# SYNCC-IN/hyperscanning-signal-analysis

Hardware: AMD Instinct MI355X
Metric: MVAR+ffDTF windows/sec, 2x32-ch dyad p=8, 256 freqs (higher is better)
Workload: dtype f64; 1 GPU; C2: 1 dyad(s)/GPU, 2x32 ch @500 Hz, 10 min, 2 s windows 50% overlap (599 windows per dyad), MVAR p=8, 256 freqs 0.5-128 Hz; dyads_per_gpu=1, k1=hop blocks summed once, shared by the overlapping windows (hop 500), k2=block Levinson-Whittle recursion, one workgroup per window, one launch, normalisation=inside K3 (rows of window w by workgroups of window w+lag), parallelism=dyad-sharded x1, gather=none

## Files before the change

### hyperscanning_signal_analysis_amd/_lib.py

```python
from __future__ import annotations

import ctypes
import os
from ctypes import POINTER, c_char_p, c_double, c_int, c_int32, c_int64, c_void_p

_HERE = os.path.dirname(os.path.abspath(__file__))
LIB_PATH = os.path.join(_HERE, "libhypermvar.so")

SIGNATURES = {
    "hmv_version": (c_int, []),
    "hmv_last_error": (c_char_p, []),
    "hmv_pad": (c_int, [c_int]),
    "hmv_set_tuning": (c_int, [c_int, c_int64]),
    "hmv_get_tuning": (c_int64, [c_int]),
    "hmv_yw_workspace_doubles": (c_int64, [c_int, c_int]),
    "hmv_lagcov_f64": (c_int, [c_void_p, c_int64, c_int64, c_void_p, c_void_p, c_int64, c_int, c_int, c_int,
                               c_void_p, c_void_p]),
    "hmv_lagcov_regular_workspace_doubles": (c_int64, [c_int64, c_int, c_int, c_int64, c_int]),
    "hmv_lagcov_regular_f64": (c_int, [c_void_p, c_int64, c_int64, c_int64, c_int64, c_int64, c_int, c_int, c_int,
                                       c_void_p, c_void_p, c_void_p]),
    "hmv_yw_solve_f64": (c_int, [c_void_p, c_int64, c_int, c_int, c_void_p, c_void_p, c_void_p, c_void_p,
                                 c_void_p, c_int64, c_void_p]),
    "hmv_twiddles_f64": (c_int, [c_void_p, c_int, c_double, c_int, c_void_p, c_void_p]),
    "hmv_tf_workspace_doubles": (c_int64, [c_int64, c_int, c_int]),
    "hmv_tf_f64": (c_int, [c_void_p, c_int64, c_int, c_int, c_void_p, c_int, c_void_p, c_void_p, c_void_p,
                           c_void_p, c_void_p, c_double, c_void_p, c_void_p]),
    "hmv_ffdtf_norm_f64": (c_int, [c_void_p, c_void_p, c_void_p, c_void_p, c_int64, c_int, c_int, c_int,
                                   c_void_p]),
    "hmv_transpose_c128": (c_int, [c_void_p, c_void_p, c_int64, c_int, c_int, c_void_p]),
    "hmv_spectra_f64": (c_int, [c_void_p, c_void_p, c_void_p, c_int64, c_int, c_int, c_void_p]),
    "hmv_spectra_mmf_f64": (c_int, [c_void_p, c_void_p, c_void_p, c_int64, c_int, c_int, c_void_p]),
    "hmv_pack_c128": (c_int, [c_void_p, c_void_p, c_int64, c_int, c_int, c_void_p]),
    "hmv_cinv_c128": (c_int, [c_void_p, c_int64, c_int, c_int, c_void_p, c_void_p, c_void_p, c_double, c_void_p]),
    "hmv_partial_coherence_c128": (c_int, [c_void_p, c_void_p, c_void_p, c_int64, c_int, c_int, c_void_p]),
    "hmv_gpdc_f64": (c_int, [c_void_p, c_void_p, c_void_p, c_int64, c_int, c_int, c_void_p]),
    "hmv_trial_mean_f64": (c_int, [c_void_p, c_int64, c_int, c_int, c_void_p, c_void_p]),
    "hmv_ddtf_f64": (c_int, [c_void_p, c_void_p, c_void_p, c_int64, c_int, c_int, c_void_p]),
    "hmv_band_sums_f64": (c_int, [c_void_p, c_int64, c_int, c_void_p, c_void_p, c_int, c_void_p, c_void_p]),
    "hmv_dpss_workspace_bytes": (c_int64, [c_int64, c_int, c_int]),
    "hmv_dpss_f64": (c_int, [c_int64, c_double, c_int, c_int, c_void_p, c_void_p, c_void_p, c_int64, c_void_p]),
    "hmv_psd_workspace_bytes": (c_int64, [c_int64, c_int64, c_int]),
    "hmv_psd_multitaper_f64": (c_int, [c_void_p, c_int64, c_int64, c_int64, c_void_p, c_void_p, c_int, c_int64, c_int64,
                                       c_void_p, c_void_p, c_int64, c_int64, c_void_p]),
    "hmv_sliding_workspace_bytes": (c_int64, [c_int64, c_int, c_int, c_int]),
    "hmv_tf_ffdtf_workspace_bytes": (c_int64, [c_int64, c_int, c_int, c_int]),
    "hmv_tf_ffdtf_f64": (c_int, [c_void_p, c_int64, c_int, c_int, c_void_p, c_int, c_void_p, c_void_p, c_void_p, c_void_p,
                                 c_double, c_void_p, c_int64, c_int64, c_void_p, c_void_p, c_void_p]),
    "hmv_tf_ffdtf_bands_workspace_bytes": (c_int64, [c_int64, c_int, c_int, c_int]),
    "hmv_tf_ffdtf_bands_f64": (c_int, [c_void_p, c_int64, c_int, c_int, c_void_p, c_int, c_void_p, c_void_p, c_void_p, c_int,
                                       c_void_p, c_void_p, c_double, c_void_p, c_int64, c_int64, c_void_p, c_void_p,
                                       c_void_p]),
    "hmv_sliding_bands_workspace_bytes": (c_int64, [c_int64, c_int, c_int, c_int]),
    "hmv_sliding_ffdtf_bands_f64": (c_int, [c_void_p, c_int64, c_int64, c_void_p, c_void_p, c_int64, c_int, c_int,
                                            c_int, c_void_p, c_int, c_double, c_void_p, c_void_p, c_void_p, c_int,
                                            c_void_p, c_void_p, c_void_p, c_void_p, c_void_p, c_int64, c_int64, c_double,
                                            c_int64, c_int64, c_int64, c_int64, c_int64, c_void_p, c_void_p, c_void_p,
                                            c_void_p]),
    "hmv_sliding_spectra_workspace_bytes": (c_int64, [c_int64, c_int, c_int, c_int]),
    "hmv_sliding_ffdtf_spectra_f64": (c_int, [c_void_p, c_int64, c_int64, c_void_p, c_void_p, c_int64, c_int, c_int,
                                              c_int, c_void_p, c_int, c_double, c_void_p, c_void_p, c_void_p, c_void_p,
                                              c_void_p, c_void_p, c_void_p, c_int64, c_int64, c_double, c_int64, c_int64,
                                              c_int64, c_int64, c_int64, c_void_p, c_void_p]),
    "hmv_sliding_ffdtf_f64": (c_int, [c_void_p, c_int64, c_int64, c_void_p, c_void_p, c_int64, c_int, c_int,
                                      c_int, c_void_p, c_int, c_double, c_void_p, c_void_p, c_void_p, c_void_p,
                                      c_void_p, c_void_p, c_int64, c_int64, c_double, c_int64, c_int64, c_int64, c_int64,
                                      c_int64, c_void_p, c_void_p, c_void_p, c_void_p]),
    "hmv_sliding_ddtf_workspace_bytes": (c_int64, [c_int64, c_int, c_int, c_int, c_int]),
    "hmv_sliding_ddtf_f64": (c_int, [c_void_p, c_int64, c_int64, c_void_p, c_void_p, c_int64, c_int, c_int, c_int, c_void_p,
                                     c_int, c_double, c_void_p, c_void_p, c_void_p, c_int, c_void_p, c_void_p, c_void_p,
                                     c_void_p, c_void_p, c_int64, c_int64, c_double, c_int64, c_int64, c_int64, c_int64,
                                     c_int64, c_void_p, c_void_p]),
    "hmv_sliding_gpdc_workspace_bytes": (c_int64, [c_int64, c_int, c_int, c_int, c_int]),
    "hmv_sliding_gpdc_f64": (c_int, [c_void_p, c_int64, c_int64, c_void_p, c_void_p, c_int64, c_int, c_int, c_int, c_void_p,
                                     c_int, c_double, c_void_p, c_void_p, c_void_p, c_int, c_void_p, c_void_p, c_void_p,
                                     c_void_p, c_int64, c_int64, c_int64, c_int64, c_int64, c_int64, c_int64, c_void_p,
                                     c_void_p]),
    "hmv_yw_solve_auto_f64": (c_int, [c_void_p, c_int64, c_int, c_int, c_int, c_int] + [c_void_p] * 7 + [c_int64, c_void_p]),
    "hmv_sliding_auto_workspace_bytes": (c_int64, [c_int, c_int64, c_int, c_int, c_int, c_int]),
    "hmv_sliding_auto_f64": (c_int, [c_int, c_void_p, c_int64, c_int64, c_void_p, c_void_p, c_int64, c_int, c_int, c_int,
                                     c_int, c_void_p, c_int, c_double, c_void_p, c_void_p, c_void_p, c_int] +
                             [c_void_p] * 8 + [c_int64, c_int64, c_double, c_int64, c_int64, c_int64, c_int64, c_int64,
                                               c_void_p, c_void_p]),
    "hmv_lagcov_ensemble_workspace_doubles": (c_int64, [c_int64, c_int, c_int, c_int, c_int64, c_int64]),
    "hmv_lagcov_ensemble_f64": (c_int, [c_void_p, c_int64, c_int64, c_int64, c_void_p, c_void_p, c_void_p, c_int64,
                                        c_void_p, c_void_p, c_int64, c_int, c_int, c_int, c_void_p, c_void_p, c_int64,
                                        c_int64, c_int64, c_int64, c_void_p]),
    "hmv_sliding_ensemble_workspace_bytes": (c_int64, [c_int, c_int64, c_int, c_int, c_int, c_int, c_int, c_int64, c_int64]),
    "hmv_sliding_ensemble_f64": (c_int, [c_int, c_void_p, c_int64, c_int64, c_int64, c_void_p, c_void_p, c_void_p, c_int64,
                                         c_void_p, c_void_p, c_int64, c_int, c_int, c_int, c_void_p, c_int, c_double,
                                         c_void_p, c_void_p, c_void_p, c_int] + [c_void_p] * 6 +
                                 [c_int64, c_int64, c_double, c_int64, c_int64, c_int64, c_void_p, c_void_p]),
    "hmv_fad_workspace_bytes": (c_int64, [c_int64, c_int]),
    "hmv_fad_f64": (c_int, [c_void_p, c_int64, c_int64, c_void_p, c_void_p, c_int64, c_int, c_int, c_int, c_int, c_int,
                            c_double, c_double, c_int] + [c_void_p] * 17),
    "hmv_fad_decompose_f64": (c_int, [c_void_p, c_int64, c_int, c_double, c_double, c_int] + [c_void_p] * 13),
    "hmv_surrogate_shift_f64": (c_int, [c_void_p, c_int64, c_int64, c_int64, c_void_p, c_void_p, c_int64, c_void_p, c_int64,
                                        c_int, c_int, c_int, c_int, c_void_p, c_void_p]),
    "hmv_surrogate_phase_c128": (c_int, [c_void_p, c_int64, c_void_p, c_int, c_int, c_int, c_void_p, c_void_p]),
    "hmv_null_accumulate_f64": (c_int, [c_void_p, c_void_p, c_void_p, c_void_p, c_int64, c_int, c_int, c_int] + [c_void_p] * 12),
}

FLAG_UNFUSED_NORM = 1
FLAG_YW_TILED = 2
FLAG_YW_ONE_LAUNCH = 4
FLAG_DIRECT_LAGCOV = 8
MEASURE_FFDTF = 0
MEASURE_DDTF = 1
MEASURE_GPDC = 2
CRITERIA = {"AIC": 0, "HQ": 1, "SC": 2}
TUNE_NORM_LAG = 1
TUNE_LAG_GROUP = 2
TUNE_K3_FORM = 3
TUNE_YW_FORM = 4
TUNE_K3_LDS_PAD = 5


_lib = None


class HypermvarLibraryError(ImportError):
    pass


def load():
    global _lib
    if _lib is not None:
        return _lib
    global LIB_PATH
    LIB_PATH = os.environ.get("HYPERMVAR_LIB", LIB_PATH)
    if not os.path.exists(LIB_PATH):
        raise HypermvarLibraryError(
            f"{LIB_PATH} not found: build the HIP library first "
            f"(python -c 'import __graft_entry__ as g; g.build()' or make -C {_HERE}/csrc). "
            "There is no CPU fallback for the MVAR/ffDTF path.")
    lib = ctypes.CDLL(LIB_PATH)
    for name, (res, args) in SIGNATURES.items():
        try:
            fn = getattr(lib, name)
        except AttributeError as e:
            raise HypermvarLibraryError(f"{LIB_PATH} does not export {name}") from e
        fn.restype = res
        fn.argtypes = args
    _lib = lib
    return lib


def check(rc: int, what: str):
    if rc == 0:
        return
    lib = load()
    if rc < 0:
        raise ValueError(f"{what}: {lib.hmv_last_error().decode()} (code {rc})")
    raise RuntimeError(f"{what}: HIP error {rc}")
```

### hyperscanning_signal_analysis_amd/csrc/capi.hip

```cpp
#include "../../include/hypermvar.h"
#include "hmv_kernels.h"

#include <atomic>
#include <cmath>
#include <cstdio>
#include <cstdlib>
#include <cstring>

namespace {
thread_local char g_err[256] = "";

int fail(int code, const char* msg) {
  snprintf(g_err, sizeof(g_err), "%s", msg);
  return code;
}
int pad_of(int m) { return (m < 1 || m > HMV_MAX_CHANNELS) ? -1 : ((m + 15) / 16) * 16; }
inline hipStream_t S(void* s) { return reinterpret_cast<hipStream_t>(s); }
inline size_t align256(size_t b) { return (b + 255) & ~size_t(255); }

constexpr int N_TUNE = 6;
struct TuneRange { long long lo, hi; };
constexpr TuneRange kTuneRange[N_TUNE] = {{0, 0}, {0, 1 << 20}, {0, 3}, {0, 2}, {0, 3}, {0, 140000}};
long long env_knob(const char* name, int key) {
  const char* e = getenv(name);
  if (!e || !*e) return 0;
  char* end = nullptr;
  const long long v = strtoll(e, &end, 10);
  if (end == e || *end != 0 || v < kTuneRange[key].lo || v > kTuneRange[key].hi) {
    fprintf(stderr, "hypermvar: ignoring %s=%s (not an integer in %lld..%lld)\n", name, e, kTuneRange[key].lo,
            kTuneRange[key].hi);
    return 0;
  }
  return v;
}
std::atomic<long long> g_tune[N_TUNE] = {{0}, {env_knob("HYPERMVAR_NORM_LAG", 1)}, {env_knob("HYPERMVAR_LAG_GROUP", 2)},
                                         {env_knob("HYPERMVAR_K3_FORM", 3)}, {env_knob("HYPERMVAR_YW_FORM", 4)},
                                         {env_knob("HYPERMVAR_K3_LDS_PAD", 5)}};
}

namespace hmv {
long long tuning(int key) { return (key >= 1 && key < N_TUNE) ? g_tune[key].load(std::memory_order_relaxed) : -1; }
}

#ifdef HMV_STAMP
static unsigned long long* g_tf_stamps = nullptr;
extern "C" void hmv_debug_set_tf_stamps(void* p) { g_tf_stamps = static_cast<unsigned long long*>(p); }
#endif

extern "C" {

int hmv_version(void) { return HMV_VERSION; }
const char* hmv_last_error(void) { return g_err; }
int hmv_pad(int m) { return pad_of(m); }

int hmv_set_tuning(int key, int64_t value) {
  if (key < 1 || key >= N_TUNE) return fail(-1, "hmv_set_tuning: unknown key");
  if (value < kTuneRange[key].lo || value > kTuneRange[key].hi) return fail(-1, "hmv_set_tuning: value out of range");
  g_tune[key].store(value, std::memory_order_relaxed);
  return 0;
}
int64_t hmv_get_tuning(int key) { return hmv::tuning(key); }

int64_t hmv_yw_workspace_doubles(int m, int p) {
  const int mp = pad_of(m);
  if (mp < 0 || p < 1 || p > HMV_MAX_ORDER) return -1;
  return hmv::yw_ws_tiles(p) * (int64_t)mp * mp;
}

int hmv_lagcov_f64(const double* x, int64_t rec_stride, int64_t ld, const int64_t* item_rec,
                   const int64_t* item_start, int64_t n_items, int m, int n, int p, double* R, void* stream) {
  const int mp = pad_of(m);
  if (mp < 0) return fail(-1, "hmv_lagcov_f64: channel count must be in 1..64");
  if (p < 1 || p > HMV_MAX_ORDER) return fail(-2, "hmv_lagcov_f64: model order must be in 1..32");
  if (n <= p) return fail(-3, "hmv_lagcov_f64: window shorter than the model order");
  if (!x || !item_rec || !item_start || !R || n_items < 0) return fail(-4, "hmv_lagcov_f64: null pointer");
  hmv::LagcovArgs a{};
  a.x = x; a.rec_stride = rec_stride; a.ld = ld;
  a.item_rec = reinterpret_cast<const long long*>(item_rec);
  a.item_start = reinterpret_cast<const long long*>(item_start);
  a.n_items = n_items; a.m = m; a.n = n; a.p = p; a.R = R;
  return hmv::launch_lagcov(a, mp, S(stream));
}

int64_t hmv_lagcov_regular_workspace_doubles(int64_t n_win, int m, int n, int64_t hop, int p) {
  const int mp = pad_of(m);
  if (mp < 0 || n_win < 0 || hop < 1 || n < 1 || n % hop != 0 || p < 0) return -1;
  return (n_win + n / hop - 1) * (int64_t)(p + 1) * mp * mp;
}

int hmv_lagcov_regular_f64(const double* x, int64_t ld, int64_t T, int64_t first, int64_t hop, int64_t n_win, int m,
                           int n, int p, double* R, double* workspace, void* stream) {
  const int mp = pad_of(m);
  if (mp < 0) return fail(-1, "hmv_lagcov_regular_f64: channel count must be in 1..64");
  if (p < 1 || p > HMV_MAX_ORDER) return fail(-2, "hmv_lagcov_regular_f64: model order must be in 1..32");
  if (n <= p) return fail(-3, "hmv_lagcov_regular_f64: window shorter than the model order");
  if (!x || !R || !workspace || n_win < 0) return fail(-4, "hmv_lagcov_regular_f64: null pointer");
  if (hop < 1 || n % hop != 0 || hop <= p)
    return fail(-5, "hmv_lagcov_regular_f64: the window must be a whole number of hops and a hop longer than the order");
  if (first < 0 || ld < T || (n_win > 0 && first + (n_win - 1) * hop + n > T))
    return fail(-6, "hmv_lagcov_regular_f64: windows do not lie inside the recording");
  if (n_win == 0) return 0;
  const int k = (int)(n / hop);
  hmv::LagcovArgs a{};
  a.x = x; a.rec_stride = 0; a.ld = ld; a.item_rec = nullptr; a.item_start = nullptr;
  a.n_items = n_win + k - 1; a.m = m; a.n = (int)hop; a.p = p; a.R = workspace;
  a.blocks = 1; a.blk_first = first; a.blk_T = T;
  int rc = hmv::launch_lagcov(a, mp, S(stream));
  if (rc) return rc;
  hmv::LagcombArgs c{};
  c.Q = workspace; c.x = x; c.ld = ld; c.first = first; c.hop = hop; c.T = T; c.n_win = n_win; c.k = k; c.m = m; c.p = p;
  c.R = R;
  return hmv::launch_lagcomb(c, mp, S(stream));
}

namespace {
bool ens_shared_form(int n, int p, int64_t grid_hop, int64_t flags) {
  return grid_hop > 0 && !(flags & HMV_FLAG_DIRECT_LAGCOV) &&
         hmv::lagcov_ensemble_shared_ok(n, grid_hop, p, HMV_MAX_HOPS_ENSEMBLE);
}
bool ens_grid_ok(int64_t n_items, int64_t n_groups, int n, int64_t ld, int64_t T, int64_t grid_hop, int64_t grid_nwin) {
  return grid_hop > 0 && grid_nwin >= 1 && n_items == n_groups * grid_nwin && (grid_nwin - 1) * grid_hop + n <= T && ld >= T;
}
int64_t ens_q_tiles(int64_t n_items, int n, int p, int64_t grid_hop, int64_t grid_nwin) {
  if (grid_hop <= 0 || grid_nwin < 1 || !ens_shared_form(n, p, grid_hop, 0)) return 0;
  return hmv::lagcov_ensemble_q_tiles(n_items, grid_nwin, (int)(n / grid_hop));
}
}

int64_t hmv_lagcov_ensemble_workspace_doubles(int64_t n_items, int m, int n, int p, int64_t grid_hop, int64_t grid_nwin) {
  const int mp = pad_of(m);
  if (mp < 0 || n_items < 0 || p < 1 || p > HMV_MAX_ORDER || n <= p || grid_hop < 0 || grid_nwin < 0) return -1;
  return ens_q_tiles(n_items, n, p, grid_hop, grid_nwin) * (int64_t)(p + 1) * mp * mp;
}

int hmv_lagcov_ensemble_f64(const double* x, int64_t rec_stride, int64_t ld, int64_t T, const int64_t* trial_rec,
                            const int64_t* trial_start, const int64_t* group_ptr, int64_t n_groups,
                            const int64_t* item_group, const int64_t* item_offset, int64_t n_items, int m, int n, int p,
                            double* R, double* workspace, int64_t workspace_doubles, int64_t grid_hop, int64_t grid_nwin,
                            int64_t flags, void* stream) {
  const int mp = pad_of(m);
  if (mp < 0) return fail(-1, "hmv_lagcov_ensemble_f64: channel count must be in 1..64");
  if (p < 1 || p > HMV_MAX_ORDER) return fail(-2, "hmv_lagcov_ensemble_f64: model order must be in 1..32");
  if (n <= p) return fail(-3, "hmv_lagcov_ensemble_f64: window shorter than the model order");
  if (!x || !trial_rec || !trial_start || !group_ptr || !item_group || !item_offset || !R || n_items < 0)
    return fail(-4, "hmv_lagcov_ensemble_f64: null pointer");
  if (n_groups < 1) return fail(-10, "hmv_lagcov_ensemble_f64: n_groups must be >= 1");
  if (grid_hop != 0 && !ens_grid_ok(n_items, n_groups, n, ld, T, grid_hop, grid_nwin))
    return fail(-9, "hmv_lagcov_ensemble_f64: inconsistent regular window grid");
  const bool shared = ens_shared_form(n, p, grid_hop, flags);
  if (shared) {
    const int64_t need = ens_q_tiles(n_items, n, p, grid_hop, grid_nwin) * (int64_t)(p + 1) * mp * mp;
    if (!workspace || workspace_doubles < need) return fail(-7, "hmv_lagcov_ensemble_f64: workspace too small");
  }
  hmv::LagcovEnsArgs a{};
  a.x = x; a.rec_stride = rec_stride; a.ld = ld; a.T = T;
  a.trial_rec = reinterpret_cast<const long long*>(trial_rec);
  a.trial_start = reinterpret_cast<const long long*>(trial_start);
  a.group_ptr = reinterpret_cast<const long long*>(group_ptr);
  a.item_group = reinterpret_cast<const long long*>(item_group);
  a.item_offset = reinterpret_cast<const long long*>(item_offset);
  a.n_items = n_items; a.m = m; a.n = n; a.p = p; a.R = R;
  if (shared) { a.it0 = 0; a.nwin = grid_nwin; a.hop = grid_hop; a.k = (int)(n / grid_hop); a.Q = workspace; }
  return hmv::launch_lagcov_ensemble(a, mp, shared, S(stream));
}

int hmv_yw_solve_f64(const double* R, int64_t n_items, int m, int p, double* ws, double* ar, double* V,
                     double* vq_logdet, int32_t* info, int64_t flags, void* stream) {
  const int mp = pad_of(m);
  if (mp < 0) return fail(-1, "hmv_yw_solve_f64: channel count must be in 1..64");
  if (p < 1 || p > HMV_MAX_ORDER) return fail(-2, "hmv_yw_solve_f64: model order must be in 1..32");
  if (!R || !ws || !ar || !V || !info || n_items < 0) return fail(-4, "hmv_yw_solve_f64: null pointer");
  hmv::YwArgs a{};
  a.R = R; a.n_items = n_items; a.m = m; a.p = p; a.ws = ws; a.ar = ar; a.V = V;
  a.Vq_logdet = vq_logdet; a.info = info; a.tiled = (flags & HMV_FLAG_YW_TILED) ? 1 : ((flags & HMV_FLAG_YW_ONE_LAUNCH) ? 0 : -1);
  return hmv::launch_yw(a, mp, S(stream));
}

namespace {
double crit_factor(int crit, int n) {
  return crit == 0 ? 2.0 : (crit == 1 ? 2.0 * log(log((double)n)) : log((double)n));
}
}

int hmv_yw_solve_auto_f64(const double* R, int64_t n_items, int m, int pmax, int n, int crit, double* ws, double* ar,
                          double* V, int32_t* order_out, double* crit_out, double* vq_logdet, int32_t* info, int64_t flags,
                          void* stream) {
  const int mp = pad_of(m);
  if (mp < 0) return fail(-1, "hmv_yw_solve_auto_f64: channel count must be in 1..64");
  if (pmax < 1 || pmax > HMV_MAX_ORDER) return fail(-2, "hmv_yw_solve_auto_f64: largest model order must be in 1..32");
  if (n <= pmax) return fail(-3, "hmv_yw_solve_auto_f64: window shorter than the largest model order");
  if (crit < 0 || crit > 2) return fail(-5, "hmv_yw_solve_auto_f64: criterion must be 0 (AIC), 1 (HQ) or 2 (SC)");
  if (flags & (HMV_FLAG_YW_TILED | HMV_FLAG_YW_ONE_LAUNCH))
    return fail(-6, "hmv_yw_solve_auto_f64: the LDL^T forms of K2 have no automatic order");
  if (!R || !ws || !ar || !V || !order_out || !info || n_items < 0) return fail(-4, "hmv_yw_solve_auto_f64: null pointer");
  hmv::YwArgs a{};
  a.R = R; a.n_items = n_items; a.m = m; a.p = pmax; a.ws = ws; a.ar = ar; a.V = V; a.Vq_logdet = vq_logdet; a.info = info;
  a.tiled = -1;
  hmv::YwAutoArgs sel{};
  sel.n = n; sel.crit_c = crit_factor(crit, n); sel.order_out = order_out; sel.crit_out = crit_out;
  return hmv::launch_yw_auto(a, sel, mp, S(stream));
}

int hmv_twiddles_f64(const double* freqs, int F, double fs, int p, double* tw, void* stream) {
  if (!freqs || !tw || F < 0 || p < 1) return fail(-4, "hmv_twiddles_f64: bad argument");
  if (F == 0) return 0;
  return hmv::launch_twiddles(freqs, F, fs, p, tw, S(stream));
}

int64_t hmv_tf_workspace_doubles(int64_t n_items, int m, int p) {
  const int mp = pad_of(m);
  if (mp < 0 || p < 1 || n_items < 0) return -1;
  return (int64_t)hmv::tf_workspace_doubles(n_items, mp, p);
}

int hmv_tf_f64(const double* ar, int64_t n_items, int m, int p, const double* tw, int F, double* P,
               double* rowsum, double* H, double* A, int32_t* info, double pivot_tau, double* ws,
               void* stream) {
  const int mp = pad_of(m);
  if (mp < 0) return fail(-1, "hmv_tf_f64: channel count must be in 1..64");
  if (p < 1) return fail(-2, "hmv_tf_f64: model order must be >= 1");
  if (!ar || !tw || !info || !ws || n_items < 0 || F < 0) return fail(-4, "hmv_tf_f64: null pointer");
  if ((P == nullptr) != (rowsum == nullptr)) return fail(-5, "hmv_tf_f64: P and rowsum go together");
  if (!(pivot_tau > 0.0) || pivot_tau > 1.0) return fail(-6, "hmv_tf_f64: pivot_tau must be in (0, 1]");
  hmv::TfArgs a{};
  a.ar = ar; a.arx = ws; a.tw = tw; a.Zin = nullptr; a.detph = nullptr; a.P = P; a.rowsum = rowsum; a.H = H; a.A = A; a.info = info;
  a.n_items = n_items; a.F = F; a.p = p; a.m = m; a.tau = pivot_tau;
  a.stamps = nullptr;
#ifdef HMV_STAMP
  a.stamps = g_tf_stamps;
#endif
  return hmv::launch_tf_inv(a, mp, S(stream));
}

int hmv_ffdtf_norm_f64(const double* P, const double* rowsum, double* den, double* out, int64_t n_items,
                       int F, int m, int normalise, void* stream) {
  const int mp = pad_of(m);
  if (mp < 0) return fail(-1, "hmv_ffdtf_norm_f64: channel count must be in 1..64");
  if (!P || !out || (normalise && (!rowsum || !den))) return fail(-4, "hmv_ffdtf_norm_f64: null pointer");
  hmv::NormArgs a;
  a.P = P; a.rowsum = rowsum; a.den = den; a.out = out; a.n_items = n_items; a.F = F; a.m = m; a.m_pad = mp;
  a.normalise = normalise;
  return hmv::launch_ffdtf_norm(a, S(stream));
}

int hmv_transpose_c128(const double* in, double* out, int64_t n_items, int F, int m, void* stream) {
  const int mp = pad_of(m);
  if (mp < 0) return fail(-1, "hmv_transpose_c128: channel count must be in 1..64");
  if (!in || !out) return fail(-4, "hmv_transpose_c128: null pointer");
  return hmv::launch_transpose_c128(in, out, n_items, F, m, mp, S(stream));
}

int hmv_spectra_f64(const double* H, const double* V, double* Sout, int64_t n_items, int m, int F, void* stream) {
  const int mp = pad_of(m);
  if (mp < 0) return fail(-1, "hmv_spectra_f64: channel count must be in 1..64");
  if (!H || !V || !Sout) return fail(-4, "hmv_spectra_f64: null pointer");
  hmv::SpecArgs a;
  a.H = H; a.V = V; a.S = Sout; a.S_mmf = nullptr; a.n_items = n_items; a.F = F; a.m = m; a.sym = 0;
  return hmv::launch_spectra(a, mp, S(stream));
}

int hmv_spectra_mmf_f64(const double* H, const double* V, double* Sout, int64_t n_items, int m, int F, void* stream) {
  const int mp = pad_of(m);
  if (mp < 0) return fail(-1, "hmv_spectra_mmf_f64: channel count must be in 1..64");
  if (!H || !V || !Sout) return fail(-4, "hmv_spectra_mmf_f64: null pointer");
  hmv::SpecArgs a;
  a.H = H; a.V = V; a.S = nullptr; a.S_mmf = Sout; a.n_items = n_items; a.F = F; a.m = m; a.sym = 0;
  return hmv::launch_spectra(a, mp, S(stream));
}

int hmv_pack_c128(const double* in, double* out, int64_t n_items, int F, int m, void* stream) {
  const int mp = pad_of(m);
  if (mp < 0) return fail(-1, "hmv_pack_c128: channel count must be in 1..64");
  if (!in || !out || n_items < 0 || F < 0) return fail(-4, "hmv_pack_c128: null pointer");
  return hmv::launch_pack_c128(in, out, n_items, F, m, mp, S(stream));
}

int hmv_cinv_c128(const double* Z, int64_t n_items, int m, int F, double* Zinv, double* detph, int32_t* info,
                  double pivot_tau, void* stream) {
  const int mp = pad_of(m);
  if (mp < 0) return fail(-1, "hmv_cinv_c128: channel count must be in 1..64");
  if (!Z || !Zinv || !info || n_items < 0 || F < 0) return fail(-4, "hmv_cinv_c128: null pointer");
  if (!(pivot_tau > 0.0) || pivot_tau > 1.0) return fail(-6, "hmv_cinv_c128: pivot_tau must be in (0, 1]");
  hmv::TfArgs a{};
  a.ar = nullptr; a.arx = nullptr; a.tw = nullptr; a.Zin = Z; a.detph = detph; a.P = nullptr; a.rowsum = nullptr;
  a.H = Zinv; a.A = nullptr; a.info = info; a.n_items = n_items; a.F = F; a.p = 0; a.m = m; a.tau = pivot_tau;
  a.stamps = nullptr;
  return hmv::launch_cinv(a, mp, S(stream));
}

int hmv_partial_coherence_c128(const double* Sinv, const double* detph, double* kappa, int64_t n_items, int m, int F,
                               void* stream) {
  const int mp = pad_of(m);
  if (mp < 0) return fail(-1, "hmv_partial_coherence_c128: channel count must be in 1..64");
  if (!Sinv || !detph || !kappa || n_items < 0 || F < 0) return fail(-4, "hmv_partial_coherence_c128: null pointer");
  return hmv::launch_pcoh(Sinv, detph, kappa, n_items, F, m, mp, S(stream));
}

int hmv_gpdc_f64(const double* A, const double* V, double* G, int64_t n_items, int m, int F, void* stream) {
  const int mp = pad_of(m);
  if (mp < 0) return fail(-1, "hmv_gpdc_f64: channel count must be in 1..64");
  if (!A || !V || !G || n_items < 0 || F < 0) return fail(-4, "hmv_gpdc_f64: null pointer");
  return hmv::launch_gpdc(A, V, G, n_items, F, m, mp, S(stream));
}

int hmv_trial_mean_f64(const double* R_trials, int64_t n_trials, int m, int p, double* R_mean, void* stream) {
  const int mp = pad_of(m);
  if (mp < 0) return fail(-1, "hmv_trial_mean_f64: channel count must be in 1..64");
  if (!R_trials || !R_mean || n_trials < 1 || n_trials > 0x7fffffff || p < 0)
    return fail(-4, "hmv_trial_mean_f64: bad argument");
  return hmv::launch_trial_mean(R_trials, R_mean, (long long)(p + 1) * mp * mp, (int)n_trials, S(stream));
}

int hmv_ddtf_f64(const double* ffdtf, const double* kappa, double* ddtf, int64_t n_items, int m, int F, void* stream) {
  if (!ffdtf || !kappa || !ddtf || n_items < 0 || m < 1 || F < 0) return fail(-4, "hmv_ddtf_f64: bad argument");
  return hmv::launch_ddtf(ffdtf, kappa, ddtf, (long long)n_items * m * m * F, S(stream));
}

int hmv_band_sums_f64(const double* ffdtf, int64_t n_rows, int F, const int32_t* bin_lo, const int32_t* bin_hi,
                      int n_bands, double* out, void* stream) {
  if (!ffdtf || !bin_lo || !bin_hi || !out || n_rows < 0 || F < 1 || n_bands < 0)
    return fail(-4, "hmv_band_sums_f64: bad argument");
  return hmv::launch_band_sums(ffdtf, bin_lo, bin_hi, out, n_rows, F, n_bands, S(stream));
}

int64_t hmv_psd_workspace_bytes(int64_t ch_chunk, int64_t n_times, int n_tapers) {
  if (ch_chunk < 1 || n_times < 2 || n_tapers < 1) return -1;
  return (int64_t)hmv::psd_workspace_bytes(ch_chunk, n_times, n_tapers);
}

int hmv_psd_multitaper_f64(const double* x, int64_t n_ch, int64_t n_times, int64_t ld, const double* tapers,
                           const double* weights, int n_tapers, int64_t bin_lo, int64_t bin_hi, double* psd,
                           void* workspace, int64_t workspace_bytes, int64_t ch_chunk, void* stream) {
  if (!x || !tapers || !weights || !psd || !workspace) return fail(-4, "hmv_psd_multitaper_f64: null pointer");
  if (n_ch < 0 || n_times < 2 || n_times > 0x7fffffff || n_tapers < 1 || ch_chunk < 1 || ld < n_times)
    return fail(-2, "hmv_psd_multitaper_f64: bad size");
  if (bin_lo < 0 || bin_hi < bin_lo || bin_hi > n_times / 2) return fail(-3, "hmv_psd_multitaper_f64: bad frequency bins");
  if (workspace_bytes < hmv::psd_workspace_bytes(ch_chunk, n_times, n_tapers))
    return fail(-7, "hmv_psd_multitaper_f64: workspace too small");
  const int rc = hmv::launch_psd(x, n_ch, n_times, ld, tapers, weights, n_tapers, bin_lo, bin_hi, psd, workspace, ch_chunk,
                                 S(stream));
  if (rc <= -20) return fail(rc, "hmv_psd_multitaper_f64: hipFFT plan / execution failed");
  return rc;
}

int64_t hmv_dpss_workspace_bytes(int64_t n_times, int k_max, int sym) {
  if (n_times < 2 || k_max < 1 || k_max > n_times) return -1;
  return (int64_t)hmv::dpss_workspace_bytes(n_times, k_max, sym != 0);
}

int hmv_dpss_f64(int64_t n_times, double half_nbw, int k_max, int sym, double* tapers, double* ratios, void* workspace,
                 int64_t workspace_bytes, void* stream) {
  if (!tapers || !workspace) return fail(-4, "hmv_dpss_f64: null pointer");
  if (n_times < 2 || n_times > 0x3fffffff || k_max < 1 || k_max > n_times)
    return fail(-2, "hmv_dpss_f64: bad size");
  if (!(half_nbw > 0.0) || half_nbw >= 0.5 * (double)n_times)
    return fail(-3, "hmv_dpss_f64: the time-half-bandwidth product must lie in (0, n_times / 2)");
  if (workspace_bytes < hmv::dpss_workspace_bytes(n_times, k_max, sym != 0)) return fail(-7, "hmv_dpss_f64: workspace too small");
  const int rc = hmv::launch_dpss(n_times, half_nbw, k_max, sym != 0, tapers, ratios, workspace, S(stream));
  if (rc <= -20) return fail(rc, "hmv_dpss_f64: hipFFT plan / execution failed");
  if (rc < 0) return fail(rc, "hmv_dpss_f64: bad argument");
  return rc;
}

namespace {
struct TfFfWs {
  size_t off_arx, off_P, off_rowsum, off_cnt, off_tail, total;
};
int64_t norm_lag_items(int mp, int F);
TfFfWs tf_ff_layout(int64_t n, int mp, int p, int F, bool bands = false) {
  TfFfWs w;
  size_t o = 0;
  const size_t t = (size_t)mp * mp;
  w.off_arx = o;    o += align256(sizeof(double) * hmv::tf_workspace_doubles(n, mp, p));
  w.off_P = o;      o += align256(sizeof(double) * n * F * t);
  w.off_rowsum = o; o += align256(sizeof(double) * n * F * mp);
  w.off_cnt = o;    o += align256(sizeof(int) * (2 * n + 1 + n * mp));
  w.off_tail = o;
  if (bands) {
    const int64_t lag = norm_lag_items(mp, F);
    o += align256(sizeof(double) * (size_t)(n < lag ? n : lag) * F * t);
  }
  w.total = o;
  return w;
}
int64_t norm_lag_items(int mp, int F) {
  const int64_t slots = (mp == 64 || mp == 48) ? 1024 : (mp == 32 ? 2048 : 5120);
  int64_t lag = (6 * slots + F - 1) / (F < 1 ? 1 : F);
  if (const int64_t t = hmv::tuning(HMV_TUNE_NORM_LAG)) lag = t;
  return lag < 8 ? 8 : lag;
}
}

int64_t hmv_tf_ffdtf_workspace_bytes(int64_t n_items, int m, int p, int F) {
  const int mp = pad_of(m);
  if (mp < 0 || n_items < 0 || p < 1 || F < 1) return -1;
  return (int64_t)tf_ff_layout(n_items, mp, p, F).total;
}

namespace {
int tf_ffdtf_impl(const char* who, const double* ar, int64_t n_items, int m, int p, const double* tw, int F, double* ffdtf,
                  double* band_out, const int32_t* bin_lo, const int32_t* bin_hi, int n_bands, double* den, double* H,
                  int32_t* info, double pivot_tau, void* workspace, int64_t workspace_bytes, int64_t flags,
                  void* ev_k3_start, void* ev_k3_stop, void* stream) {
  auto failw = [&](int code, const char* msg) {
    char buf[200];
    snprintf(buf, sizeof(buf), "%s: %s", who, msg);
    return fail(code, buf);
  };
  const int mp = pad_of(m);
  const bool bands = (band_out != nullptr);
  if (mp < 0) return failw(-1, "channel count must be in 1..64");
  if (p < 1) return failw(-2, "model order must be >= 1");
  if (n_items == 0) return 0;
  if (!ar || !tw || (!ffdtf && !bands) || !den || !info || !workspace || n_items < 0 || F < 1)
    return failw(-4, "null pointer / empty grid");
  if (!(pivot_tau > 0.0) || pivot_tau > 1.0) return failw(-6, "pivot_tau must be in (0, 1]");
  if (bands) {
    if (!bin_lo || !bin_hi || n_bands < 1) return failw(-4, "band bins missing");
    if (F % 32 != 0 || F > hmv::tf_band_max_F(mp) || (flags & HMV_FLAG_UNFUSED_NORM))
      return failw(-10, "in-kernel band sums need F % 32 == 0, F within the row worker's LDS block and the fused normalisation");
  }
  const TfFfWs w = tf_ff_layout(n_items, mp, p, F, bands);
  if ((int64_t)w.total > workspace_bytes) return failw(-7, "workspace too small");
  char* base = static_cast<char*>(workspace);
  const size_t t = (size_t)mp * mp;
  hmv::TfArgs a{};
  a.ar = ar; a.arx = reinterpret_cast<double*>(base + w.off_arx); a.tw = tw;
  a.P = reinterpret_cast<double*>(base + w.off_P); a.rowsum = reinterpret_cast<double*>(base + w.off_rowsum);
  a.H = H;
  a.info = info; a.n_items = n_items; a.F = F; a.p = p; a.m = m; a.tau = pivot_tau;
  const bool fused = bands || (!(flags & HMV_FLAG_UNFUSED_NORM) && (F % 16 == 0) && (reinterpret_cast<uintptr_t>(ffdtf) % 16 == 0));
  const int64_t lag = norm_lag_items(mp, F);
  const int64_t n_fused = fused ? n_items : 0;
  if (n_fused > 0) {
    a.ff = bands ? nullptr : ffdtf; a.den = den; a.fuse_items = n_fused; a.lag = (int)lag;
    if (bands) {
      a.bands = band_out; a.band_lo = reinterpret_cast<const int*>(bin_lo); a.band_hi = reinterpret_cast<const int*>(bin_hi);
      a.nb = n_bands;
    }
    a.wcount = reinterpret_cast<int*>(base + w.off_cnt);
    a.ready = a.wcount + n_items;
    a.missed = a.ready + n_items;
  }
#ifdef HMV_STAMP
  a.stamps = g_tf_stamps;
#endif
  hipStream_t st = S(stream);
  int rc = hmv::launch_tf_inv(a, mp, st, reinterpret_cast<hipEvent_t>(ev_k3_start), reinterpret_cast<hipEvent_t>(ev_k3_stop));
  if (rc) return rc;
  if (n_fused < n_items) {
    const int64_t n_tail = n_items - n_fused;
    double* tail = bands ? reinterpret_cast<double*>(base + w.off_tail) : ffdtf + (size_t)n_fused * m * m * F;
    rc = hmv_ffdtf_norm_f64(a.P + (size_t)n_fused * F * t, a.rowsum + (size_t)n_fused * F * mp, den + (size_t)n_fused * mp,
                            tail, n_tail, F, m, 1, stream);
    if (!rc && bands)
      rc = hmv::launch_band_sums(tail, reinterpret_cast<const int*>(bin_lo), reinterpret_cast<const int*>(bin_hi),
                                 band_out + (size_t)n_fused * m * m * n_bands, n_tail * (long long)m * m, F, n_bands, st);
  }
  return rc;
}
}

int64_t hmv_tf_ffdtf_bands_workspace_bytes(int64_t n_items, int m, int p, int F) {
  const int mp = pad_of(m);
  if (mp < 0 || n_items < 0 || p < 1 || F < 1) return -1;
  return (int64_t)tf_ff_layout(n_items, mp, p, F, true).total;
}

int hmv_tf_ffdtf_f64(const double* ar, int64_t n_items, int m, int p, const double* tw, int F, double* ffdtf,
                     double* den, double* H, int32_t* info, double pivot_tau, void* workspace, int64_t workspace_bytes,
                     int64_t flags, void* ev_k3_start, void* ev_k3_stop, void* stream) {
  return tf_ffdtf_impl("hmv_tf_ffdtf_f64", ar, n_items, m, p, tw, F, ffdtf, nullptr, nullptr, nullptr, 0, den, H, info,
                       pivot_tau, workspace, workspace_bytes, flags, ev_k3_start, ev_k3_stop, stream);
}

int hmv_tf_ffdtf_bands_f64(const double* ar, int64_t n_items, int m, int p, const double* tw, int F, double* band_out,
                           const int32_t* bin_lo, const int32_t* bin_hi, int n_bands, double* den, int32_t* info,
                           double pivot_tau, void* workspace, int64_t workspace_bytes, int64_t flags, void* ev_k3_start,
                           void* ev_k3_stop, void* stream) {
  if (!band_out) return fail(-4, "hmv_tf_ffdtf_bands_f64: null pointer / empty grid");
  return tf_ffdtf_impl("hmv_tf_ffdtf_bands_f64", ar, n_items, m, p, tw, F, nullptr, band_out, bin_lo, bin_hi, n_bands, den,
                       nullptr, info, pivot_tau, workspace, workspace_bytes, flags, ev_k3_start, ev_k3_stop, stream);
}

namespace {
enum Measure { MEAS_FFDTF = 0, MEAS_DDTF = 1, MEAS_GPDC = 2 };
struct SlidingWs {
  size_t off_R, off_Q, off_ws, off_ar, off_V, off_tf, off_den, off_tw, off_H, off_B, off_G, off_full, total;
};
SlidingWs sliding_layout(int64_t chunk, int mp, int p, int F, bool bands = false, bool spectra = false, int measure = MEAS_FFDTF,
                         int64_t q_tiles = -1) {
  SlidingWs w;
  size_t o = 0;
  const size_t t = (size_t)mp * mp;
  w.off_R = o;      o += align256(sizeof(double) * chunk * (p + 1) * t);
  w.off_Q = o;      o += align256(sizeof(double) * (q_tiles >= 0 ? q_tiles : chunk + HMV_MAX_HOPS_PER_WINDOW - 1) * (p + 1) * t);
  w.off_ws = o;     o += align256(sizeof(double) * chunk * hmv::yw_ws_tiles(p) * t);
  w.off_ar = o;     o += align256(sizeof(double) * chunk * t * p);
  w.off_V = o;      o += align256(sizeof(double) * chunk * t);
  w.off_tf = o;
  if (measure != MEAS_GPDC) o += tf_ff_layout(chunk, mp, p, F, bands && measure == MEAS_FFDTF).total;
  w.off_den = o;    o += align256(sizeof(double) * chunk * mp);
  w.off_tw = o;     o += align256(sizeof(double) * F * p * 2);
  w.off_H = o;
  if (spectra) o += align256(sizeof(double) * 2 * chunk * F * t);
  w.off_B = o;
  if (measure == MEAS_DDTF) o += align256(sizeof(double) * chunk * (p + 1) * t);
  w.off_G = o;
  if (measure == MEAS_DDTF) o += align256(sizeof(double) * chunk * (2 * p + 1) * t);
  w.off_full = o;
  if (measure != MEAS_FFDTF && bands) o += align256(sizeof(double) * chunk * (mp * mp) * F);
  w.total = o;
  return w;
}
int64_t sliding_bytes(int64_t chunk, int m, int p, int F, int n_bands = 0, bool spectra = false, int measure = MEAS_FFDTF,
                      int64_t q_tiles = -1) {
  const int mp = pad_of(m);
  if (mp < 0 || chunk < 1 || p < 1 || p > HMV_MAX_ORDER || F < 1 || n_bands < 0 || measure < MEAS_FFDTF ||
      measure > MEAS_GPDC)
    return -1;
  return (int64_t)sliding_layout(chunk, mp, p, F, n_bands > 0, spectra, measure, q_tiles).total;
}
struct ForkJoin {
  hipEvent_t fork = nullptr, join = nullptr;
};
ForkJoin* fork_join_events() {
  constexpr int MAXDEV = 64;
  thread_local ForkJoin tl[MAXDEV];
  int dev = 0;
  if (hipGetDevice(&dev) != hipSuccess || dev < 0 || dev >= MAXDEV) return nullptr;
  ForkJoin& e = tl[dev];
  if (!e.fork) {
    if (hipEventCreateWithFlags(&e.fork, hipEventDisableTiming) != hipSuccess) return nullptr;
    if (hipEventCreateWithFlags(&e.join, hipEventDisableTiming) != hipSuccess) return nullptr;
  }
  return &e;
}
}

int64_t hmv_sliding_workspace_bytes(int64_t chunk, int m, int p, int F) { return sliding_bytes(chunk, m, p, F); }

namespace {
struct EnsDesc {
  const int64_t* trial_rec;
  const int64_t* trial_start;
  const int64_t* group_ptr;
  int64_t n_groups, T;
};
struct SlidingArgs {
  const char* who;
  const double* x = nullptr;
  int64_t rec_stride = 0, ld = 0;
  const int64_t* item_rec = nullptr;
  const int64_t* item_start = nullptr;
  int64_t n_items = 0;
  int m = 0, n = 0, p = 0;
  const double* freqs = nullptr;
  int F = 0;
  double fs = 0.0;
  double* ffdtf = nullptr;
  double* band_out = nullptr;
  const int32_t* bin_lo = nullptr;
  const int32_t* bin_hi = nullptr;
  int n_bands = 0;
  double* S_out = nullptr;
  double* ar_out = nullptr;
  double* V_out = nullptr;
  int32_t* info_yw = nullptr;
  int32_t* info_tf = nullptr;
  void* workspace = nullptr;
  int64_t workspace_bytes = 0, chunk = 0;
  double pivot_tau = 1.0;
  int64_t flags = 0, grid_hop = 0, grid_first = 0, grid_nwin = 0, grid_T = 0;
  void* ev_k3_start = nullptr;
  void* ev_k3_stop = nullptr;
  void* stream = nullptr;
  void* aux_stream = nullptr;
  int measure = MEAS_FFDTF;
  int crit = -1;
  int32_t* order_out = nullptr;
  double* crit_out = nullptr;
  const EnsDesc* ens = nullptr;
};
int sliding_impl(const SlidingArgs& a) {
  const bool automatic = a.crit >= 0;
  const bool bands = (a.band_out != nullptr);
  auto fail = [&](int code, const char* msg) {
    const char* own = strchr(msg, ':');
    char buf[220];
    snprintf(buf, sizeof(buf), "%s%s", a.who, own ? own : msg);
    return ::fail(code, buf);
  };
  const int mp = pad_of(a.m);
  if (mp < 0) return fail(-1, "hmv_sliding_ffdtf_f64: channel count must be in 1..64");
  if (a.p < 1 || a.p > HMV_MAX_ORDER) return fail(-2, "hmv_sliding_ffdtf_f64: model order must be in 1..32");
  if (a.n <= a.p) return fail(-3, "hmv_sliding_ffdtf_f64: window shorter than the model order");
  if (automatic && a.crit > 2) return fail(-5, "hmv_sliding_ffdtf_f64: criterion must be 0 (AIC), 1 (HQ) or 2 (SC)");
  if (automatic && (a.flags & (HMV_FLAG_YW_TILED | HMV_FLAG_YW_ONE_LAUNCH)))
    return fail(-6, "hmv_sliding_ffdtf_f64: the LDL^T forms of K2 have no automatic order");
  if (a.n_items == 0) return 0;
  if (automatic && !a.order_out) return fail(-4, "hmv_sliding_ffdtf_f64: null pointer / empty grid");
  if (!a.x || !a.item_rec || !a.item_start || !a.freqs || (!a.ffdtf && !bands) || !a.info_yw ||
      (!a.info_tf && a.measure != MEAS_GPDC) || !a.workspace || a.F < 1 || a.chunk < 1)
    return fail(-4, "hmv_sliding_ffdtf_f64: null pointer / empty grid");
  if (bands && (!a.bin_lo || !a.bin_hi || a.n_bands < 1)) return fail(-4, "hmv_sliding_ffdtf_f64: band bins missing");
  bool ens_shared = false;
  if (a.ens) {
    if (!a.ens->trial_rec || !a.ens->trial_start || !a.ens->group_ptr)
      return fail(-4, "hmv_sliding_ffdtf_f64: null pointer / empty grid");
    if (a.ens->n_groups < 1) return fail(-10, "hmv_sliding_ffdtf_f64: n_groups must be >= 1");
    if (a.grid_hop != 0 && !ens_grid_ok(a.n_items, a.ens->n_groups, a.n, a.ld, a.ens->T, a.grid_hop, a.grid_nwin))
      return fail(-9, "hmv_sliding_ffdtf_f64: inconsistent regular window grid");
    ens_shared = ens_shared_form(a.n, a.p, a.grid_hop, a.flags);
  }
  const SlidingWs w = sliding_layout(a.chunk, mp, a.p, a.F, bands, a.S_out != nullptr, a.measure,
                                     a.ens ? (ens_shared ? ens_q_tiles(a.chunk, a.n, a.p, a.grid_hop, a.grid_nwin) : 0) : -1);
  if ((int64_t)w.total > a.workspace_bytes) return fail(-7, "hmv_sliding_ffdtf_f64: workspace too small");
  bool regular = !a.ens && a.grid_hop > 0 && !(a.flags & HMV_FLAG_DIRECT_LAGCOV);
  if (regular) {
    if (a.grid_nwin < 1 || a.grid_first < 0 || a.n_items % a.grid_nwin != 0 ||
        a.grid_first + (a.grid_nwin - 1) * a.grid_hop + a.n > a.grid_T || a.ld < a.grid_T)
      return fail(-9, "hmv_sliding_ffdtf_f64: inconsistent regular window grid");
    regular = (a.n % a.grid_hop == 0) && (a.n / a.grid_hop >= 2) && (a.n / a.grid_hop <= HMV_MAX_HOPS_PER_WINDOW) &&
              a.grid_hop > a.p;
  }
  hipStream_t st0 = S(a.stream), st1 = S(a.aux_stream);
  const bool split = (a.aux_stream && a.aux_stream != a.stream) && !(a.flags & HMV_FLAG_YW_ONE_LAUNCH);
  ForkJoin* fj = nullptr;
  if (split) {
    fj = fork_join_events();
    if (!fj) return fail(-8, "hmv_sliding_ffdtf_f64: cannot create fork/join events");
  }
  int rc = 0;
  const size_t t = (size_t)mp * mp;
  const int64_t n_chunks = (a.n_items + a.chunk - 1) / a.chunk;
  char* base = static_cast<char*>(a.workspace);
  double* R = reinterpret_cast<double*>(base + w.off_R);
  double* Qb = reinterpret_cast<double*>(base + w.off_Q);
  double* ws = reinterpret_cast<double*>(base + w.off_ws);
  double* ar = reinterpret_cast<double*>(base + w.off_ar);
  double* V = reinterpret_cast<double*>(base + w.off_V);
  void* tfws = base + w.off_tf;
  double* den = reinterpret_cast<double*>(base + w.off_den);
  double* tw = reinterpret_cast<double*>(base + w.off_tw);
  const bool k3_bands = bands && a.measure == MEAS_FFDTF;
  const int64_t tfws_bytes = (int64_t)tf_ff_layout(a.chunk, mp, a.p, a.F, k3_bands).total;
  rc = hmv_twiddles_f64(a.freqs, a.F, a.fs, a.p, tw, st0);
  const size_t ws_item = (size_t)hmv_yw_workspace_doubles(a.m, a.p);
  for (int64_t ci = 0; ci < n_chunks && rc == 0; ++ci) {
    const int64_t i0 = ci * a.chunk;
    const int64_t c = (a.n_items - i0 < a.chunk) ? (a.n_items - i0) : a.chunk;
    double* ar_c = a.ar_out ? a.ar_out + (size_t)i0 * t * a.p : ar;
    double* V_c = a.V_out ? a.V_out + (size_t)i0 * t : V;
    if (a.ens) {
      hmv::LagcovEnsArgs ea{};
      ea.x = a.x; ea.rec_stride = a.rec_stride; ea.ld = a.ld; ea.T = a.ens->T;
      ea.trial_rec = reinterpret_cast<const long long*>(a.ens->trial_rec);
      ea.trial_start = reinterpret_cast<const long long*>(a.ens->trial_start);
      ea.group_ptr = reinterpret_cast<const long long*>(a.ens->group_ptr);
      ea.item_group = reinterpret_cast<const long long*>(a.item_rec + i0);
      ea.item_offset = reinterpret_cast<const long long*>(a.item_start + i0);
      ea.n_items = c; ea.m = a.m; ea.n = a.n; ea.p = a.p; ea.R = R;
      if (ens_shared) {
        ea.it0 = i0; ea.nwin = a.grid_nwin; ea.hop = a.grid_hop; ea.k = (int)(a.n / a.grid_hop); ea.Q = Qb;
      }
      rc = hmv::launch_lagcov_ensemble(ea, mp, ens_shared, st0);
    } else if (regular) {
      for (int64_t it = i0; it < i0 + c && rc == 0;) {
        const int64_t rec = it / a.grid_nwin, w0 = it - rec * a.grid_nwin;
        const int64_t run = ((a.grid_nwin - w0) < (i0 + c - it)) ? (a.grid_nwin - w0) : (i0 + c - it);
        rc = hmv_lagcov_regular_f64(a.x + rec * a.rec_stride, a.ld, a.grid_T, a.grid_first + w0 * a.grid_hop, a.grid_hop,
                                    run, a.m, a.n, a.p, R + (size_t)(it - i0) * (a.p + 1) * t, Qb, st0);
        it += run;
      }
    } else {
      rc = hmv_lagcov_f64(a.x, a.rec_stride, a.ld, a.item_rec + i0, a.item_start + i0, c, a.m, a.n, a.p, R, st0);
    }
    if (rc) break;
    if (automatic) {
      hmv::YwArgs ya{};
      ya.R = R; ya.n_items = c; ya.m = a.m; ya.p = a.p; ya.ws = ws; ya.ar = ar_c; ya.V = V_c; ya.info = a.info_yw + i0;
      ya.tiled = -1;
      hmv::YwAutoArgs sel{};
      sel.n = a.n; sel.crit_c = crit_factor(a.crit, a.n); sel.order_out = a.order_out + i0;
      sel.crit_out = a.crit_out ? a.crit_out + (size_t)i0 * a.p : nullptr;
      rc = hmv::launch_yw_auto(ya, sel, mp, st0);
      if (rc) break;
    }
    const bool ldl = (a.flags & (HMV_FLAG_YW_TILED | HMV_FLAG_YW_ONE_LAUNCH)) || hmv::tuning(HMV_TUNE_YW_FORM) == 1;
    const bool tiled = (a.flags & HMV_FLAG_YW_TILED) || (ldl && !(a.flags & HMV_FLAG_YW_ONE_LAUNCH) && mp == 64 && c >= 128);
    const int64_t yw_flags = (a.flags & ~(int64_t)(HMV_FLAG_YW_TILED | HMV_FLAG_YW_ONE_LAUNCH)) |
                             (ldl ? (tiled ? HMV_FLAG_YW_TILED : HMV_FLAG_YW_ONE_LAUNCH) : 0);
    const int64_t c0 = (split && tiled && c >= 16) ? (c + 1) / 2 : c, c1 = c - c0;
    if (c1 > 0 && !automatic) {
      int hrc = (int)hipEventRecord(fj->fork, st0);
      if (!hrc) hrc = (int)hipStreamWaitEvent(st1, fj->fork, 0);
      if (hrc) { rc = hrc; break; }
      rc = hmv_yw_solve_f64(R + (size_t)c0 * (a.p + 1) * t, c1, a.m, a.p, ws + (size_t)c0 * ws_item,
                            ar_c + (size_t)c0 * t * a.p, V_c + (size_t)c0 * t, nullptr, a.info_yw + i0 + c0, yw_flags, st1);
      hrc = (int)hipEventRecord(fj->join, st1);
      if (!hrc) hrc = (int)hipStreamWaitEvent(st0, fj->join, 0);
      if (hrc) {
        (void)hipStreamSynchronize(st1);
        if (!rc) rc = hrc;
      }
      if (rc) break;
    }
    if (!automatic) rc = hmv_yw_solve_f64(R, c0, a.m, a.p, ws, ar_c, V_c, nullptr, a.info_yw + i0, yw_flags, st0);
    if (rc) break;
    const bool last = (ci == n_chunks - 1);
    double* Hc = a.S_out ? reinterpret_cast<double*>(base + w.off_H) : nullptr;
    double* full_c = (a.measure == MEAS_FFDTF) ? nullptr
                     : bands ? reinterpret_cast<double*>(base + w.off_full) : a.ffdtf + (size_t)i0 * a.m * a.m * a.F;
    if (a.measure == MEAS_GPDC) {
      rc = hmv::launch_gpdc_sliding(ar_c, V_c, tw, full_c, c, a.F, a.m, mp, a.p, st0);
    } else {
      rc = tf_ffdtf_impl(a.who, ar_c, c, a.m, a.p, tw, a.F,
                         k3_bands ? nullptr : (full_c ? full_c : a.ffdtf + (size_t)i0 * a.m * a.m * a.F),
                         k3_bands ? a.band_out + (size_t)i0 * a.m * a.m * a.n_bands : nullptr, a.bin_lo, a.bin_hi,
                         a.n_bands, den, Hc, a.info_tf + (size_t)i0 * a.F, a.pivot_tau, tfws, tfws_bytes, a.flags,
                         last ? a.ev_k3_start : nullptr, last ? a.ev_k3_stop : nullptr, st0);
    }
    if (!rc && a.measure == MEAS_DDTF) {
      hmv::DdtfArgs da{};
      da.ar = ar_c; da.V = V_c; da.info_yw = a.info_yw + i0;
      da.B = reinterpret_cast<double*>(base + w.off_B); da.G = reinterpret_cast<double*>(base + w.off_G);
      da.freqs = a.freqs; da.fs = a.fs; da.ff = full_c; da.out = full_c;
      da.n_items = c; da.F = a.F; da.m = a.m; da.p = a.p;
      rc = hmv::launch_ddtf_sliding(da, mp, st0);
    }
    if (!rc && a.measure != MEAS_FFDTF && bands)
      rc = hmv::launch_band_sums(full_c, reinterpret_cast<const int*>(a.bin_lo), reinterpret_cast<const int*>(a.bin_hi),
                                 a.band_out + (size_t)i0 * a.m * a.m * a.n_bands, c * (long long)a.m * a.m, a.F,
                                 a.n_bands, st0);
    if (!rc && a.S_out) {
      hmv::SpecArgs sa;
      sa.H = Hc; sa.V = V_c; sa.S = nullptr; sa.S_mmf = a.S_out + (size_t)i0 * a.m * a.m * a.F * 2;
      sa.n_items = c; sa.F = a.F; sa.m = a.m; sa.sym = 1;
      rc = hmv::launch_spectra(sa, mp, st0);
    }
  }
  return rc;
}
}

int64_t hmv_sliding_bands_workspace_bytes(int64_t chunk, int m, int p, int F) { return sliding_bytes(chunk, m, p, F, 1); }

int hmv_sliding_ffdtf_f64(const double* x, int64_t rec_stride, int64_t ld, const int64_t* item_rec,
                          const int64_t* item_start, int64_t n_items, int m, int n, int p,
                          const double* freqs, int F, double fs, double* ffdtf, double* ar_out, double* V_out,
                          int32_t* info_yw, int32_t* info_tf, void* workspace, int64_t workspace_bytes,
                          int64_t chunk, double pivot_tau, int64_t flags, int64_t grid_hop, int64_t grid_first,
                          int64_t grid_nwin, int64_t grid_T, void* ev_k3_start, void* ev_k3_stop, void* stream,
                          void* aux_stream) {
  SlidingArgs a{"hmv_sliding_ffdtf_f64"};
  a.x = x; a.rec_stride = rec_stride; a.ld = ld; a.item_rec = item_rec; a.item_start = item_start; a.n_items = n_items;
  a.m = m; a.n = n; a.p = p; a.freqs = freqs; a.F = F; a.fs = fs;
  a.ffdtf = ffdtf;
  a.ar_out = ar_out; a.V_out = V_out; a.info_yw = info_yw; a.info_tf = info_tf;
  a.workspace = workspace; a.workspace_bytes = workspace_bytes; a.chunk = chunk; a.pivot_tau = pivot_tau; a.flags = flags;
  a.grid_hop = grid_hop; a.grid_first = grid_first; a.grid_nwin = grid_nwin; a.grid_T = grid_T;
  a.ev_k3_start = ev_k3_start; a.ev_k3_stop = ev_k3_stop;
  a.stream = stream; a.aux_stream = aux_stream;
  return sliding_impl(a);
}

int hmv_sliding_ffdtf_bands_f64(const double* x, int64_t rec_stride, int64_t ld, const int64_t* item_rec,
                                const int64_t* item_start, int64_t n_items, int m, int n, int p,
                                const double* freqs, int F, double fs, double* band_out, const int32_t* bin_lo,
                                const int32_t* bin_hi, int n_bands, double* ar_out, double* V_out,
                                int32_t* info_yw, int32_t* info_tf, void* workspace, int64_t workspace_bytes,
                                int64_t chunk, double pivot_tau, int64_t flags, int64_t grid_hop, int64_t grid_first,
                                int64_t grid_nwin, int64_t grid_T, void* ev_k3_start, void* ev_k3_stop, void* stream,
                                void* aux_stream) {
  if (!band_out && n_items != 0) return fail(-4, "hmv_sliding_ffdtf_bands_f64: null pointer / empty grid");
  SlidingArgs a{"hmv_sliding_ffdtf_bands_f64"};
  a.x = x; a.rec_stride = rec_stride; a.ld = ld; a.item_rec = item_rec; a.item_start = item_start; a.n_items = n_items;
  a.m = m; a.n = n; a.p = p; a.freqs = freqs; a.F = F; a.fs = fs;
  a.band_out = band_out; a.bin_lo = bin_lo; a.bin_hi = bin_hi; a.n_bands = n_bands;
  a.ar_out = ar_out; a.V_out = V_out; a.info_yw = info_yw; a.info_tf = info_tf;
  a.workspace = workspace; a.workspace_bytes = workspace_bytes; a.chunk = chunk; a.pivot_tau = pivot_tau; a.flags = flags;
  a.grid_hop = grid_hop; a.grid_first = grid_first; a.grid_nwin = grid_nwin; a.grid_T = grid_T;
  a.ev_k3_start = ev_k3_start; a.ev_k3_stop = ev_k3_stop;
  a.stream = stream; a.aux_stream = aux_stream;
  return sliding_impl(a);
}

int64_t hmv_sliding_spectra_workspace_bytes(int64_t chunk, int m, int p, int F) {
  return sliding_bytes(chunk, m, p, F, 0, true);
}

int hmv_sliding_ffdtf_spectra_f64(const double* x, int64_t rec_stride, int64_t ld, const int64_t* item_rec,
                                  const int64_t* item_start, int64_t n_items, int m, int n, int p,
                                  const double* freqs, int F, double fs, double* ffdtf, double* S_out, double* ar_out,
                                  double* V_out, int32_t* info_yw, int32_t* info_tf, void* workspace,
                                  int64_t workspace_bytes, int64_t chunk, double pivot_tau, int64_t flags,
                                  int64_t grid_hop, int64_t grid_first, int64_t grid_nwin, int64_t grid_T, void* stream,
                                  void* aux_stream) {
  if (!S_out && n_items != 0) return fail(-4, "hmv_sliding_ffdtf_spectra_f64: null pointer / empty grid");
  SlidingArgs a{"hmv_sliding_ffdtf_spectra_f64"};
  a.x = x; a.rec_stride = rec_stride; a.ld = ld; a.item_rec = item_rec; a.item_start = item_start; a.n_items = n_items;
  a.m = m; a.n = n; a.p = p; a.freqs = freqs; a.F = F; a.fs = fs;
  a.ffdtf = ffdtf; a.S_out = S_out;
  a.ar_out = ar_out; a.V_out = V_out; a.info_yw = info_yw; a.info_tf = info_tf;
  a.workspace = workspace; a.workspace_bytes = workspace_bytes; a.chunk = chunk; a.pivot_tau = pivot_tau; a.flags = flags;
  a.grid_hop = grid_hop; a.grid_first = grid_first; a.grid_nwin = grid_nwin; a.grid_T = grid_T;
  a.stream = stream; a.aux_stream = aux_stream;
  return sliding_impl(a);
}

int64_t hmv_sliding_ddtf_workspace_bytes(int64_t chunk, int m, int p, int F, int n_bands) {
  return sliding_bytes(chunk, m, p, F, n_bands, false, MEAS_DDTF);
}

int hmv_sliding_ddtf_f64(const double* x, int64_t rec_stride, int64_t ld, const int64_t* item_rec,
                         const int64_t* item_start, int64_t n_items, int m, int n, int p, const double* freqs, int F,
                         double fs, double* out, const int32_t* bin_lo, const int32_t* bin_hi, int n_bands,
                         double* ar_out, double* V_out, int32_t* info_yw, int32_t* info_tf, void* workspace,
                         int64_t workspace_bytes, int64_t chunk, double pivot_tau, int64_t flags, int64_t grid_hop,
                         int64_t grid_first, int64_t grid_nwin, int64_t grid_T, void* stream, void* aux_stream) {
  if (n_bands < 0) return fail(-4, "hmv_sliding_ddtf_f64: n_bands must be >= 0");
  if (!out && n_items != 0) return fail(-4, "hmv_sliding_ddtf_f64: null pointer / empty grid");
  SlidingArgs a{"hmv_sliding_ddtf_f64"};
  a.measure = MEAS_DDTF;
  a.x = x; a.rec_stride = rec_stride; a.ld = ld; a.item_rec = item_rec; a.item_start = item_start; a.n_items = n_items;
  a.m = m; a.n = n; a.p = p; a.freqs = freqs; a.F = F; a.fs = fs;
  if (n_bands > 0) a.band_out = out; else a.ffdtf = out;
  a.bin_lo = bin_lo; a.bin_hi = bin_hi; a.n_bands = n_bands;
  a.ar_out = ar_out; a.V_out = V_out; a.info_yw = info_yw; a.info_tf = info_tf;
  a.workspace = workspace; a.workspace_bytes = workspace_bytes; a.chunk = chunk; a.pivot_tau = pivot_tau; a.flags = flags;
  a.grid_hop = grid_hop; a.grid_first = grid_first; a.grid_nwin = grid_nwin; a.grid_T = grid_T;
  a.stream = stream; a.aux_stream = aux_stream;
  return sliding_impl(a);
}

int64_t hmv_sliding_gpdc_workspace_bytes(int64_t chunk, int m, int p, int F, int n_bands) {
  return sliding_bytes(chunk, m, p, F, n_bands, false, MEAS_GPDC);
}

int hmv_sliding_gpdc_f64(const double* x, int64_t rec_stride, int64_t ld, const int64_t* item_rec,
                         const int64_t* item_start, int64_t n_items, int m, int n, int p, const double* freqs, int F,
                         double fs, double* out, const int32_t* bin_lo, const int32_t* bin_hi, int n_bands,
                         double* ar_out, double* V_out, int32_t* info_yw, void* workspace, int64_t workspace_bytes,
                         int64_t chunk, int64_t flags, int64_t grid_hop, int64_t grid_first, int64_t grid_nwin,
                         int64_t grid_T, void* stream, void* aux_stream) {
  if (n_bands < 0) return fail(-4, "hmv_sliding_gpdc_f64: n_bands must be >= 0");
  if (!out && n_items != 0) return fail(-4, "hmv_sliding_gpdc_f64: null pointer / empty grid");
  SlidingArgs a{"hmv_sliding_gpdc_f64"};
  a.measure = MEAS_GPDC;
  a.x = x; a.rec_stride = rec_stride; a.ld = ld; a.item_rec = item_rec; a.item_start = item_start; a.n_items = n_items;
  a.m = m; a.n = n; a.p = p; a.freqs = freqs; a.F = F; a.fs = fs;
  if (n_bands > 0) a.band_out = out; else a.ffdtf = out;
  a.bin_lo = bin_lo; a.bin_hi = bin_hi; a.n_bands = n_bands;
  a.ar_out = ar_out; a.V_out = V_out; a.info_yw = info_yw;
  a.workspace = workspace; a.workspace_bytes = workspace_bytes; a.chunk = chunk; a.flags = flags;
  a.grid_hop = grid_hop; a.grid_first = grid_first; a.grid_nwin = grid_nwin; a.grid_T = grid_T;
  a.stream = stream; a.aux_stream = aux_stream;
  return sliding_impl(a);
}

int64_t hmv_sliding_auto_workspace_bytes(int measure, int64_t chunk, int m, int pmax, int F, int n_bands) {
  const bool spectra = (n_bands == -1 && measure == HMV_MEASURE_FFDTF);
  return sliding_bytes(chunk, m, pmax, F, spectra ? 0 : n_bands, spectra, measure);
}

int hmv_sliding_auto_f64(int measure, const double* x, int64_t rec_stride, int64_t ld, const int64_t* item_rec,
                         const int64_t* item_start, int64_t n_items, int m, int n, int pmax, int crit, const double* freqs,
                         int F, double fs, double* out, const int32_t* bin_lo, const int32_t* bin_hi, int n_bands,
                         double* S_out, double* ar_out, double* V_out, int32_t* order_out, double* crit_out,
                         int32_t* info_yw, int32_t* info_tf, void* workspace, int64_t workspace_bytes, int64_t chunk,
                         double pivot_tau, int64_t flags, int64_t grid_hop, int64_t grid_first, int64_t grid_nwin,
                         int64_t grid_T, void* stream, void* aux_stream) {
  if (measure < HMV_MEASURE_FFDTF || measure > HMV_MEASURE_GPDC)
    return fail(-4, "hmv_sliding_auto_f64: measure must be HMV_MEASURE_FFDTF, _DDTF or _GPDC");
  if (crit < 0 || crit > 2) return fail(-5, "hmv_sliding_auto_f64: criterion must be 0 (AIC), 1 (HQ) or 2 (SC)");
  if (n_bands < 0) return fail(-4, "hmv_sliding_auto_f64: n_bands must be >= 0");
  if (S_out && (measure != HMV_MEASURE_FFDTF || n_bands != 0))
    return fail(-4, "hmv_sliding_auto_f64: spectra come with the full ffDTF only");
  if (!out && n_items != 0) return fail(-4, "hmv_sliding_auto_f64: null pointer / empty grid");
  SlidingArgs a{"hmv_sliding_auto_f64"};
  a.measure = measure; a.crit = crit; a.order_out = order_out; a.crit_out = crit_out;
  a.x = x; a.rec_stride = rec_stride; a.ld = ld; a.item_rec = item_rec; a.item_start = item_start; a.n_items = n_items;
  a.m = m; a.n = n; a.p = pmax; a.freqs = freqs; a.F = F; a.fs = fs;
  if (n_bands > 0) a.band_out = out; else a.ffdtf = out;
  a.bin_lo = bin_lo; a.bin_hi = bin_hi; a.n_bands = n_bands; a.S_out = S_out;
  a.ar_out = ar_out; a.V_out = V_out; a.info_yw = info_yw; a.info_tf = info_tf;
  a.workspace = workspace; a.workspace_bytes = workspace_bytes; a.chunk = chunk; a.pivot_tau = pivot_tau; a.flags = flags;
  if (measure == HMV_MEASURE_GPDC) { a.info_tf = nullptr; a.pivot_tau = 1.0; }
  a.grid_hop = grid_hop; a.grid_first = grid_first; a.grid_nwin = grid_nwin; a.grid_T = grid_T;
  a.stream = stream; a.aux_stream = aux_stream;
  return sliding_impl(a);
}

int64_t hmv_sliding_ensemble_workspace_bytes(int measure, int64_t chunk, int m, int n, int p, int F, int n_bands,
                                             int64_t grid_hop, int64_t grid_nwin) {
  const bool spectra = (n_bands == -1 && measure == HMV_MEASURE_FFDTF);
  if (n <= p || grid_hop < 0 || grid_nwin < 0) return -1;
  const int64_t q_tiles = ens_q_tiles(chunk, n, p, grid_hop, grid_nwin);
  return sliding_bytes(chunk, m, p, F, spectra ? 0 : n_bands, spectra, measure, q_tiles);
}

int hmv_sliding_ensemble_f64(int measure, const double* x, int64_t rec_stride, int64_t ld, int64_t T,
                             const int64_t* trial_rec, const int64_t* trial_start, const int64_t* group_ptr,
                             int64_t n_groups, const int64_t* item_group, const int64_t* item_offset, int64_t n_items,
                             int m, int n, int p, const double* freqs, int F, double fs, double* out,
                             const int32_t* bin_lo, const int32_t* bin_hi, int n_bands, double* S_out, double* ar_out,
                             double* V_out, int32_t* info_yw, int32_t* info_tf, void* workspace, int64_t workspace_bytes,
                             int64_t chunk, double pivot_tau, int64_t flags, int64_t grid_hop, int64_t grid_nwin,
                             void* stream, void* aux_stream) {
  if (measure < HMV_MEASURE_FFDTF || measure > HMV_MEASURE_GPDC)
    return fail(-4, "hmv_sliding_ensemble_f64: measure must be HMV_MEASURE_FFDTF, _DDTF or _GPDC");
  if (n_bands < 0) return fail(-4, "hmv_sliding_ensemble_f64: n_bands must be >= 0");
  if (S_out && (measure != HMV_MEASURE_FFDTF || n_bands != 0))
    return fail(-4, "hmv_sliding_ensemble_f64: spectra come with the full ffDTF only");
  const int mp = pad_of(m);
  if (mp >= 0 && p >= 1 && p <= HMV_MAX_ORDER && n > p && !out && n_items != 0)
    return fail(-4, "hmv_sliding_ensemble_f64: null pointer / empty grid");
  const EnsDesc ens{trial_rec, trial_start, group_ptr, n_groups, T};
  SlidingArgs a{"hmv_sliding_ensemble_f64"};
  a.measure = measure; a.ens = &ens;
  a.x = x; a.rec_stride = rec_stride; a.ld = ld; a.item_rec = item_group; a.item_start = item_offset; a.n_items = n_items;
  a.m = m; a.n = n; a.p = p; a.freqs = freqs; a.F = F; a.fs = fs;
  if (n_bands > 0) a.band_out = out; else a.ffdtf = out;
  a.bin_lo = bin_lo; a.bin_hi = bin_hi; a.n_bands = n_bands; a.S_out = S_out;
  a.ar_out = ar_out; a.V_out = V_out; a.info_yw = info_yw; a.info_tf = info_tf;
  a.workspace = workspace; a.workspace_bytes = workspace_bytes; a.chunk = chunk; a.pivot_tau = pivot_tau; a.flags = flags;
  if (measure == HMV_MEASURE_GPDC) { a.info_tf = nullptr; a.pivot_tau = 1.0; }
  a.grid_hop = grid_hop; a.grid_nwin = grid_nwin; a.grid_T = T;
  a.stream = stream; a.aux_stream = aux_stream;
  return sliding_impl(a);
}

int64_t hmv_fad_workspace_bytes(int64_t n_series, int pmax) {
  return (n_series < 0 || pmax < 1 || pmax > HMV_MAX_ORDER) ? -1 : 0;
}

int hmv_fad_f64(const double* x, int64_t rec_stride, int64_t ld, const int64_t* item_rec, const int64_t* item_start,
                int64_t n_items, int m, int n, int pmax, int order, int crit, double fs, double imag_tol,
                int pair_conjugates, int32_t* order_out, double* crit_out, double* ar, double* noise_variance,
                double* poles, double* C, double* alpha, double* freq, double* beta, double* bandwidth, double* phi,
                double* B, uint8_t* osc_mask, int32_t* paired, int32_t* n_paired, int32_t* info, void* stream) {
  if (m < 1 || m > HMV_MAX_CHANNELS) return fail(-1, "hmv_fad_f64: channel count must be in 1..64");
  if (pmax < 1 || pmax > HMV_MAX_ORDER) return fail(-2, "hmv_fad_f64: maximum model order must be in 1..32");
  if (n <= pmax) return fail(-3, "hmv_fad_f64: series shorter than the model order");
  if (!x || !item_rec || !item_start || !order_out || !ar || !noise_variance || !poles || !C || !alpha || !freq ||
      !beta || !bandwidth || !phi || !B || !osc_mask || !paired || !n_paired || !info || n_items < 0)
    return fail(-4, "hmv_fad_f64: null pointer");
  if (crit < 0 || crit > 2) return fail(-5, "hmv_fad_f64: criterion must be 0 (AIC), 1 (HQ) or 2 (SC)");
  if (order < 0 || order > pmax) return fail(-6, "hmv_fad_f64: model order must be 0 (automatic) or in 1..pmax");
  hmv::FadArgs a{};
  a.from_fit = 1;
  a.x = x; a.rec_stride = rec_stride; a.ld = ld;
  a.item_rec = reinterpret_cast<const long long*>(item_rec);
  a.item_start = reinterpret_cast<const long long*>(item_start);
  a.n_series = n_items * m; a.m = m; a.n = n; a.pmax = pmax; a.order = order; a.crit = crit;
  a.fs = fs; a.imag_tol = imag_tol; a.pair_conjugates = pair_conjugates != 0;
  a.order_out = order_out; a.crit_out = crit_out; a.ar = ar; a.noise = noise_variance;
  a.poles = poles; a.C = C; a.alpha = alpha; a.freq = freq; a.beta = beta; a.bw = bandwidth; a.phi = phi; a.B = B;
  a.osc = osc_mask; a.paired = paired; a.n_paired = n_paired; a.info = info;
  return hmv::launch_fad(a, S(stream));
}

int hmv_fad_decompose_f64(const double* ar, int64_t n_series, int p, double fs, double imag_tol, int pair_conjugates,
                          double* poles, double* C, double* alpha, double* freq, double* beta, double* bandwidth,
                          double* phi, double* B, uint8_t* osc_mask, int32_t* paired, int32_t* n_paired, int32_t* info,
                          void* stream) {
  if (p < 1 || p > HMV_MAX_ORDER) return fail(-2, "hmv_fad_decompose_f64: model order must be in 1..32");
  if (!ar || !poles || !C || !alpha || !freq || !beta || !bandwidth || !phi || !B || !osc_mask || !paired ||
      !n_paired || !info || n_series < 0)
    return fail(-4, "hmv_fad_decompose_f64: null pointer");
  hmv::FadArgs a{};
  a.from_fit = 0;
  a.n_series = n_series; a.pmax = p;
  a.fs = fs; a.imag_tol = imag_tol; a.pair_conjugates = pair_conjugates != 0;
  a.ar = const_cast<double*>(ar);
  a.poles = poles; a.C = C; a.alpha = alpha; a.freq = freq; a.beta = beta; a.bw = bandwidth; a.phi = phi; a.B = B;
  a.osc = osc_mask; a.paired = paired; a.n_paired = n_paired; a.info = info;
  return hmv::launch_fad(a, S(stream));
}

int hmv_surrogate_shift_f64(const double* x, int64_t rec_stride, int64_t ld, int64_t T, const int64_t* item_rec,
                            const int64_t* item_start, int64_t n_win, const int64_t* shift, int64_t n_rec, int n_surr, int m,
                            int n, int split, double* out, void* stream) {
  if (m < 1 || m > HMV_MAX_CHANNELS) return fail(-1, "hmv_surrogate_shift_f64: channel count must be in 1..64");
  if (n < 2 || n > T) return fail(-3, "hmv_surrogate_shift_f64: window length must be in 2..T");
  if (split < 1 || split >= m) return fail(-5, "hmv_surrogate_shift_f64: split must be in 1..m-1");
  if (n_surr < 1) return fail(-6, "hmv_surrogate_shift_f64: surrogate count must be >= 1");
  if (n_win < 0 || n_rec < 1) return fail(-4, "hmv_surrogate_shift_f64: bad window / recording count");
  if (n_win == 0) return 0;
  if (!x || !item_rec || !item_start || !shift || !out) return fail(-4, "hmv_surrogate_shift_f64: null pointer");
  return hmv::launch_surrogate_shift(x, rec_stride, ld, T, reinterpret_cast<const long long*>(item_rec),
                                     reinterpret_cast<const long long*>(item_start), n_win,
                                     reinterpret_cast<const long long*>(shift), n_rec, n_surr, m, n, split, out, S(stream));
}

int hmv_surrogate_phase_c128(const double* spec, int64_t n_win, const double* phi, int n_surr, int m, int n, double* out,
                             void* stream) {
  if (m < 1 || m > HMV_MAX_CHANNELS) return fail(-1, "hmv_surrogate_phase_c128: channel count must be in 1..64");
  if (n < 2) return fail(-3, "hmv_surrogate_phase_c128: window length must be >= 2");
  if (n_surr < 1) return fail(-6, "hmv_surrogate_phase_c128: surrogate count must be >= 1");
  if (n_win < 0) return fail(-4, "hmv_surrogate_phase_c128: bad window count");
  if (n_win == 0) return 0;
  if (!spec || !phi || !out) return fail(-4, "hmv_surrogate_phase_c128: null pointer");
  return hmv::launch_surrogate_phase(spec, n_win, phi, n_surr, m, n, out, S(stream));
}

int hmv_null_accumulate_f64(const double* observed, const double* surr, const uint8_t* surr_bad, const uint8_t* tested,
                            int64_t n_win, int n_surr, int m, int n_bands, double* M, int32_t* n_valid, int32_t* count,
                            int32_t* count_fwe, int32_t* n_cell, double* mean, double* m2, double* p, double* p_fwe,
                            double* null_mean, double* null_std, void* stream) {
  if (m < 1 || m > HMV_MAX_CHANNELS) return fail(-1, "hmv_null_accumulate_f64: channel count must be in 1..64");
  if (n_bands < 1) return fail(-2, "hmv_null_accumulate_f64: band count must be >= 1");
  if (n_surr < 1) return fail(-6, "hmv_null_accumulate_f64: surrogate count must be >= 1");
  if (n_win < 0) return fail(-4, "hmv_null_accumulate_f64: bad window count");
  const int fin = (p != nullptr) + (p_fwe != nullptr) + (null_mean != nullptr) + (null_std != nullptr);
  if (fin != 0 && fin != 4) return fail(-7, "hmv_null_accumulate_f64: p, p_fwe, null_mean and null_std go together");
  if (n_win == 0) return 0;
  if (!observed || !surr || !surr_bad || !tested || !M || !n_valid || !count || !count_fwe || !n_cell || !mean || !m2)
    return fail(-4, "hmv_null_accumulate_f64: null pointer");
  hmv::NullAccArgs a{};
  a.obs = observed; a.surr = surr; a.bad = surr_bad; a.tested = tested;
  a.n_win = n_win; a.n_surr = n_surr; a.m = m; a.nb = n_bands;
  a.M = M; a.n_valid = n_valid; a.cnt = count; a.cnt_fwe = count_fwe; a.n_cell = n_cell; a.mean = mean; a.m2 = m2;
  a.p = p; a.p_fwe = p_fwe; a.null_mean = null_mean; a.null_std = null_std;
// ... 5 lines not shown
```

### hyperscanning_signal_analysis_amd/csrc/hmv_common.h

```cpp
#pragma once
#include <hip/hip_runtime.h>
#include <stdint.h>
#include <utility>

#define HMV_WAVE 64

namespace hmv {

__device__ __forceinline__ double mfma4(double a, double b, double c) {
  return __builtin_amdgcn_mfma_f64_4x4x4f64(a, b, c, 0, 0, 0);
}
__device__ __forceinline__ double mfma4_nega(double a, double b, double c) {
  return __builtin_amdgcn_mfma_f64_4x4x4f64(a, b, c, 0, 0, 1);
}

template <typename F, int... S>
__device__ __forceinline__ void static_for_impl(F&& f, std::integer_sequence<int, S...>) {
  (f(std::integral_constant<int, S>{}), ...);
}
template <int N, typename F>
__device__ __forceinline__ void static_for(F&& f) {
  static_for_impl(static_cast<F&&>(f), std::make_integer_sequence<int, N>{});
}

__device__ __forceinline__ int lane_id() { return threadIdx.x & 63; }

__device__ __forceinline__ int uni(int v) { return __builtin_amdgcn_readfirstlane(v); }

__device__ __forceinline__ double readlane_f64(double v, int lane) {
  union { double d; int i[2]; } u;
  u.d = v;
  u.i[0] = __builtin_amdgcn_readlane(u.i[0], lane);
  u.i[1] = __builtin_amdgcn_readlane(u.i[1], lane);
  return u.d;
}

__device__ __forceinline__ double shfl_f64(double v, int src_lane) {
  union { double d; int i[2]; } u;
  u.d = v;
  u.i[0] = __builtin_amdgcn_ds_bpermute(src_lane << 2, u.i[0]);
  u.i[1] = __builtin_amdgcn_ds_bpermute(src_lane << 2, u.i[1]);
  return u.d;
}

template <int PATTERN>
__device__ __forceinline__ double swizzle_f64(double v) {
  union { double d; int i[2]; } u;
  u.d = v;
  u.i[0] = __builtin_amdgcn_ds_swizzle(u.i[0], PATTERN);
  u.i[1] = __builtin_amdgcn_ds_swizzle(u.i[1], PATTERN);
  return u.d;
}

__device__ __forceinline__ unsigned long long shfl_u64(unsigned long long v, int src_lane) {
  union { unsigned long long q; int i[2]; } u;
  u.q = v;
  u.i[0] = __builtin_amdgcn_ds_bpermute(src_lane << 2, u.i[0]);
  u.i[1] = __builtin_amdgcn_ds_bpermute(src_lane << 2, u.i[1]);
  return u.q;
}

__device__ __forceinline__ unsigned long long wave_max_u64(unsigned long long k) {
  const int l = lane_id();
#pragma unroll
  for (int m = 1; m < 64; m <<= 1) {
    unsigned long long o = shfl_u64(k, l ^ m);
    k = o > k ? o : k;
  }
  return k;
}

template <int CTRL>
__device__ __forceinline__ unsigned dpp_u32(unsigned v) {
  return (unsigned)__builtin_amdgcn_update_dpp((int)v, (int)v, CTRL, 0xf, 0xf, false);
}
__device__ __forceinline__ unsigned row16_max_u32(unsigned v) {
  asm("s_nop 1\n\t"
      "v_max_u32_dpp %0, %0, %0 quad_perm:[1,0,3,2] row_mask:0xf bank_mask:0xf\n\t"
      "s_nop 1\n\t"
      "v_max_u32_dpp %0, %0, %0 quad_perm:[2,3,0,1] row_mask:0xf bank_mask:0xf\n\t"
      "s_nop 1\n\t"
      "v_max_u32_dpp %0, %0, %0 row_half_mirror row_mask:0xf bank_mask:0xf\n\t"
      "s_nop 1\n\t"
      "v_max_u32_dpp %0, %0, %0 row_mirror row_mask:0xf bank_mask:0xf\n\t"
      "s_nop 1"
      : "+v"(v));
  return v;
}
__device__ __forceinline__ unsigned wave_max_u32(unsigned v) {
  v = row16_max_u32(v);
  asm("v_max_u32_dpp %0, %0, %0 row_bcast:15 row_mask:0xa bank_mask:0xf\n\t"
      "s_nop 1\n\t"
      "v_max_u32_dpp %0, %0, %0 row_bcast:31 row_mask:0xc bank_mask:0xf\n\t"
      "s_nop 1"
      : "+v"(v));
  return (unsigned)__builtin_amdgcn_readlane((int)v, 63);
}
template <int CTRL>
__device__ __forceinline__ double dpp_f64(double v) {
  union { double d; int i[2]; } u;
  u.d = v;
  u.i[0] = __builtin_amdgcn_update_dpp(u.i[0], u.i[0], CTRL, 0xf, 0xf, false);
  u.i[1] = __builtin_amdgcn_update_dpp(u.i[1], u.i[1], CTRL, 0xf, 0xf, false);
  return u.d;
}
__device__ __forceinline__ double row16_sum_dpp(double v) {
  v += dpp_f64<0xB1>(v);
  v += dpp_f64<0x4E>(v);
  v += dpp_f64<0x141>(v);
  v += dpp_f64<0x140>(v);
  return v;
}

__device__ __forceinline__ double row16_sum(double v) {
  const int l = lane_id();
#pragma unroll
  for (int m = 1; m < 16; m <<= 1) v += shfl_f64(v, l ^ m);
  return v;
}

}
```

### hyperscanning_signal_analysis_amd/csrc/hmv_kernels.h

```cpp
#pragma once
#include <hip/hip_runtime.h>
#include <stdint.h>

namespace hmv {

long long tuning(int key);

struct LagcovArgs {
  const double* x;
  long long rec_stride;
  long long ld;
  const long long* item_rec;
  const long long* item_start;
  long long n_items;
  int m, n, p;
  double* R;
  int blocks;
  long long blk_first, blk_T;
};
int launch_lagcov(const LagcovArgs& a, int m_pad, hipStream_t st);
struct LagcombArgs {
  const double* Q;
  const double* x;
  long long ld, first, hop, T;
  long long n_win;
  int k, m, p;
  double* R;
};
int launch_lagcomb(const LagcombArgs& a, int m_pad, hipStream_t st);
struct LagcovEnsArgs {
  const double* x;
  long long rec_stride, ld;
  long long T;
  const long long* trial_rec;
  const long long* trial_start;
  const long long* group_ptr;
  const long long* item_group;
  const long long* item_offset;
  long long n_items;
  int m, n, p;
  double* R;
  long long it0, nwin, hop;
  int k;
  double* Q;
};
bool lagcov_ensemble_shared_ok(int n, long long hop, int p, int max_k);
long long lagcov_ensemble_q_tiles(long long n_items, long long nwin, int k);
int launch_lagcov_ensemble(const LagcovEnsArgs& a, int m_pad, bool shared, hipStream_t st);

struct YwArgs {
  const double* R;
  long long n_items;
  int m, p;
  double* ws;
  double* ar;
  double* V;
  double* Vq_logdet;
  int* info;
  int tiled;
  int only_guarded;
  const int* order;
};
struct YwAutoArgs {
  int n;
  double crit_c;
  int* order_out;
  double* crit_out;
};
long long yw_ws_tiles(int p);
int launch_yw(const YwArgs& a, int m_pad, hipStream_t st);
int launch_yw_lwr(const YwArgs& a, int m_pad, hipStream_t st);
int launch_yw_lwr2(const YwArgs& a, int m_pad, hipStream_t st);
int launch_yw_auto(const YwArgs& a, const YwAutoArgs& s, int m_pad, hipStream_t st);
int launch_yw_guarded(const YwArgs& a, int m_pad, hipStream_t st);

struct TfArgs {
  const double* ar;
  const double* arx;
  const double* tw;
  const double* Zin;
  double* detph;
  double* P;
  double* rowsum;
  double* H;
  double* A;
  int* info;
  long long n_items;
  int F, p, m;
  double tau;
  double* ff;
  double* den;
  int* wcount;
  int* ready;
  int* missed;
  long long fuse_items;
  int lag;
  double* bands;
  const int* band_lo;
  const int* band_hi;
  int nb;
  unsigned long long* stamps;
};
int launch_twiddles(const double* freqs, int F, double fs, int p, double* tw, hipStream_t st);
int launch_tf_inv(const TfArgs& a, int m_pad, hipStream_t st, hipEvent_t ev_start = nullptr, hipEvent_t ev_stop = nullptr);
int launch_cinv(const TfArgs& a, int m_pad, hipStream_t st);
long long tf_workspace_doubles(long long n_items, int m_pad, int p);
int tf_band_max_F(int m_pad);

struct NormArgs {
  const double* P;
  const double* rowsum;
  double* den;
  double* out;
  long long n_items;
  int F, m, m_pad;
  int normalise;
};
int launch_ffdtf_norm(const NormArgs& a, hipStream_t st);

int launch_trial_mean(const double* in, double* out, long long n, int trials, hipStream_t st);
int launch_ddtf(const double* ff, const double* kappa, double* out, long long n, hipStream_t st);
int launch_band_sums(const double* in, const int* lo, const int* hi, double* out, long long rows, int F, int nb,
                     hipStream_t st);

int launch_transpose_c128(const double* in, double* out, long long n_items, int F, int m, int m_pad, hipStream_t st);

struct SpecArgs {
  const double* H;
  const double* V;
  double* S;
  double* S_mmf;
  long long n_items;
  int F, m;
  int sym;
};
int launch_spectra(const SpecArgs& a, int m_pad, hipStream_t st);

int launch_pack_c128(const double* in, double* out, long long n_items, int F, int m, int m_pad, hipStream_t st);
int launch_pcoh(const double* Sinv, const double* detph, double* out, long long n_items, int F, int m, int m_pad, hipStream_t st);
int launch_gpdc(const double* A, const double* V, double* out, long long n_items, int F, int m, int m_pad, hipStream_t st);

struct DdtfArgs {
  const double* ar;
  const double* V;
  int* info_yw;
  double* B;
  double* G;
  const double* freqs;
  double fs;
  const double* ff;
  double* out;
  long long n_items;
  int F, m, p;
};
int launch_ddtf_sliding(const DdtfArgs& a, int m_pad, hipStream_t st);
int launch_gpdc_sliding(const double* ar, const double* V, const double* tw, double* out, long long n_items, int F, int m,
                        int m_pad, int p, hipStream_t st);

long long psd_workspace_bytes(long long ch_chunk, long long n, int K);
int launch_psd(const double* x, long long n_ch, long long n, long long ld, const double* tapers, const double* w, int K,
               long long lo, long long hi, double* psd, void* workspace, long long ch_chunk, hipStream_t st);

long long dpss_workspace_bytes(long long M, int K, int sym);
int launch_dpss(long long M, double NW, int K, int sym, double* tapers, double* ratios, void* workspace, hipStream_t st);

struct FadArgs {
  int from_fit;
  const double* x;
  long long rec_stride, ld;
  const long long* item_rec;
  const long long* item_start;
  long long n_series;
  int m, n;
  int pmax;
  int order;
  int crit;
  double fs, imag_tol;
  int pair_conjugates;
  int* order_out;
  double* crit_out;
  double* ar;
  double* noise;
  double* poles;
  double* C;
  double* alpha;
  double* freq, *beta, *bw, *phi, *B;
  unsigned char* osc;
  int* paired;
  int* n_paired;
  int* info;
};
int launch_fad(const FadArgs& a, hipStream_t st);

int launch_surrogate_shift(const double* x, long long rec_stride, long long ld, long long T, const long long* item_rec,
                           const long long* item_start, long long n_win, const long long* shift, long long n_rec, int n_surr,
                           int m, int n, int split, double* out, hipStream_t st);
int launch_surrogate_phase(const double* spec, long long n_win, const double* phi, int n_surr, int m, int n, double* out,
                           hipStream_t st);
struct NullAccArgs {
  const double* obs;
  const double* surr;
  const unsigned char* bad;
  const unsigned char* tested;
  long long n_win;
  int n_surr, m, nb;
  double* M;
  int* n_valid;
  int* cnt, *cnt_fwe, *n_cell;
  double* mean, *m2;
  double* p, *p_fwe, *null_mean, *null_std;
};
int launch_null_accumulate(const NullAccArgs& a, hipStream_t st);

}
```

### hyperscanning_signal_analysis_amd/csrc/lagcov.hip

```cpp
#include "hmv_common.h"
#include "hmv_kernels.h"
#include <cstdlib>

namespace hmv {

constexpr int LC_TC = 64;
constexpr int LC_HALO = 32;
constexpr int LC_S = LC_TC + LC_HALO + 6;

template <int NT, int LG>
__global__ void __launch_bounds__(256, 2) lagcov_kernel(LagcovArgs a) {
  constexpr int MP = 16 * NT, NIW = NT, NJ = NT;
  __shared__ double xs[MP * LC_S];
  const int l = lane_id();
  const int wv = uni(threadIdx.x >> 6);
  const long long item = blockIdx.x;
  const int lag0 = blockIdx.y * LG;
  const int nl = min(LG, a.p + 1 - lag0);
  const int i = l >> 4, cc = l & 15;
  const int n = a.n, m = a.m;
  const bool blk = a.blocks != 0;
  const long long start = blk ? a.blk_first + item * (long long)n : a.item_start[item];
  const double* x = a.x + (blk ? 0 : a.item_rec[item] * a.rec_stride) + start;
  const long long vlen = blk ? a.blk_T - start : (long long)n;
  const bool mask_a = blk && (n & 3) != 0;

  double acc[LG][NIW][NJ];
#pragma unroll
  for (int g = 0; g < LG; ++g)
#pragma unroll
    for (int I = 0; I < NIW; ++I)
#pragma unroll
      for (int J = 0; J < NJ; ++J) acc[g][I][J] = 0.0;

  constexpr int W = LC_TC + LC_HALO;
  constexpr int NLD = (MP * W + 255) / 256;
  for (int t0 = 0; t0 < n; t0 += LC_TC) {
    double stg[NLD];
#pragma unroll
    for (int r = 0; r < NLD; ++r) {
      const int idx = threadIdx.x + 256 * r;
      const int ch = idx / W, tt = idx - ch * W;
      const int t = t0 + tt;
      stg[r] = (idx < MP * W && ch < m && t < vlen) ? x[(size_t)ch * a.ld + t] : 0.0;
    }
    __syncthreads();
#pragma unroll
    for (int r = 0; r < NLD; ++r) {
      const int idx = threadIdx.x + 256 * r;
      const int ch = idx / W, tt = idx - ch * W;
      if (idx < MP * W) xs[ch * LC_S + tt] = stg[r];
    }
    __syncthreads();
    const int steps = min(LC_TC, n - t0 + 3) >> 2;
    const double* xa = xs + (4 * NT * wv + (l & 3)) * LC_S + (l >> 4);
    const double* xb = xs + cc * LC_S + lag0 + (l >> 4);
    for (int ts = 0; ts < steps; ++ts) {
      double av[NIW];
#pragma unroll
      for (int I = 0; I < NIW; ++I) av[I] = xa[4 * I * LC_S + 4 * ts];
      if (mask_a && t0 + 4 * ts + 3 >= n) {
        const bool in = t0 + 4 * ts + (l >> 4) < n;
#pragma unroll
        for (int I = 0; I < NIW; ++I) av[I] = in ? av[I] : 0.0;
      }
      static_for<LG>([&](auto gc) __attribute__((always_inline)) {
        constexpr int g = decltype(gc)::value;
        if (g < nl) {
          double bv[NJ];
#pragma unroll
          for (int J = 0; J < NJ; ++J) bv[J] = xb[16 * J * LC_S + 4 * ts + g];
#pragma unroll
          for (int I = 0; I < NIW; ++I)
#pragma unroll
            for (int J = 0; J < NJ; ++J) acc[g][I][J] = mfma4(av[I], bv[J], acc[g][I][J]);
        }
      });
    }
  }
  const double scale = blk ? 1.0 : 1.0 / (double)n;
  static_for<LG>([&](auto gc) __attribute__((always_inline)) {
    constexpr int g = decltype(gc)::value;
    if (g < nl) {
      const int lag = lag0 + g;
      double* R = a.R + ((size_t)item * (a.p + 1) + lag) * MP * MP;
#pragma unroll
      for (int I = 0; I < NIW; ++I)
#pragma unroll
        for (int J = 0; J < NJ; ++J) {
          const int row = 4 * (NT * wv + I) + i, col = 16 * J + cc;
          double v = acc[g][I][J] * scale;
          if (!blk && lag == 0 && row == col && row >= m) v = 1.0;
          R[(size_t)row * MP + col] = v;
        }
    }
  });
}

template <int NT>
__global__ void __launch_bounds__(256) lagcomb_kernel(LagcombArgs a) {
  constexpr int MP = 16 * NT, TILE = MP * MP;
  __shared__ double xa[MP * 32], xb[MP * 32];
  const long long w = blockIdx.x;
  const int lag = blockIdx.y;
  const int n = (int)(a.hop * a.k), m = a.m;
  const long long s = a.first + w * a.hop;
  for (int idx = threadIdx.x; idx < MP * lag; idx += 256) {
    const int ch = idx / lag, u = idx - ch * lag;
    const long long ta = s + n - lag + u, tb = s + n + u;
    xa[ch * 32 + u] = (ch < m && ta < a.T) ? a.x[(size_t)ch * a.ld + ta] : 0.0;
    xb[ch * 32 + u] = (ch < m && tb < a.T) ? a.x[(size_t)ch * a.ld + tb] : 0.0;
  }
  __syncthreads();
  const double inv_n = 1.0 / (double)n;
  const double* Q = a.Q + ((size_t)w * (a.p + 1) + lag) * TILE;
  double* R = a.R + ((size_t)w * (a.p + 1) + lag) * TILE;
  for (int e = threadIdx.x; e < TILE; e += 256) {
    const int row = e / MP, col = e - row * MP;
    double acc = 0.0;
    for (int j = 0; j < a.k; ++j) acc += Q[(size_t)j * (a.p + 1) * TILE + e];
    double c = 0.0;
    for (int u = 0; u < lag; ++u) c = __builtin_fma(xa[row * 32 + u], xb[col * 32 + u], c);
    double v = (acc - c) * inv_n;
    if (lag == 0 && row == col && row >= m) v = 1.0;
    R[e] = v;
  }
}

int launch_lagcomb(const LagcombArgs& a, int m_pad, hipStream_t st) {
  if (a.n_win == 0) return 0;
  if (a.p > LC_HALO) return -2;
  const dim3 grid((unsigned)a.n_win, a.p + 1), block(256);
  switch (m_pad) {
    case 16: hipLaunchKernelGGL(lagcomb_kernel<1>, grid, block, 0, st, a); break;
    case 32: hipLaunchKernelGGL(lagcomb_kernel<2>, grid, block, 0, st, a); break;
    case 48: hipLaunchKernelGGL(lagcomb_kernel<3>, grid, block, 0, st, a); break;
    case 64: hipLaunchKernelGGL(lagcomb_kernel<4>, grid, block, 0, st, a); break;
    default: return -1;
  }
  return (int)hipGetLastError();
}

template <int LG>
static int launch_lagcov_lg(const LagcovArgs& a, int m_pad, hipStream_t st) {
  const dim3 grid((unsigned)a.n_items, (a.p + LG) / LG), block(256);
  switch (m_pad) {
    case 16: hipLaunchKernelGGL((lagcov_kernel<1, LG>), grid, block, 0, st, a); break;
    case 32: hipLaunchKernelGGL((lagcov_kernel<2, LG>), grid, block, 0, st, a); break;
    case 48: hipLaunchKernelGGL((lagcov_kernel<3, LG>), grid, block, 0, st, a); break;
    case 64: hipLaunchKernelGGL((lagcov_kernel<4, LG>), grid, block, 0, st, a); break;
    default: return -1;
  }
  return (int)hipGetLastError();
}

int launch_lagcov(const LagcovArgs& a, int m_pad, hipStream_t st) {
  if (a.n_items == 0) return 0;
  if (a.p > LC_HALO) return -2;
  const long long lg = tuning(2 );
  switch (lg) {
    case 1: return launch_lagcov_lg<1>(a, m_pad, st);
    case 2: return launch_lagcov_lg<2>(a, m_pad, st);
    default: return launch_lagcov_lg<3>(a, m_pad, st);
  }
}

}
```

### hyperscanning_signal_analysis_amd/csrc/tf_inv.hip

```cpp
#include "hmv_common.h"
#include "hmv_kernels.h"

namespace hmv {

#ifndef HMV_K3_WGS
#define HMV_K3_WGS 4
#endif

#ifndef HMV_ROW_LOADS_SC1
#define HMV_ROW_LOADS_SC1 0
#endif

#define HMV_LDS_FENCE()                                     \
  do {                                                      \
    __builtin_amdgcn_fence(__ATOMIC_RELEASE, "wavefront");  \
    __builtin_amdgcn_wave_barrier();                        \
    __builtin_amdgcn_fence(__ATOMIC_ACQUIRE, "wavefront");  \
  } while (0)

#ifdef HMV_STAMP
#define HMV_T(idx)                                                                     \
  do {                                                                                 \
    __builtin_amdgcn_sched_barrier(0);                                                 \
    unsigned long long t_;                                                             \
// ... 532 lines not shown
        dd = __builtin_fma(pr, pr, pi * pi);
        double y = __builtin_amdgcn_rcp(dd);
        y = __builtin_fma(__builtin_fma(-dd, y, 1.0), y, y);
        const double e = __builtin_fma(-dd, y, 1.0), tr = pr * y, ti = -pi * y;
        ivr = __builtin_fma(tr, e, tr);
        ivi = __builtin_fma(ti, e, ti);
      };
      reciprocal();
      int rstar = col;
      if (__builtin_expect(need_search, 0)) {
        const unsigned key = valid ? __float_as_uint((float)cand) : 0u;
        const unsigned kmax = wave_max_u32(key);
        rstar = (int)__builtin_ctzll(__builtin_amdgcn_ballot_w64(valid && key == kmax));
        if (rstar != col) {
          pr = readlane_f64(x[jj].x, rstar);
          pi = readlane_f64(x[jj].y, rstar);
          reciprocal();
#pragma unroll
          for (int j2 = 0; j2 < 4; ++j2) {
            const double2 cv = Pbuf[col * 5 + j2];
            x[j2].x = (l == rstar) ? cv.x : x[j2].x;
            x[j2].y = (l == rstar) ? cv.y : x[j2].y;
          }
          if (l == 0) {
            const int oc = s_orig[col], orr = s_orig[rstar];
            s_orig[col] = orr;
            s_orig[rstar] = oc;
          }
        }
      }
      rs[jj] = rstar;
      if constexpr (GEN) {
        double rsq = __builtin_amdgcn_rsq(dd);
        rsq = rsq * __builtin_fma(-0.5 * dd * rsq, rsq, 1.5);
        rsq = rsq * __builtin_fma(-0.5 * dd * rsq, rsq, 1.5);
        const double sg = (rstar != col) ? -rsq : rsq;
        const double ur = pr * sg, ui = pi * sg;
        const double nr_ = __builtin_fma(dpr, ur, -(dpi * ui)), ni_ = __builtin_fma(dpr, ui, dpi * ur);
        dpr = nr_;
        dpi = ni_;
      }
      double2 pv[4];
      {
        const double2* prow = Pbuf + uni(rstar) * 5;
#pragma unroll
        for (int j2 = 0; j2 < 4; ++j2) pv[j2] = prow[j2];
      }
      HMV_LDS_FENCE();
      dds[jj] = dd;
      const bool isp = (l == col);
      const double fr = x[jj].x, fi = x[jj].y;
      double mr = __builtin_fma(fi, ivi, -(fr * ivr));
      double mi = __builtin_fma(-fr, ivi, -(fi * ivr));
      mr = isp ? ivr : mr;
      mi = isp ? ivi : mi;
      const double keep = isp ? 0.0 : 1.0;
#pragma unroll
      for (int j2 = 0; j2 < 4; ++j2) {
        if (j2 == jj) continue;
        const double br = x[j2].x * keep, bi = x[j2].y * keep;
        x[j2].x = __builtin_fma(-mi, pv[j2].y, __builtin_fma(mr, pv[j2].x, br));
        x[j2].y = __builtin_fma(mi, pv[j2].x, __builtin_fma(mr, pv[j2].y, bi));
      }
      x[jj].x = mr;
      x[jj].y = mi;
    }
    if (NT == 4 || l < MP) {
#pragma unroll
      for (int jj = 0; jj < 4; ++jj) Nout[l * 4 + jj] = x[jj];
    }
    const bool all_ok = (dds[0] > 0.0) && (dds[1] > 0.0) && (dds[2] > 0.0) && (dds[3] > 0.0);
    if (l == 0) {
      *reinterpret_cast<int4*>(&s_swp[t % NR][0]) =
          make_int4(rs[0] - 4 * t, rs[1] - (4 * t + 1), rs[2] - (4 * t + 2), rs[3] - (4 * t + 3));
      if (__builtin_expect(!all_ok, 0)) {
        const int bad = !(dds[0] > 0.0) ? 4 * t + 1 : (!(dds[1] > 0.0) ? 4 * t + 2 : (!(dds[2] > 0.0) ? 4 * t + 3 : 4 * t + 4));
        if (s_info == 0) s_info = bad;
      }
      if constexpr (GEN) {
        const double qr = s_det[0], qi = s_det[1];
        s_det[0] = __builtin_fma(qr, dpr, -(qi * dpi));
        s_det[1] = __builtin_fma(qr, dpi, qi * dpr);
      }
    }
    __builtin_amdgcn_s_setprio(0);
  };

  auto load_n = [&](auto tc, double (&nr)[NG], double (&ni)[NG]) __attribute__((always_inline)) {
    constexpr int t = decltype(tc)::value;
    const double2* Nt = Nbuf + (t % NR) * L::NBUF;
    const double dlt = (b == (t & 3) && j == i) ? 1.0 : 0.0;
#pragma unroll
    for (int Ig = 0; Ig < NG; ++Ig) {
      const double2 v = Nt[(16 * Ig + (l & 15)) * 4 + (l >> 4)];
      nr[Ig] = (Ig == (t >> 2)) ? v.x - dlt : v.x;
      ni[Ig] = v.y;
    }
  };
  auto update_block = [&](auto tc, auto jc, const double (&nr)[NG], const double (&ni)[NG])
                          __attribute__((always_inline)) {
    constexpr int t = decltype(tc)::value, J = decltype(jc)::value;
    constexpr int pat = 0x13 | (((t & 3) << 2) << 5);
    const double ur = swizzle_f64<pat>(re[t >> 2][J]), ui = swizzle_f64<pat>(im[t >> 2][J]);
#pragma unroll
    for (int Ig = 0; Ig < NG; ++Ig) {
      re[Ig][J] = mfma4(nr[Ig], ur, re[Ig][J]);
      im[Ig][J] = mfma4(nr[Ig], ui, im[Ig][J]);
    }
#pragma unroll
    for (int Ig = 0; Ig < NG; ++Ig) {
      re[Ig][J] = mfma4_nega(ni[Ig], ui, re[Ig][J]);
      im[Ig][J] = mfma4(ni[Ig], ur, im[Ig][J]);
    }
  };
  auto interchange = [&](auto tc) __attribute__((always_inline)) {
    constexpr int t = decltype(tc)::value, Igp = t >> 2, bp = t & 3;
    const int4 swv = *reinterpret_cast<const int4*>(&s_swp[t % NR][0]);
    if (__builtin_expect(uni(swv.x | swv.y | swv.z | swv.w) == 0, 1)) return;
    const int swr[4] = {uni(swv.x) + 4 * t, uni(swv.y) + 4 * t + 1, uni(swv.z) + 4 * t + 2, uni(swv.w) + 4 * t + 3};
#pragma unroll
    for (int jj = 0; jj < 4; ++jj) {
      const int col = 4 * t + jj;
      const int rstar = swr[jj];
      if (rstar != col) {
        const int Igs = rstar >> 4, bs = (rstar >> 2) & 3, is = rstar & 3;
        if (i == jj && b == bp) {
#pragma unroll
          for (int Jl = 0; Jl < 4; ++Jl) swapb[Jl * 4 + j] = make_double2(re[Igp][Jl], im[Igp][Jl]);
        }
        HMV_LDS_FENCE();
        static_for<NG - Igp>([&](auto ic) __attribute__((always_inline)) {
          constexpr int Ig = Igp + decltype(ic)::value;
          if (Ig == Igs) {
            if (i == is && b == bs) {
#pragma unroll
              for (int Jl = 0; Jl < 4; ++Jl) swapb[16 + Jl * 4 + j] = make_double2(re[Ig][Jl], im[Ig][Jl]);
#pragma unroll
              for (int Jl = 0; Jl < 4; ++Jl) {
                const double2 v = swapb[Jl * 4 + j];
                re[Ig][Jl] = v.x;
                im[Ig][Jl] = v.y;
              }
            }
          }
        });
        HMV_LDS_FENCE();
        if (i == jj && b == bp) {
#pragma unroll
          for (int Jl = 0; Jl < 4; ++Jl) {
            const double2 v = swapb[16 + Jl * 4 + j];
            re[Igp][Jl] = v.x;
            im[Igp][Jl] = v.y;
          }
        }
        HMV_LDS_FENCE();
      }
    }
  };
  auto take_panel = [&](auto tc, auto jc) __attribute__((always_inline)) {
    constexpr int t = decltype(tc)::value, J = decltype(jc)::value;
    const double2* Nt = Nbuf + (t % NR) * L::NBUF;
#pragma unroll
    for (int Ig = 0; Ig < NG; ++Ig) {
      const double2 v = Nt[(16 * Ig + rowl) * 4 + j];
      re[Ig][J] = v.x;
      im[Ig][J] = v.y;
    }
  };

  if (w == 0) factor_panel(std::integral_constant<int, 0>{}, std::integral_constant<int, 0>{});
  HMV_T(1);
  __syncthreads();
  HMV_T(2);
  static_for<NSTEP>([&](auto sc) __attribute__((always_inline)) {
    constexpr int s = decltype(sc)::value;
    constexpr int own = s % NT, Js = s / NT;
    constexpr bool has_next = (s + 1 < NSTEP);
    constexpr int nxt = (s + 1) % NT, Jn = has_next ? (s + 1) / NT : 0;
    if (has_next && w == nxt) __builtin_amdgcn_s_setprio(3);
    if constexpr (s >= 1) {
      constexpr int t = s - 1;
      double ar_[NG], ai_[NG];
#pragma unroll
      for (int Ig = 0; Ig < NG; ++Ig) ar_[Ig] = ai_[Ig] = 0.0;
      if (w == own) load_n(std::integral_constant<int, t>{}, ar_, ai_);
      static_for<4>([&](auto jc) __attribute__((always_inline)) {
        constexpr int Jl = decltype(jc)::value;
        if constexpr (Jl != Js && !(NT == 1 && Jl == t / NT)) {
          if (w == own) update_block(std::integral_constant<int, t>{}, jc, ar_, ai_);
        }
      });
    }
    HMV_T(3);
    __builtin_amdgcn_sched_barrier(0);
    double nr[NG], ni[NG];
    load_n(sc, nr, ni);
    interchange(sc);
    HMV_T(3);
    const bool is_nxt = has_next && (w == nxt);
    if (w == own) take_panel(sc, std::integral_constant<int, Js>{});
    if (is_nxt || !(w == own && Jn == Js)) update_block(sc, std::integral_constant<int, Jn>{}, nr, ni);
    static_for<4>([&](auto jc) __attribute__((always_inline)) {
      constexpr int Jl = decltype(jc)::value;
      if constexpr (Jl != Jn) {
        if (!is_nxt && !(w == own && Jl == Js)) update_block(sc, jc, nr, ni);
      }
    });
    HMV_T(3);
    __builtin_amdgcn_sched_barrier(0);
    if (is_nxt) factor_panel(std::integral_constant<int, s + 1>{}, std::integral_constant<int, Jn>{});
    HMV_T(1);
    __syncthreads();
    HMV_T(2);
  });

  HMV_T(3);
  tf_outputs<NT, GEN, (NT < 4)>(a, item, f, gw, w, wv, re, im, smem, rsum, s_orig, &s_info, s_det
#ifdef HMV_STAMP
                      , tsum, tlast
#endif
  );
}

#ifndef HMV_K3A_INC
#define HMV_K3A_INC "tf_inv64_body.inc"
#endif
#include HMV_K3A_INC
#ifndef HMV_K3A_WGS
#ifdef HMV_STAMP
#define HMV_K3A_WGS 4
#else
#define HMV_K3A_WGS 5
#endif
#endif
static_assert(K3A_PBUF == 0 && K3A_NBUF == 16 * TfLds<4>::PBUF && K3A_RSUM == 16 * (TfLds<4>::TOTAL - TfLds<4>::RSUM),
              "LDS map of the generated body and of the epilogue disagree");

__global__ void __launch_bounds__(256, HMV_K3A_WGS) tf_inv64_asm_kernel(TfArgs a) {
  constexpr int NT = 4;
  __shared__ __attribute__((aligned(16))) unsigned char lds[K3A_LDS_TOTAL];
  int* s_orig = reinterpret_cast<int*>(lds + K3A_SORIG);
  int* s_flag = reinterpret_cast<int*>(lds + K3A_SINFO);
  const int wv = uni(threadIdx.x >> 6);
  const int w = (wv + (int)((blockIdx.x * 2654435761u) >> 20)) % NT;
  const int item = uni((int)(blockIdx.x / (unsigned)a.F));
  const int f = uni((int)(blockIdx.x - (unsigned)item * (unsigned)a.F));
  const long long gw = (long long)item * a.F + f;
  if (w == 0) {
    const int l = lane_id();
    s_orig[l] = l;
    if (l == 0) *s_flag = 0;
  }
  const int p = a.p, P2 = (p + 1) >> 1;
  const double* arx = a.arx + ((size_t)item * NT + w) * (size_t)(16 * 64 * 2) * P2;
  const double* tw = a.tw + (size_t)f * p * 2;
  const double tau = a.tau;
  const unsigned ldsbase = (unsigned)(uintptr_t)lds;
  double acc[32];
#ifdef HMV_STAMP
  unsigned long long tsum[8] = {0, 0, 0, 0, 0, 0, 0, 0}, tlast = 0, q0, q1, q2, q3;
  unsigned tl32;
  K3A_BODY_STAMPED(acc, arx, tw, p, w, tau, ldsbase, q0, q1, q2, q3, tl32);
  {
    const unsigned long long d[8] = {q0 & 0xffffffffull, q0 >> 32, q1 & 0xffffffffull, q1 >> 32,
                                     q2 & 0xffffffffull, q2 >> 32, q3 & 0xffffffffull, q3 >> 32};
    tsum[0] = d[0]; tsum[2] = d[1]; tsum[3] = d[2] + d[3] + d[4]; tsum[1] = d[5] + d[6] + d[7];
    unsigned long long now;
    asm volatile("s_memtime %0\n\ts_waitcnt lgkmcnt(0)" : "=s"(now)::"memory");
    tlast = (now & ~0xffffffffull) | tl32;
    if (tlast > now) tlast -= 0x100000000ull;
    if (a.stamps && lane_id() == 0) {
      unsigned long long* det = a.stamps + ((size_t)a.n_items * a.F * NT + (size_t)(gw * NT + wv)) * 8;
      for (int k = 0; k < 8; ++k) det[k] = d[k];
    }
  }
#else
  K3A_BODY(acc, arx, tw, p, w, tau, ldsbase);
#endif
  double re[NT][4], im[NT][4];
#pragma unroll
  for (int Ig = 0; Ig < 4; ++Ig)
#pragma unroll
    for (int Jl = 0; Jl < 4; ++Jl) {
      re[Ig][Jl] = acc[2 * (4 * Ig + Jl)];
      im[Ig][Jl] = acc[2 * (4 * Ig + Jl) + 1];
    }
  double2* smem = reinterpret_cast<double2*>(lds);
  double* rsum = reinterpret_cast<double*>(lds + K3A_RSUM);
  tf_outputs<NT, false>(a, item, f, gw, w, wv, re, im, smem, rsum, s_orig, s_flag, nullptr
#ifdef HMV_STAMP
                        , tsum, tlast
#endif
  );
}

template <int NT>
__global__ void __launch_bounds__(256) ar_pack_kernel(const double* ar, double* arx, long long n_items, int p) {
  constexpr int MP = 16 * NT;
  const int P2 = (p + 1) >> 1;
  const long long per_item = (long long)MP * MP * P2;
  const long long idx = (long long)blockIdx.x * 256 + threadIdx.x;
  if (idx >= n_items * per_item) return;
  const long long item = idx / per_item;
  long long r = idx - item * per_item;
  const int lane = (int)(r & 63); r >>= 6;
  const int h = (int)(r % P2); r /= P2;
  const int Jl = (int)(r & 3); r >>= 2;
  const int Ig = (int)(r % NT);
  const int w = (int)(r / NT);
  const int row = 16 * Ig + 4 * ((lane >> 2) & 3) + (lane >> 4), col = 4 * (Jl * NT + w) + (lane & 3);
  const double* e = ar + ((size_t)item * MP * MP + (size_t)row * MP + col) * p;
  double2 v;
  v.x = e[2 * h];
  v.y = (2 * h + 1 < p) ? e[2 * h + 1] : 0.0;
  reinterpret_cast<double2*>(arx)[idx] = v;
}

__global__ void twiddle_kernel(const double* freqs, int F, double fs, int p, double* tw) {
  const int idx = blockIdx.x * blockDim.x + threadIdx.x;
  if (idx >= F * p) return;
  const int f = idx / p, k = idx - f * p;
  const double c = (double)(-(k + 1) * 2) * 3.141592653589793;
  const double th = c * freqs[f] / fs;
  double s, co;
  sincos(th, &s, &co);
  tw[2 * idx] = co;
  tw[2 * idx + 1] = s;
}

int launch_twiddles(const double* freqs, int F, double fs, int p, double* tw, hipStream_t st) {
  const int n = F * p;
  hipLaunchKernelGGL(twiddle_kernel, dim3((n + 255) / 256), dim3(256), 0, st, freqs, F, fs, p, tw);
  return (int)hipGetLastError();
}

int tf_band_max_F(int m_pad) {
  switch (m_pad) {
    case 16: return (2 * TfLds<1>::TOTAL) & ~31;
    case 32: return (2 * TfLds<2>::TOTAL) & ~31;
    case 48: return (2 * TfLds<3>::TOTAL) & ~31;
    case 64: return (2 * TfLds<4>::TOTAL) & ~31;
  }
  return 0;
}

long long tf_workspace_doubles(long long n_items, int m_pad, int p) {
  return n_items * (long long)m_pad * m_pad * 2 * ((p + 1) / 2);
}

int launch_tf_inv(const TfArgs& a_in, int m_pad, hipStream_t st, hipEvent_t ev_start, hipEvent_t ev_stop) {
  TfArgs a = a_in;
  if (a.n_items == 0 || a.F == 0) return 0;
  const bool fused = ((a.ff != nullptr || a.bands != nullptr) && a.fuse_items > 0);
  if (fused) {
    if (!a.P || !a.den || !a.wcount || !a.ready || !a.missed || a.lag < 1) return -3;
    if (a.bands && (!a.band_lo || !a.band_hi || a.nb < 1 || a.F % 32 != 0 || a.F > tf_band_max_F(m_pad) || a.A)) return -3;
    if (const hipError_t e = hipMemsetAsync(a.wcount, 0, sizeof(int) * (2 * (size_t)a.n_items + 1), st)) return (int)e;
  } else {
    a.ff = nullptr;
    a.bands = nullptr;
  }
  const long long n = a.n_items * (long long)a.F;
  const dim3 grid((unsigned)n);
  const long long slots = a.n_items * (long long)m_pad * m_pad * ((a.p + 1) / 2);
  const dim3 pgrid((unsigned)((slots + 255) / 256));
  double* arx = const_cast<double*>(a.arx);
  switch (m_pad) {
    case 16: hipLaunchKernelGGL(ar_pack_kernel<1>, pgrid, dim3(256), 0, st, a.ar, arx, a.n_items, a.p); break;
    case 32: hipLaunchKernelGGL(ar_pack_kernel<2>, pgrid, dim3(256), 0, st, a.ar, arx, a.n_items, a.p); break;
    case 48: hipLaunchKernelGGL(ar_pack_kernel<3>, pgrid, dim3(256), 0, st, a.ar, arx, a.n_items, a.p); break;
    case 64: hipLaunchKernelGGL(ar_pack_kernel<4>, pgrid, dim3(256), 0, st, a.ar, arx, a.n_items, a.p); break;
    default: return -1;
  }
  if (ev_start)
    if (const hipError_t e = hipEventRecord(ev_start, st)) return (int)e;
  switch (m_pad) {
    case 16: hipLaunchKernelGGL((tf_inv_kernel<1, false>), grid, dim3(64), 0, st, a); break;
    case 32: hipLaunchKernelGGL((tf_inv_kernel<2, false>), grid, dim3(128), 0, st, a); break;
    case 48: hipLaunchKernelGGL((tf_inv_kernel<3, false>), grid, dim3(192), 0, st, a); break;
    case 64:
      if (tuning(5) > 0) {
        (void)hipFuncSetAttribute(reinterpret_cast<const void*>(&tf_inv64_asm_kernel), hipFuncAttributeMaxDynamicSharedMemorySize,
                                  (int)tuning(5));
        (void)hipFuncSetAttribute(reinterpret_cast<const void*>(&tf_inv_kernel<4, false>),
                                  hipFuncAttributeMaxDynamicSharedMemorySize, (int)tuning(5));
      }
      if ((tuning(3 ) != 1 || a.bands != nullptr) && a.A == nullptr)
        hipLaunchKernelGGL(tf_inv64_asm_kernel, grid, dim3(256), (unsigned)tuning(5 ), st, a);
      else
        hipLaunchKernelGGL((tf_inv_kernel<4, false>), grid, dim3(256), (unsigned)tuning(5), st, a);
      break;
  }
  if (ev_stop)
    if (const hipError_t e = hipEventRecord(ev_stop, st)) return (int)e;
  if (fused) {
    const long long tail_rows = (a.fuse_items > a.lag ? a.lag : a.fuse_items) * a.m;
    const dim3 mgrid((unsigned)(tail_rows > 2048 ? 2048 : (tail_rows < 256 ? 256 : tail_rows)));
    switch (m_pad) {
      case 16: hipLaunchKernelGGL(norm_missed_kernel<1>, mgrid, dim3(64), 0, st, a); break;
      case 32: hipLaunchKernelGGL(norm_missed_kernel<2>, mgrid, dim3(128), 0, st, a); break;
      case 48: hipLaunchKernelGGL(norm_missed_kernel<3>, mgrid, dim3(192), 0, st, a); break;
      case 64: hipLaunchKernelGGL(norm_missed_kernel<4>, mgrid, dim3(256), 0, st, a); break;
    }
  }
  return (int)hipGetLastError();
}

int launch_cinv(const TfArgs& a_in, int m_pad, hipStream_t st) {
  TfArgs a = a_in;
  a.ff = nullptr;
  a.bands = nullptr;
  a.fuse_items = 0;
  const long long n = a.n_items * (long long)a.F;
  if (n == 0) return 0;
  const dim3 grid((unsigned)n);
  switch (m_pad) {
    case 16: hipLaunchKernelGGL((tf_inv_kernel<1, true>), grid, dim3(64), 0, st, a); break;
    case 32: hipLaunchKernelGGL((tf_inv_kernel<2, true>), grid, dim3(128), 0, st, a); break;
    case 48: hipLaunchKernelGGL((tf_inv_kernel<3, true>), grid, dim3(192), 0, st, a); break;
    case 64: hipLaunchKernelGGL((tf_inv_kernel<4, true>), grid, dim3(256), 0, st, a); break;
    default: return -1;
  }
  return (int)hipGetLastError();
}

}
```

### hyperscanning_signal_analysis_amd/csrc/yw_auto.hip

```cpp
#include "yw_lwr_core.h"

namespace hmv {

template <int NT>
__global__ void __launch_bounds__(256, 3) yw_auto_kernel(YwArgs a, YwAutoArgs sel) {
  yw_lwr_body<NT, true, true>(a, sel);
}

int launch_yw_auto(const YwArgs& a_in, const YwAutoArgs& sel, int m_pad, hipStream_t st) {
  YwArgs a = a_in;
  if (a.n_items == 0) return 0;
  a.order = nullptr;
  a.only_guarded = 0;
  const dim3 grid((unsigned)a.n_items), block(256);
  switch (m_pad) {
    case 16: hipLaunchKernelGGL((yw_auto_kernel<1>), grid, block, 0, st, a, sel); break;
    case 32: hipLaunchKernelGGL((yw_auto_kernel<2>), grid, block, 0, st, a, sel); break;
    case 48: hipLaunchKernelGGL((yw_auto_kernel<3>), grid, block, 0, st, a, sel); break;
    case 64: hipLaunchKernelGGL((yw_auto_kernel<4>), grid, block, 0, st, a, sel); break;
    default: return -1;
  }
  if (const int rc = (int)hipGetLastError()) return rc;
  a.order = sel.order_out;
  return launch_yw_guarded(a, m_pad, st);
}

}
```

### hyperscanning_signal_analysis_amd/csrc/yw_common.h

```cpp
#pragma once
#include "hmv_common.h"
#include "hmv_kernels.h"

namespace hmv {

typedef double f64x2 __attribute__((ext_vector_type(2)));

#define HMV_WAVE_SYNC()                                     \
  do {                                                      \
    __builtin_amdgcn_fence(__ATOMIC_RELEASE, "wavefront");  \
    __builtin_amdgcn_wave_barrier();                        \
    __builtin_amdgcn_fence(__ATOMIC_ACQUIRE, "wavefront");  \
  } while (0)

__host__ __device__ inline long long yw_tri(int a, int b) { return (long long)a * (a + 1) / 2 + b; }
__host__ __device__ inline long long yw_ws_tiles_d(int p) {
  const long long a = 2 * yw_tri(p + 1, 0) + 2 * (long long)p, b = 4 * (long long)p + 6;
  return (a > b ? a : b) + 1;
}
__host__ __device__ inline int* yw_guard_ptr(double* ws, long long item, int p, int tile) {
  return reinterpret_cast<int*>(ws + (size_t)(item + 1) * yw_ws_tiles_d(p) * tile) - 1;
}

template <int NT>
struct YwCfg {
  static constexpr int MP = 16 * NT;
  static constexpr int S = (MP <= 38) ? 38 : 70;
};

template <int NT, int S>
__device__ __forceinline__ void spd_inverse_coop(const double* Xs, double* Pb, double* Nb2, int* s_info,
                                                 double* s_ld, double* dinv_out, double* logdet_out, int info_base,
                                                 double* pm = nullptr) {
  constexpr int MP = 16 * NT, NI = 4 * NT, NSTEP = MP / 4;
  const int l = lane_id();
  const int w = uni(threadIdx.x >> 6);
  const int i = l >> 4, cc = l & 15;
  const bool active = (w < NT);
  double m[NI];
  if (active) {
#pragma unroll
    for (int I = 0; I < NI; ++I) m[I] = Xs[(4 * I + i) * S + 16 * w + cc];
  }
  double mypiv = 1.0;
  double pmin = 1.7976931348623157e308, pmax = 0.0;
  static_for<NSTEP>([&](auto sc) __attribute__((always_inline)) {
    constexpr int s = decltype(sc)::value;
    constexpr int ws = s >> 2, q = s & 3;
    double* Nb = Nb2 + (s & 1) * MP * 4;
    if (w == ws) {
      if ((cc >> 2) == q) {
#pragma unroll
        for (int I = 0; I < NI; ++I) Pb[(4 * I + i) * 4 + (cc & 3)] = m[I];
      }
      HMV_WAVE_SYNC();
      double x[4];
      {
        const int r = (l < MP) ? l : 0;
#pragma unroll
        for (int jj = 0; jj < 4; ++jj) x[jj] = Pb[r * 4 + jj];
      }
#pragma unroll
      for (int jj = 0; jj < 4; ++jj) {
        const int col = 4 * s + jj;
        const double piv = readlane_f64(x[jj], col);
        if (!(piv > 0.0) && l == 0 && *s_info == 0) *s_info = info_base + col + 1;
        mypiv = (l == col) ? piv : mypiv;
        pmin = fmin(pmin, piv);
        pmax = fmax(pmax, piv);
        double inv = __builtin_amdgcn_rcp(piv);
        inv = __builtin_fma(__builtin_fma(-piv, inv, 1.0), inv, inv);
        inv = __builtin_fma(__builtin_fma(-piv, inv, 1.0), inv, inv);
        double qv[4];
#pragma unroll
        for (int j2 = 0; j2 < 4; ++j2) qv[j2] = (j2 == jj) ? inv : readlane_f64(x[j2], col) * inv;
        const double f = x[jj];
        const bool isp = (l == col);
#pragma unroll
        for (int j2 = 0; j2 < 4; ++j2) {
          const double base = (j2 == jj) ? 0.0 : x[j2];
          const double nr = __builtin_fma(-f, qv[j2], base);
          x[j2] = isp ? qv[j2] : nr;
        }
      }
      if (l < MP) {
#pragma unroll
        for (int jj = 0; jj < 4; ++jj) Nb[l * 4 + jj] = x[jj];
      }
    }
    __syncthreads();
    if (active) {
      const double u = m[s];
#pragma unroll
      for (int I = 0; I < NI; ++I) {
        double nv = Nb[(4 * I + (l & 3)) * 4 + (l >> 4)];
        if (I == s) nv -= ((l & 3) == (l >> 4)) ? 1.0 : 0.0;
        m[I] = mfma4(nv, u, m[I]);
      }
      if (w == ws && (cc >> 2) == q) {
#pragma unroll
        for (int I = 0; I < NI; ++I) m[I] = Nb[(4 * I + i) * 4 + (cc & 3)];
      }
    }
  });
  if (dinv_out && active) {
#pragma unroll
    for (int I = 0; I < NI; ++I) dinv_out[(size_t)(4 * I + i) * MP + 16 * w + cc] = m[I];
  }
  if (logdet_out) {
    double v = row16_sum_dpp(log(mypiv));
    v = readlane_f64(v, 0) + readlane_f64(v, 16) + readlane_f64(v, 32) + readlane_f64(v, 48);
    if (l == 0) s_ld[w] = v;
    __syncthreads();
    if (threadIdx.x == 0) *logdet_out = ((s_ld[0] + s_ld[1]) + s_ld[2]) + s_ld[3];
  }
  if (pm) {
    __syncthreads();
    if (l == 0 && w < NT) {
      pm[2 + 2 * w] = pmin;
      pm[3 + 2 * w] = pmax;
    }
    __syncthreads();
    if (threadIdx.x == 0) {
      double a = pm[2], b = pm[3];
      for (int k = 1; k < NT; ++k) {
        a = fmin(a, pm[2 + 2 * k]);
        b = fmax(b, pm[3 + 2 * k]);
      }
      pm[0] = a;
      pm[1] = b;
    }
    __syncthreads();
  }
}

template <int NT, int S>
__device__ __forceinline__ void spd_inverse_coop2(const double (&ga)[NT][NT], const double (&gb)[NT][NT], double* img,
                                                  double* Pb2, double* Nb4, int* s_info, double* s_ld, double* out_a,
                                                  double* out_b, double* logdet_b, int info_base, double* pm) {
  constexpr int MP = 16 * NT, NI = 4 * NT, NSTEP = MP / 4, ROT = NT / 2;
  const int l = lane_id();
  const int w = uni(threadIdx.x >> 6);
  const int i = l >> 4, cc = l & 15;
  const bool active = (w < NT);
  const int wB = active ? (w + ROT) % NT : 0;
  double ma[NI], mb[NI];
  __syncthreads();
#pragma unroll
  for (int ii = 0; ii < NT; ++ii)
#pragma unroll
    for (int J = 0; J < NT; ++J) img[(4 * (w * NT + ii) + i) * S + 16 * J + cc] = ga[ii][J];
  __syncthreads();
  if (active) {
#pragma unroll
    for (int I = 0; I < NI; ++I) ma[I] = img[(4 * I + i) * S + 16 * w + cc];
  }
  __syncthreads();
#pragma unroll
  for (int ii = 0; ii < NT; ++ii)
#pragma unroll
    for (int J = 0; J < NT; ++J) img[(4 * (w * NT + ii) + i) * S + 16 * J + cc] = gb[ii][J];
  __syncthreads();
  if (active) {
#pragma unroll
    for (int I = 0; I < NI; ++I) mb[I] = img[(4 * I + i) * S + 16 * wB + cc];
  }
  double mypiv_b = 1.0;
  double pmin_a = 1.7976931348623157e308, pmax_a = 0.0, pmin_b = 1.7976931348623157e308, pmax_b = 0.0;
  auto factor = [&](double (&m)[NI], auto sc, double* Pb, double* Nb, double& pmin, double& pmax, double* mypiv)
                    __attribute__((always_inline)) {
    constexpr int s = decltype(sc)::value, q = s & 3;
    if ((cc >> 2) == q) {
#pragma unroll
      for (int I = 0; I < NI; ++I) Pb[(4 * I + i) * 4 + (cc & 3)] = m[I];
    }
    HMV_WAVE_SYNC();
    double x[4];
    {
      const int r = (l < MP) ? l : 0;
#pragma unroll
      for (int jj = 0; jj < 4; ++jj) x[jj] = Pb[r * 4 + jj];
    }
#pragma unroll
    for (int jj = 0; jj < 4; ++jj) {
      const int col = 4 * s + jj;
      const double piv = readlane_f64(x[jj], col);
      if (!(piv > 0.0) && l == 0 && *s_info == 0) *s_info = info_base + col + 1;
      if (mypiv) *mypiv = (l == col) ? piv : *mypiv;
      pmin = fmin(pmin, piv);
      pmax = fmax(pmax, piv);
      double inv = __builtin_amdgcn_rcp(piv);
      inv = __builtin_fma(__builtin_fma(-piv, inv, 1.0), inv, inv);
      inv = __builtin_fma(__builtin_fma(-piv, inv, 1.0), inv, inv);
      double qv[4];
#pragma unroll
      for (int j2 = 0; j2 < 4; ++j2) qv[j2] = (j2 == jj) ? inv : readlane_f64(x[j2], col) * inv;
      const double f = x[jj];
      const bool isp = (l == col);
#pragma unroll
      for (int j2 = 0; j2 < 4; ++j2) {
        const double base = (j2 == jj) ? 0.0 : x[j2];
        const double nr = __builtin_fma(-f, qv[j2], base);
        x[j2] = isp ? qv[j2] : nr;
      }
    }
    if (l < MP) {
#pragma unroll
      for (int jj = 0; jj < 4; ++jj) Nb[l * 4 + jj] = x[jj];
    }
  };
  auto update = [&](double (&m)[NI], auto sc, const double* Nb, bool owner) __attribute__((always_inline)) {
    constexpr int s = decltype(sc)::value, q = s & 3;
    const double u = m[s];
#pragma unroll
    for (int I = 0; I < NI; ++I) {
      double nv = Nb[(4 * I + (l & 3)) * 4 + (l >> 4)];
      if (I == s) nv -= ((l & 3) == (l >> 4)) ? 1.0 : 0.0;
      m[I] = mfma4(nv, u, m[I]);
    }
    if (owner && (cc >> 2) == q) {
#pragma unroll
      for (int I = 0; I < NI; ++I) m[I] = Nb[(4 * I + i) * 4 + (cc & 3)];
    }
  };
  static_for<NSTEP>([&](auto sc) __attribute__((always_inline)) {
    constexpr int s = decltype(sc)::value;
    constexpr int wa = s >> 2, wb = ((s >> 2) - ROT + NT) % NT;
    double* NbA = Nb4 + (s & 1) * MP * 4;
    double* NbB = Nb4 + (2 + (s & 1)) * MP * 4;
    if (w == wa) factor(ma, sc, Pb2, NbA, pmin_a, pmax_a, nullptr);
    if (w == wb) factor(mb, sc, Pb2 + MP * 4, NbB, pmin_b, pmax_b, &mypiv_b);
    __syncthreads();
    if (active) {
      update(ma, sc, NbA, w == wa);
      update(mb, sc, NbB, w == wb);
    }
  });
  if (active) {
#pragma unroll
    for (int I = 0; I < NI; ++I) {
      out_a[(size_t)(4 * I + i) * MP + 16 * w + cc] = ma[I];
      out_b[(size_t)(4 * I + i) * MP + 16 * wB + cc] = mb[I];
    }
  }
  if (logdet_b) {
    double v = row16_sum_dpp(log(mypiv_b));
    v = readlane_f64(v, 0) + readlane_f64(v, 16) + readlane_f64(v, 32) + readlane_f64(v, 48);
    if (l == 0 && active) s_ld[wB] = v;
    if (l == 0 && !active) s_ld[w] = 0.0;
    __syncthreads();
    if (threadIdx.x == 0) *logdet_b = ((s_ld[0] + s_ld[1]) + s_ld[2]) + s_ld[3];
  }
  __syncthreads();
  if (l == 0 && w < NT) {
    pm[4 + 4 * w] = pmin_a;
    pm[5 + 4 * w] = pmax_a;
    pm[6 + 4 * w] = pmin_b;
    pm[7 + 4 * w] = pmax_b;
  }
  __syncthreads();
  if (threadIdx.x == 0) {
    double a0 = pm[4], a1 = pm[5], b0 = pm[6], b1 = pm[7];
    for (int k = 1; k < NT; ++k) {
      a0 = fmin(a0, pm[4 + 4 * k]);
      a1 = fmax(a1, pm[5 + 4 * k]);
      b0 = fmin(b0, pm[6 + 4 * k]);
      b1 = fmax(b1, pm[7 + 4 * k]);
    }
    pm[0] = a0;
    pm[1] = a1;
    pm[2] = b0;
    pm[3] = b1;
  }
  __syncthreads();
}

}
```

### hyperscanning_signal_analysis_amd/csrc/yw_lwr.hip

```cpp
#include "yw_lwr_core.h"

namespace hmv {

template <int NT, bool VQ>
__global__ void __launch_bounds__(256, 3) yw_lwr_kernel(YwArgs a) {
  yw_lwr_body<NT, VQ, false>(a, YwAutoArgs{});
}

int launch_yw_lwr(const YwArgs& a, int m_pad, hipStream_t st) {
  if (a.n_items == 0) return 0;
  if (tuning(4 ) == 3) return launch_yw_lwr2(a, m_pad, st);
  const dim3 grid((unsigned)a.n_items), block(256);
  const bool vq = (a.Vq_logdet != nullptr);
  switch (m_pad) {
    case 16: if (vq) hipLaunchKernelGGL((yw_lwr_kernel<1, true>), grid, block, 0, st, a);
             else hipLaunchKernelGGL((yw_lwr_kernel<1, false>), grid, block, 0, st, a); break;
    case 32: if (vq) hipLaunchKernelGGL((yw_lwr_kernel<2, true>), grid, block, 0, st, a);
             else hipLaunchKernelGGL((yw_lwr_kernel<2, false>), grid, block, 0, st, a); break;
    case 48: if (vq) hipLaunchKernelGGL((yw_lwr_kernel<3, true>), grid, block, 0, st, a);
             else hipLaunchKernelGGL((yw_lwr_kernel<3, false>), grid, block, 0, st, a); break;
    case 64: if (vq) hipLaunchKernelGGL((yw_lwr_kernel<4, true>), grid, block, 0, st, a);
             else hipLaunchKernelGGL((yw_lwr_kernel<4, false>), grid, block, 0, st, a); break;
    default: return -1;
  }
  return (int)hipGetLastError();
}

}
```

### hyperscanning_signal_analysis_amd/csrc/yw_lwr_core.h

```cpp
#pragma once
#include "yw_common.h"

namespace hmv {

#ifndef HMV_LWR_GUARD
#define HMV_LWR_GUARD 1e-7
#endif

template <int NT, bool VQ, bool AUTO>
__device__ __forceinline__ void yw_lwr_body(const YwArgs& a, const YwAutoArgs& sel) {
  static_assert(VQ || !AUTO, "the selecting form needs every log det Vf_q");
  constexpr int MP = 16 * NT, KH = MP / 2, SH = KH + 6, NIW = NT, NJ = NT, TILE = MP * MP;
  constexpr int NV = (MP * KH / 2 + 255) / 256;
  constexpr int SI = YwCfg<NT>::S;
  constexpr int GEMM_D = 2 * MP * SH, INV_D = MP * SI, BUF_D = GEMM_D > INV_D ? GEMM_D : INV_D;
  __shared__ __attribute__((aligned(16))) double buf[BUF_D];
  __shared__ double Pb[2 * MP * 4];
  __shared__ double Nb[4 * MP * 4];
  __shared__ int s_info;
  __shared__ double s_ld[4];
  __shared__ double s_pm[4 + 4 * 4];
  __shared__ int s_guard;
  __shared__ double s_logdet, s_best;
  __shared__ int s_qstar, s_take;
  double* Xh = buf;
  double* Yh = buf + MP * SH;
  const int wv = uni(threadIdx.x >> 6);
  const int p = a.p;
  const long long item = blockIdx.x;
  double* ws = a.ws + (size_t)item * yw_ws_tiles_d(p) * TILE;
  double* Agen[2] = {ws, ws + (size_t)p * TILE};
  double* Bgen[2] = {ws + (size_t)2 * p * TILE, ws + (size_t)3 * p * TILE};
  double* Vf = ws + (size_t)4 * p * TILE;
  double* Vb = Vf + TILE;
  double* VfI = Vb + TILE;
  double* VbI = VfI + TILE;
  double* Dq = VbI + TILE;
  const double* R = a.R + (size_t)item * (p + 1) * TILE;
  if (threadIdx.x == 0) {
    s_info = 0;
    s_guard = 0;
    if (AUTO) {
      s_best = __builtin_inf();
      s_qstar = 0;
    }
  }

  auto lane = [&]() __attribute__((always_inline)) {
    int lo;
    asm volatile("v_mbcnt_lo_u32_b32 %0, -1, 0\n\tv_mbcnt_hi_u32_b32 %0, -1, %0" : "=v"(lo));
    return lo;
  };
  auto zero = [&](double (&v)[NIW][NJ]) __attribute__((always_inline)) {
#pragma unroll
    for (int ii = 0; ii < NIW; ++ii)
#pragma unroll
      for (int J = 0; J < NJ; ++J) v[ii][J] = 0.0;
  };
  auto fetch = [&](f64x2 (&v)[NV], const double* src, int kh, bool tr) __attribute__((always_inline)) {
    const int t0 = lane() + 64 * wv;
#pragma unroll
    for (int r = 0; r < NV; ++r) {
      const int idx = t0 + 256 * r;
      if (NV * 256 == MP * KH / 2 || idx < MP * KH / 2) {
        if (!tr) {
          const int row = idx / (KH / 2), c2 = idx - row * (KH / 2);
          v[r] = *reinterpret_cast<const f64x2*>(src + (size_t)row * MP + kh * KH + 2 * c2);
        } else {
          const int k = idx / (MP / 2), c2 = idx - k * (MP / 2);
          v[r] = *reinterpret_cast<const f64x2*>(src + (size_t)(kh * KH + k) * MP + 2 * c2);
        }
      }
    }
  };
  auto park = [&](double* dst, const f64x2 (&v)[NV], bool tr) __attribute__((always_inline)) {
    const int t0 = lane() + 64 * wv;
#pragma unroll
    for (int r = 0; r < NV; ++r) {
      const int idx = t0 + 256 * r;
      if (NV * 256 == MP * KH / 2 || idx < MP * KH / 2) {
        if (!tr) {
          const int row = idx / (KH / 2), c2 = idx - row * (KH / 2);
          double* d = dst + row * SH + 2 * c2;
          d[0] = v[r].x;
          d[1] = v[r].y;
        } else {
          const int k = idx / (MP / 2), c2 = idx - k * (MP / 2);
          dst[(2 * c2) * SH + k] = v[r].x;
          dst[(2 * c2 + 1) * SH + k] = v[r].y;
        }
      }
    }
  };
  auto park_strip = [&](const double (&v)[NIW][NJ], int kh) __attribute__((always_inline)) {
    const int l = lane(), i = l >> 4, cc = l & 15;
#pragma unroll
    for (int ii = 0; ii < NIW; ++ii)
#pragma unroll
      for (int J = 0; J < NJ; ++J) {
        const int col = 16 * J + cc - kh * KH;
        if (col >= 0 && col < KH) Xh[(4 * (wv * NT + ii) + i) * SH + col] = v[ii][J];
      }
  };
#ifndef HMV_LWR_GEMM_PIPE
#define HMV_LWR_GEMM_PIPE 1
#endif
  auto gemm_half = [&](double (&acc)[NIW][NJ]) __attribute__((always_inline)) {
    const int l = lane();
    const double* xa = Xh + (4 * wv * NT + (l & 3)) * SH + (l >> 4);
    const double* yb = Yh + (l & 15) * SH + (l >> 4);
#if HMV_LWR_GEMM_PIPE
    constexpr int NS = KH / 4;
    double av[2][NIW], bv[2][NJ];
    auto rd = [&](int set, int k0) __attribute__((always_inline)) {
#pragma unroll
      for (int ii = 0; ii < NIW; ++ii) av[set][ii] = xa[4 * ii * SH + k0];
#pragma unroll
      for (int J = 0; J < NJ; ++J) bv[set][J] = yb[16 * J * SH + k0];
    };
    rd(0, 0);
    static_for<NS>([&](auto sc) __attribute__((always_inline)) {
      constexpr int s = decltype(sc)::value, cur = s & 1;
      if constexpr (s + 1 < NS) rd(cur ^ 1, 4 * (s + 1));
      __builtin_amdgcn_sched_barrier(0);
#pragma unroll
      for (int ii = 0; ii < NIW; ++ii)
#pragma unroll
        for (int J = 0; J < NJ; ++J) acc[ii][J] = mfma4(av[cur][ii], bv[cur][J], acc[ii][J]);
      __builtin_amdgcn_sched_barrier(0);
    });
#else
#pragma unroll 2
    for (int k0 = 0; k0 < KH; k0 += 4) {
      double av[NIW], bv[NJ];
#pragma unroll
      for (int ii = 0; ii < NIW; ++ii) av[ii] = xa[4 * ii * SH + k0];
#pragma unroll
      for (int J = 0; J < NJ; ++J) bv[J] = yb[16 * J * SH + k0];
#pragma unroll
      for (int ii = 0; ii < NIW; ++ii)
#pragma unroll
        for (int J = 0; J < NJ; ++J) acc[ii][J] = mfma4(av[ii], bv[J], acc[ii][J]);
    }
#endif
  };
  auto product = [&](double (&acc)[NIW][NJ], const double* srcX, bool trX, const double (&xr)[NIW][NJ], const double* srcY,
                     bool trY) __attribute__((always_inline)) {
    f64x2 vx[NV], vy[NV];
    if (srcX) fetch(vx, srcX, 0, trX);
    fetch(vy, srcY, 0, trY);
    __syncthreads();
    if (srcX) park(Xh, vx, trX); else park_strip(xr, 0);
    park(Yh, vy, trY);
    if (srcX) fetch(vx, srcX, 1, trX);
    fetch(vy, srcY, 1, trY);
    __syncthreads();
    gemm_half(acc);
    __syncthreads();
    if (srcX) park(Xh, vx, trX); else park_strip(xr, 1);
    park(Yh, vy, trY);
    __syncthreads();
    gemm_half(acc);
  };
  auto store_tile = [&](double* dst, const double (&v)[NIW][NJ]) __attribute__((always_inline)) {
    const int l = lane(), i = l >> 4, cc = l & 15;
#pragma unroll
    for (int ii = 0; ii < NIW; ++ii)
#pragma unroll
      for (int J = 0; J < NJ; ++J) dst[(size_t)(4 * (wv * NT + ii) + i) * MP + 16 * J + cc] = v[ii][J];
  };
  auto load_tile = [&](double (&v)[NIW][NJ], const double* src, bool tr) __attribute__((always_inline)) {
    const int l = lane(), i = l >> 4, cc = l & 15;
#pragma unroll
    for (int ii = 0; ii < NIW; ++ii)
#pragma unroll
      for (int J = 0; J < NJ; ++J) {
        const int row = 4 * (wv * NT + ii) + i, col = 16 * J + cc;
        v[ii][J] = tr ? src[(size_t)col * MP + row] : src[(size_t)row * MP + col];
      }
  };
  auto sub = [&](double (&g)[NIW][NJ], const double (&acc)[NIW][NJ]) __attribute__((always_inline)) {
#pragma unroll
    for (int ii = 0; ii < NIW; ++ii)
#pragma unroll
      for (int J = 0; J < NJ; ++J) g[ii][J] -= acc[ii][J];
  };
  auto invert = [&](const double (&g)[NIW][NJ], double* out, double* logdet, int q) __attribute__((always_inline)) {
    const int info_base = q * MP;
    const int l = lane(), i = l >> 4, cc = l & 15;
    __syncthreads();
#pragma unroll
    for (int ii = 0; ii < NIW; ++ii)
#pragma unroll
      for (int J = 0; J < NJ; ++J) buf[(4 * (wv * NT + ii) + i) * SI + 16 * J + cc] = g[ii][J];
    __syncthreads();
    spd_inverse_coop<NT, SI>(buf, Pb, Nb, &s_info, s_ld, out, logdet, info_base, s_pm);
    if (threadIdx.x == 0 && !(s_pm[0] >= HMV_LWR_GUARD * s_pm[1])) {
      if (!AUTO) s_guard = 1;
      else if (s_guard == 0) s_guard = q + 1;
    }
    __syncthreads();
  };

  auto invert2 = [&](const double (&ga)[NIW][NJ], const double (&gb)[NIW][NJ], double* out_a, double* out_b, double* logdet_b,
                     int q) __attribute__((always_inline)) {
    const int info_base = q * MP;
    spd_inverse_coop2<NT, SI>(ga, gb, buf, Pb, Nb, &s_info, s_ld, out_a, out_b, logdet_b, info_base, s_pm);
    if (threadIdx.x == 0 && (!(s_pm[0] >= HMV_LWR_GUARD * s_pm[1]) || !(s_pm[2] >= HMV_LWR_GUARD * s_pm[3]))) {
      if (!AUTO) s_guard = 1;
      else if (s_guard == 0) s_guard = q + 1;
    }
    __syncthreads();
  };

  auto ld_dst = [&](int q) __attribute__((always_inline)) -> double* {
    if (AUTO) return &s_logdet;
    return a.Vq_logdet + (size_t)item * p + (q - 1);
  };
  auto select = [&](int q) __attribute__((always_inline)) {
    if (threadIdx.x == 0) {
      const double ld = s_logdet;
      const double crit = ld + ((sel.crit_c * (double)q) * (double)(a.m * a.m)) / (double)sel.n;
      if (sel.crit_out) sel.crit_out[(size_t)item * p + (q - 1)] = crit;
      if (a.Vq_logdet) a.Vq_logdet[(size_t)item * p + (q - 1)] = ld;
      const int take = (crit < s_best) ? 1 : 0;
      if (take) {
        s_best = crit;
        s_qstar = q;
      }
      s_take = take;
    }
    __syncthreads();
    if (s_take) {
      const double* Aq = Agen[q & 1];
      double* ar = a.ar + (size_t)item * TILE * p;
      const int total = TILE * q;
      for (int idx = threadIdx.x; idx < total; idx += 256) {
        const int e = idx / q, k = idx - e * q;
        ar[(size_t)e * p + k] = Aq[(size_t)k * TILE + e];
      }
      double* Vo = a.V + (size_t)item * TILE;
      for (int idx = threadIdx.x; idx < TILE; idx += 256) Vo[idx] = Vf[idx];
    }
  };

  double g[NIW][NJ], acc[NIW][NJ], dacc[NIW][NJ];
  const double (&none)[NIW][NJ] = g;
  load_tile(g, R, false);
  store_tile(Vf, g);
  store_tile(Vb, g);
  load_tile(g, R + TILE, true);
  store_tile(Dq, g);
  __syncthreads();
  for (int q = 0; q < p; ++q) {
    const double* Ao = Agen[q & 1];
    const double* Bo = Bgen[q & 1];
    double* An = Agen[(q + 1) & 1];
    double* Bn = Bgen[(q + 1) & 1];
    const bool last = (q == p - 1);
    load_tile(g, Vb, false);
#ifndef HMV_LWR_SINGLE_INVERSES
    if (!last || (VQ && q >= 1)) {
      load_tile(acc, Vf, false);
      invert2(g, acc, VbI, VfI, (VQ && q >= 1) ? ld_dst(q) : nullptr, q);
    } else {
      invert(g, VbI, nullptr, q);
    }
#else
    invert(g, VbI, nullptr, q);
    if (!last || (VQ && q >= 1)) {
      load_tile(g, Vf, false);
      invert(g, VfI, (VQ && q >= 1) ? ld_dst(q) : nullptr, q);
    }
#endif
    if (AUTO && q >= 1) select(q);
    zero(acc);
    product(acc, Dq, false, none, VbI, false);
    store_tile(An + (size_t)q * TILE, acc);
    zero(dacc);
    product(dacc, nullptr, false, acc, Dq, false);
    load_tile(g, Vf, false);
    sub(g, dacc);
    store_tile(Vf, g);
    if (!last) {
      zero(acc);
      product(acc, Dq, true, none, VfI, false);
      store_tile(Bn + (size_t)q * TILE, acc);
      zero(dacc);
      product(dacc, nullptr, false, acc, Dq, true);
      load_tile(g, Vb, false);
      sub(g, dacc);
      store_tile(Vb, g);
    }
    __syncthreads();
    zero(dacc);
    for (int k = 0; k < q; ++k) {
      zero(acc);
      product(acc, An + (size_t)q * TILE, false, none, Bo + (size_t)(q - 1 - k) * TILE, true);
      load_tile(g, Ao + (size_t)k * TILE, false);
      sub(g, acc);
      store_tile(An + (size_t)k * TILE, g);
      if (!last) {
        product(dacc, nullptr, false, g, R + (size_t)(q + 1 - k) * TILE, false);
        zero(acc);
        product(acc, Bn + (size_t)q * TILE, false, none, Ao + (size_t)(q - 1 - k) * TILE, true);
        load_tile(g, Bo + (size_t)k * TILE, false);
        sub(g, acc);
        store_tile(Bn + (size_t)k * TILE, g);
      }
    }
    if (!last) {
      product(dacc, An + (size_t)q * TILE, false, none, R + TILE, false);
      load_tile(g, R + (size_t)(q + 2) * TILE, true);
      sub(g, dacc);
      store_tile(Dq, g);
    }
    __syncthreads();
  }
  if (VQ) {
    load_tile(g, Vf, false);
    invert(g, VfI, ld_dst(p), p);
  }
  if (AUTO) {
    select(p);
    __syncthreads();
    const int bad = s_info, qs = bad ? 0 : s_qstar;
    if (threadIdx.x == 0) {
      a.info[item] = bad ? bad : (qs == 0 ? -1 : 0);
      sel.order_out[item] = qs;
      *yw_guard_ptr(a.ws, item, p, TILE) = (bad == 0 && qs > 0 && s_guard != 0 && s_guard - 1 <= qs) ? 1 : 0;
    }
    double* ar = a.ar + (size_t)item * TILE * p;
    const int total = TILE * p;
    for (int idx = threadIdx.x; idx < total; idx += 256) {
      const int e = idx / p, k = idx - e * p;
      if (k >= qs) ar[idx] = 0.0;
    }
    if (qs == 0) {
      double* Vo = a.V + (size_t)item * TILE;
      for (int idx = threadIdx.x; idx < TILE; idx += 256) Vo[idx] = R[idx];
    }
    return;
  }
  load_tile(g, Vf, false);
  store_tile(a.V + (size_t)item * TILE, g);
  if (threadIdx.x == 0) {
    a.info[item] = s_info;
    *yw_guard_ptr(a.ws, item, p, TILE) = (s_info == 0) ? s_guard : 0;
  }
  const double* Af = Agen[p & 1];
  double* ar = a.ar + (size_t)item * TILE * p;
  const int total = TILE * p;
  for (int idx = threadIdx.x; idx < total; idx += 256) {
    const int e = idx / p, k = idx - e * p;
    ar[idx] = Af[(size_t)k * TILE + e];
  }
}

}
```

### hyperscanning_signal_analysis_amd/csrc/yw_solve.hip

```cpp
#include "yw_common.h"
#include <cstdlib>

namespace hmv {

long long yw_ws_tiles(int p) { return yw_ws_tiles_d(p); }

struct YwPtrs {
  const double* R;
  double *Yt, *Lt, *Dinv, *Zt;
};
template <int MP>
__device__ __forceinline__ YwPtrs yw_ptrs(const YwArgs& a, long long item, int p) {
  constexpr int TILE = MP * MP;
  double* ws = a.ws + (size_t)item * yw_ws_tiles_d(a.p) * TILE;
  const long long ntri = yw_tri(p + 1, 0);
  YwPtrs q;
  q.R = a.R + (size_t)item * (a.p + 1) * TILE;
  q.Yt = ws;
  q.Lt = ws + ntri * TILE;
  q.Dinv = ws + 2 * ntri * TILE;
  q.Zt = q.Dinv + (size_t)p * TILE;
  return q;
}

template <int NT>
struct YwWin {
  static constexpr int MP = 16 * NT, KH = MP / 2, SH = KH + 6, NIW = NT, NJ = NT, TILE = MP * MP;
  static constexpr int NV = (MP * KH / 2 + 255) / 256;
  static constexpr int SI = YwCfg<NT>::S;
  static constexpr int GEMM_D = 2 * MP * SH, INV_D = MP * SI;
  static constexpr int BUF_D = GEMM_D > INV_D ? GEMM_D : INV_D;
};

template <int NT, bool VQ, int MODE = 0>
__global__ void __launch_bounds__(256, VQ ? 2 : (MODE == 2 ? 4 : 3)) yw_window_kernel(YwArgs a, int tb_arg) {
  constexpr bool BACK_ONLY = (MODE == 1);
  using W = YwWin<NT>;
  constexpr int MP = W::MP, KH = W::KH, SH = W::SH, NIW = NT, NJ = NT, TILE = W::TILE, NV = W::NV;
  constexpr bool PACKED = (MODE == 2) && !VQ && (MP * MP + 12 * MP <= W::BUF_D);
  constexpr int SI = PACKED ? MP : W::SI;
  __shared__ __attribute__((aligned(16))) double buf[W::BUF_D];
  __shared__ double Pb_[PACKED ? 1 : MP * 4];
  __shared__ double Nb_[PACKED ? 1 : 2 * MP * 4];
  double* Pb = PACKED ? buf + MP * MP : Pb_;
  double* Nb = PACKED ? buf + MP * MP + 4 * MP : Nb_;
  __shared__ int s_info;
  __shared__ double s_ld[4];
  double* Xh = buf;
  double* Yh = buf + MP * SH;
  const int wv = uni(threadIdx.x >> 6);
  int p = a.p;
  long long item = blockIdx.x;
  int ta_col = 0;
  if (MODE == 2) {
    const unsigned ntile = (unsigned)(p - tb_arg + 1);
    const unsigned grp = blockIdx.x / (8u * ntile), r = blockIdx.x - grp * (8u * ntile);
    item = (long long)grp * 8 + (r & 7u);
    if (item >= a.n_items) return;
    ta_col = tb_arg + (int)(r >> 3);
  }
  if (MODE == 0 && a.only_guarded) {
    if (*yw_guard_ptr(a.ws, item, p, TILE) == 0) return;
  }
  if (MODE == 0 && a.order) p = uni(a.order[item]);
  const YwPtrs q = yw_ptrs<MP>(a, item, p);
  if (threadIdx.x == 0) s_info = 0;

  auto lane = [&]() __attribute__((always_inline)) {
    int lo;
    asm volatile("v_mbcnt_lo_u32_b32 %0, -1, 0\n\tv_mbcnt_hi_u32_b32 %0, -1, %0" : "=v"(lo));
    return lo;
  };
  auto zero = [&](double (&v)[NIW][NJ]) __attribute__((always_inline)) {
#pragma unroll
    for (int ii = 0; ii < NIW; ++ii)
#pragma unroll
      for (int J = 0; J < NJ; ++J) v[ii][J] = 0.0;
  };
  auto fetch = [&](f64x2 (&v)[NV], const double* src, int kh, bool tr) __attribute__((always_inline)) {
    const int t0 = lane() + 64 * wv;
#pragma unroll
    for (int r = 0; r < NV; ++r) {
      const int idx = t0 + 256 * r;
      if (NV * 256 == MP * KH / 2 || idx < MP * KH / 2) {
        if (!tr) {
          const int row = idx / (KH / 2), c2 = idx - row * (KH / 2);
          v[r] = *reinterpret_cast<const f64x2*>(src + (size_t)row * MP + kh * KH + 2 * c2);
        } else {
          const int k = idx / (MP / 2), c2 = idx - k * (MP / 2);
          v[r] = *reinterpret_cast<const f64x2*>(src + (size_t)(kh * KH + k) * MP + 2 * c2);
        }
      }
    }
  };
  auto park = [&](double* dst, const f64x2 (&v)[NV], bool tr) __attribute__((always_inline)) {
    const int t0 = lane() + 64 * wv;
#pragma unroll
    for (int r = 0; r < NV; ++r) {
      const int idx = t0 + 256 * r;
      if (NV * 256 == MP * KH / 2 || idx < MP * KH / 2) {
        if (!tr) {
          const int row = idx / (KH / 2), c2 = idx - row * (KH / 2);
          double* d = dst + row * SH + 2 * c2;
          d[0] = v[r].x;
          d[1] = v[r].y;
        } else {
          const int k = idx / (MP / 2), c2 = idx - k * (MP / 2);
          dst[(2 * c2) * SH + k] = v[r].x;
          dst[(2 * c2 + 1) * SH + k] = v[r].y;
        }
      }
    }
  };
  auto park_strip = [&](const double (&v)[NIW][NJ], int kh) __attribute__((always_inline)) {
    const int l = lane(), i = l >> 4, cc = l & 15;
#pragma unroll
    for (int ii = 0; ii < NIW; ++ii)
#pragma unroll
      for (int J = 0; J < NJ; ++J) {
        const int col = 16 * J + cc - kh * KH;
        if (col >= 0 && col < KH) Xh[(4 * (wv * NT + ii) + i) * SH + col] = v[ii][J];
      }
  };
  auto gemm_half = [&](double (&acc)[NIW][NJ]) __attribute__((always_inline)) {
    const int l = lane();
    const double* xa = Xh + (4 * wv * NT + (l & 3)) * SH + (l >> 4);
    const double* yb = Yh + (l & 15) * SH + (l >> 4);
#pragma unroll 2
    for (int k0 = 0; k0 < KH; k0 += 4) {
      double av[NIW], bv[NJ];
#pragma unroll
      for (int ii = 0; ii < NIW; ++ii) av[ii] = xa[4 * ii * SH + k0];
#pragma unroll
      for (int J = 0; J < NJ; ++J) bv[J] = yb[16 * J * SH + k0];
#pragma unroll
      for (int ii = 0; ii < NIW; ++ii)
#pragma unroll
        for (int J = 0; J < NJ; ++J) acc[ii][J] = mfma4(av[ii], bv[J], acc[ii][J]);
    }
  };
  auto product = [&](double (&acc)[NIW][NJ], const double* srcX, const double (&xr)[NIW][NJ], const double* srcY,
                     bool trY) __attribute__((always_inline)) {
    f64x2 vx[NV], vy[NV];
    if (srcX) fetch(vx, srcX, 0, false);
    fetch(vy, srcY, 0, trY);
    __syncthreads();
    if (srcX) park(Xh, vx, false); else park_strip(xr, 0);
    park(Yh, vy, trY);
    if (srcX) fetch(vx, srcX, 1, false);
    fetch(vy, srcY, 1, trY);
    __syncthreads();
    gemm_half(acc);
    __syncthreads();
    if (srcX) park(Xh, vx, false); else park_strip(xr, 1);
    park(Yh, vy, trY);
    __syncthreads();
    gemm_half(acc);
  };
  auto load_G = [&](double (&g)[NIW][NJ], int ta, int tb) __attribute__((always_inline)) {
    const int l = lane(), i = l >> 4, cc = l & 15;
    const bool tr = !(ta < p) && (tb < p);
    const double* src = q.R + (size_t)((ta < p) ? (ta - tb) : (tb < p ? tb + 1 : 0)) * TILE;
#pragma unroll
    for (int ii = 0; ii < NIW; ++ii)
#pragma unroll
      for (int J = 0; J < NJ; ++J) {
        const int row = 4 * (wv * NT + ii) + i, col = 16 * J + cc;
        g[ii][J] = tr ? src[col * MP + row] : src[row * MP + col];
      }
  };
  auto store_tile = [&](double* dst, const double (&v)[NIW][NJ]) __attribute__((always_inline)) {
    const int l = lane(), i = l >> 4, cc = l & 15;
#pragma unroll
    for (int ii = 0; ii < NIW; ++ii)
#pragma unroll
      for (int J = 0; J < NJ; ++J) dst[(size_t)(4 * (wv * NT + ii) + i) * MP + 16 * J + cc] = v[ii][J];
  };
  auto load_tile = [&](double (&v)[NIW][NJ], const double* src) __attribute__((always_inline)) {
    const int l = lane(), i = l >> 4, cc = l & 15;
#pragma unroll
    for (int ii = 0; ii < NIW; ++ii)
#pragma unroll
      for (int J = 0; J < NJ; ++J) v[ii][J] = src[(size_t)(4 * (wv * NT + ii) + i) * MP + 16 * J + cc];
  };
  auto tile_to_lds = [&](const double (&v)[NIW][NJ]) __attribute__((always_inline)) {
    const int l = lane(), i = l >> 4, cc = l & 15;
    __syncthreads();
#pragma unroll
    for (int ii = 0; ii < NIW; ++ii)
#pragma unroll
      for (int J = 0; J < NJ; ++J) buf[(4 * (wv * NT + ii) + i) * SI + 16 * J + cc] = v[ii][J];
    __syncthreads();
  };

  double g[NIW][NJ], acc[NIW][NJ];
  const double (&none)[NIW][NJ] = g;
  if (MODE == 2) {
    const int tb = tb_arg, ta = ta_col;
    if (tb > 0) {
      load_tile(g, q.Yt + yw_tri(ta, tb - 1) * TILE);
      zero(acc);
      product(acc, nullptr, g, q.Dinv + (size_t)(tb - 1) * TILE, true);
      store_tile(q.Lt + yw_tri(ta, tb - 1) * TILE, acc);
      if (ta == p) store_tile(q.Zt + (size_t)(tb - 1) * TILE, acc);
      __syncthreads();
    }
    load_G(g, ta, tb);
    zero(acc);
    for (int c = 0; c < tb; ++c) {
      product(acc, q.Lt + yw_tri(ta, c) * TILE, none, q.Yt + yw_tri(tb, c) * TILE, false);
      if (VQ && ta == p && tb == p) {
        double vq[NIW][NJ];
#pragma unroll
        for (int ii = 0; ii < NIW; ++ii)
#pragma unroll
          for (int J = 0; J < NJ; ++J) vq[ii][J] = g[ii][J] - acc[ii][J];
        tile_to_lds(vq);
        spd_inverse_coop<NT, SI>(buf, Pb, Nb, &s_info, s_ld, nullptr, a.Vq_logdet + (size_t)item * p + c, tb * MP);
      }
    }
#pragma unroll
    for (int ii = 0; ii < NIW; ++ii)
#pragma unroll
      for (int J = 0; J < NJ; ++J) g[ii][J] -= acc[ii][J];
    if (ta != tb) {
      store_tile(q.Yt + yw_tri(ta, tb) * TILE, g);
    } else if (tb == p) {
      store_tile(a.V + (size_t)item * TILE, g);
    } else {
      tile_to_lds(g);
      spd_inverse_coop<NT, SI>(buf, Pb, Nb, &s_info, s_ld, q.Dinv + (size_t)tb * TILE, nullptr, tb * MP);
      __syncthreads();
      if (threadIdx.x == 0 && s_info != 0) atomicCAS(&a.info[item], 0, s_info);
    }
    return;
  }
  for (int tb = 0; tb <= (BACK_ONLY ? -1 : p); ++tb) {
    load_G(g, tb, tb);
    zero(acc);
    for (int c = 0; c < tb; ++c) {
      product(acc, q.Lt + yw_tri(tb, c) * TILE, none, q.Yt + yw_tri(tb, c) * TILE, false);
      if (VQ && tb == p) {
        double vq[NIW][NJ];
#pragma unroll
        for (int ii = 0; ii < NIW; ++ii)
#pragma unroll
          for (int J = 0; J < NJ; ++J) vq[ii][J] = g[ii][J] - acc[ii][J];
        tile_to_lds(vq);
        spd_inverse_coop<NT, SI>(buf, Pb, Nb, &s_info, s_ld, nullptr, a.Vq_logdet + (size_t)item * p + c, tb * MP);
      }
    }
#pragma unroll
    for (int ii = 0; ii < NIW; ++ii)
#pragma unroll
      for (int J = 0; J < NJ; ++J) g[ii][J] -= acc[ii][J];
    if (tb == p) {
      store_tile(a.V + (size_t)item * TILE, g);
      break;
    }
    tile_to_lds(g);
    spd_inverse_coop<NT, SI>(buf, Pb, Nb, &s_info, s_ld, q.Dinv + (size_t)tb * TILE, nullptr, tb * MP);
    __syncthreads();
    for (int ta = tb + 1; ta <= p; ++ta) {
      load_G(g, ta, tb);
      zero(acc);
      for (int c = 0; c < tb; ++c)
        product(acc, q.Lt + yw_tri(ta, c) * TILE, none, q.Yt + yw_tri(tb, c) * TILE, false);
#pragma unroll
      for (int ii = 0; ii < NIW; ++ii)
#pragma unroll
        for (int J = 0; J < NJ; ++J) g[ii][J] -= acc[ii][J];
      store_tile(q.Yt + yw_tri(ta, tb) * TILE, g);
      zero(acc);
      product(acc, nullptr, g, q.Dinv + (size_t)tb * TILE, true);
      store_tile(q.Lt + yw_tri(ta, tb) * TILE, acc);
      if (ta == p) store_tile(q.Zt + (size_t)tb * TILE, acc);
    }
    __syncthreads();
  }
  if (!BACK_ONLY && threadIdx.x == 0 && s_info != 0) a.info[item] = s_info;
  __syncthreads();
  for (int b = p - 2; b >= 0; --b) {
    load_tile(g, q.Zt + (size_t)b * TILE);
    for (int c = p - 1; c > b; --c) {
      zero(acc);
      product(acc, q.Zt + (size_t)c * TILE, none, q.Lt + yw_tri(c, b) * TILE, true);
#pragma unroll
      for (int ii = 0; ii < NIW; ++ii)
#pragma unroll
        for (int J = 0; J < NJ; ++J) g[ii][J] -= acc[ii][J];
    }
    store_tile(q.Zt + (size_t)b * TILE, g);
    __syncthreads();
  }
  const int pa = a.p;
  double* ar = a.ar + (size_t)item * TILE * pa;
  const int total = TILE * pa;
  for (int idx = threadIdx.x; idx < total; idx += 256) {
    const int e = idx / pa, k = idx - e * pa;
    ar[idx] = (k < p) ? q.Zt[(size_t)k * TILE + e] : 0.0;
  }
}

template <int NT>
static int launch_yw_nt(const YwArgs& a, hipStream_t st) {
  const int p = a.p;
  const unsigned n = (unsigned)a.n_items;
  if (const hipError_t e = hipMemsetAsync(a.info, 0, sizeof(int) * a.n_items, st)) return (int)e;
  for (int tb = 0; tb <= p; ++tb) {
    const dim3 grid(((n + 7) / 8) * 8 * (unsigned)(p - tb + 1));
    if (a.Vq_logdet && tb == p) hipLaunchKernelGGL((yw_window_kernel<NT, true, 2>), grid, dim3(256), 0, st, a, tb);
    else hipLaunchKernelGGL((yw_window_kernel<NT, false, 2>), grid, dim3(256), 0, st, a, tb);
  }
  hipLaunchKernelGGL((yw_window_kernel<NT, false, 1>), dim3(n), dim3(256), 0, st, a, 0);
  return (int)hipGetLastError();
}

int launch_yw_guarded(const YwArgs& a_in, int m_pad, hipStream_t st) {
  YwArgs a = a_in;
  a.only_guarded = 1;
  a.tiled = 0;
  a.Vq_logdet = nullptr;
  if (a.n_items == 0) return 0;
  const dim3 grid((unsigned)a.n_items), block(256);
  switch (m_pad) {
    case 16: hipLaunchKernelGGL((yw_window_kernel<1, false>), grid, block, 0, st, a, 0); break;
    case 32: hipLaunchKernelGGL((yw_window_kernel<2, false>), grid, block, 0, st, a, 0); break;
    case 48: hipLaunchKernelGGL((yw_window_kernel<3, false>), grid, block, 0, st, a, 0); break;
    case 64: hipLaunchKernelGGL((yw_window_kernel<4, false>), grid, block, 0, st, a, 0); break;
    default: return -1;
  }
  return (int)hipGetLastError();
}

int launch_yw(const YwArgs& a_in, int m_pad, hipStream_t st) {
  YwArgs a = a_in;
  a.only_guarded = 0;
  a.order = nullptr;
  if (a.n_items == 0) return 0;
  const long long form = tuning(4 );
  if (a.tiled < 0 && form != 1) {
    int rc = launch_yw_lwr(a, m_pad, st);
    if (rc) return rc;
    a.only_guarded = 1;
    a.tiled = 0;
  }
  const bool one_launch = a.tiled == 0 || (a.tiled < 0 && !(m_pad == 64 && a.n_items >= 128));
  if (one_launch) {
    if (!a.only_guarded)
      if (const hipError_t e = hipMemsetAsync(a.info, 0, sizeof(int) * a.n_items, st)) return (int)e;
    const dim3 grid((unsigned)a.n_items), block(256);
    const bool vq = (a.Vq_logdet != nullptr);
    switch (m_pad) {
      case 16: if (vq) hipLaunchKernelGGL((yw_window_kernel<1, true>), grid, block, 0, st, a, 0);
               else hipLaunchKernelGGL((yw_window_kernel<1, false>), grid, block, 0, st, a, 0); break;
      case 32: if (vq) hipLaunchKernelGGL((yw_window_kernel<2, true>), grid, block, 0, st, a, 0);
               else hipLaunchKernelGGL((yw_window_kernel<2, false>), grid, block, 0, st, a, 0); break;
      case 48: if (vq) hipLaunchKernelGGL((yw_window_kernel<3, true>), grid, block, 0, st, a, 0);
               else hipLaunchKernelGGL((yw_window_kernel<3, false>), grid, block, 0, st, a, 0); break;
      case 64: if (vq) hipLaunchKernelGGL((yw_window_kernel<4, true>), grid, block, 0, st, a, 0);
               else hipLaunchKernelGGL((yw_window_kernel<4, false>), grid, block, 0, st, a, 0); break;
      default: return -1;
    }
    return (int)hipGetLastError();
  }
  if (a.order) return -1;
  switch (m_pad) {
    case 16: return launch_yw_nt<1>(a, st);
    case 32: return launch_yw_nt<2>(a, st);
    case 48: return launch_yw_nt<3>(a, st);
    case 64: return launch_yw_nt<4>(a, st);
    default: return -1;
  }
}

}
```

### include/hypermvar.h

```cpp
#ifndef HYPERMVAR_H
#define HYPERMVAR_H

#include <stdint.h>

#ifdef __cplusplus
extern "C" {
#endif

#define HMV_VERSION 160
#define HMV_MAX_CHANNELS 64
#define HMV_MAX_ORDER 32

int hmv_version(void);
const char* hmv_last_error(void);
int hmv_pad(int m);
#define HMV_TUNE_NORM_LAG 1
#define HMV_TUNE_LAG_GROUP 2
#define HMV_TUNE_K3_FORM 3
#define HMV_TUNE_YW_FORM 4
#define HMV_TUNE_K3_LDS_PAD 5
int hmv_set_tuning(int key, int64_t value);
int64_t hmv_get_tuning(int key);
int64_t hmv_yw_workspace_doubles(int m, int p);

int hmv_lagcov_f64(const double* x, int64_t rec_stride, int64_t ld,
                   const int64_t* item_rec, const int64_t* item_start, int64_t n_items,
                   int m, int n, int p, double* R, void* stream);

#define HMV_MAX_HOPS_PER_WINDOW 8
int64_t hmv_lagcov_regular_workspace_doubles(int64_t n_win, int m, int n, int64_t hop, int p);
int hmv_lagcov_regular_f64(const double* x, int64_t ld, int64_t T, int64_t first, int64_t hop, int64_t n_win,
                           int m, int n, int p, double* R, double* workspace, void* stream);

int hmv_yw_solve_f64(const double* R, int64_t n_items, int m, int p, double* ws,
                     double* ar, double* V, double* vq_logdet, int32_t* info, int64_t flags, void* stream);

int hmv_twiddles_f64(const double* freqs, int F, double fs, int p, double* tw, void* stream);

int64_t hmv_tf_workspace_doubles(int64_t n_items, int m, int p);
int hmv_tf_f64(const double* ar, int64_t n_items, int m, int p, const double* tw, int F,
               double* P, double* rowsum, double* H, double* A, int32_t* info,
               double pivot_tau, double* ws, void* stream);

int hmv_ffdtf_norm_f64(const double* P, const double* rowsum, double* den, double* out,
                       int64_t n_items, int F, int m, int normalise, void* stream);

int hmv_transpose_c128(const double* in, double* out, int64_t n_items, int F, int m, void* stream);

int hmv_spectra_f64(const double* H, const double* V, double* S, int64_t n_items, int m, int F, void* stream);
int hmv_spectra_mmf_f64(const double* H, const double* V, double* S, int64_t n_items, int m, int F, void* stream);

int hmv_pack_c128(const double* in, double* out, int64_t n_items, int F, int m, void* stream);
int hmv_cinv_c128(const double* Z, int64_t n_items, int m, int F, double* Zinv, double* detph, int32_t* info,
                  double pivot_tau, void* stream);
int hmv_partial_coherence_c128(const double* Sinv, const double* detph, double* kappa, int64_t n_items, int m,
                               int F, void* stream);
int hmv_gpdc_f64(const double* A, const double* V, double* G, int64_t n_items, int m, int F, void* stream);

int hmv_trial_mean_f64(const double* R_trials, int64_t n_trials, int m, int p, double* R_mean, void* stream);
int hmv_ddtf_f64(const double* ffdtf, const double* kappa, double* ddtf, int64_t n_items, int m, int F, void* stream);
int hmv_band_sums_f64(const double* ffdtf, int64_t n_rows, int F, const int32_t* bin_lo, const int32_t* bin_hi,
                      int n_bands, double* out, void* stream);

int64_t hmv_dpss_workspace_bytes(int64_t n_times, int k_max, int sym);
int hmv_dpss_f64(int64_t n_times, double half_nbw, int k_max, int sym, double* tapers, double* ratios,
                 void* workspace, int64_t workspace_bytes, void* stream);
int64_t hmv_psd_workspace_bytes(int64_t ch_chunk, int64_t n_times, int n_tapers);
int hmv_psd_multitaper_f64(const double* x, int64_t n_ch, int64_t n_times, int64_t ld, const double* tapers,
                           const double* weights, int n_tapers, int64_t bin_lo, int64_t bin_hi, double* psd,
                           void* workspace, int64_t workspace_bytes, int64_t ch_chunk, void* stream);

#define HMV_FLAG_UNFUSED_NORM 1
#define HMV_FLAG_DIRECT_LAGCOV 8
#define HMV_FLAG_YW_TILED 2
#define HMV_FLAG_YW_ONE_LAUNCH 4

int64_t hmv_tf_ffdtf_workspace_bytes(int64_t n_items, int m, int p, int F);
int hmv_tf_ffdtf_f64(const double* ar, int64_t n_items, int m, int p, const double* tw, int F,
                     double* ffdtf, double* den, double* H, int32_t* info, double pivot_tau,
                     void* workspace, int64_t workspace_bytes, int64_t flags,
                     void* ev_k3_start, void* ev_k3_stop, void* stream);

int64_t hmv_tf_ffdtf_bands_workspace_bytes(int64_t n_items, int m, int p, int F);
int hmv_tf_ffdtf_bands_f64(const double* ar, int64_t n_items, int m, int p, const double* tw, int F,
                           double* band_out, const int32_t* bin_lo, const int32_t* bin_hi, int n_bands,
                           double* den, int32_t* info, double pivot_tau,
                           void* workspace, int64_t workspace_bytes, int64_t flags,
                           void* ev_k3_start, void* ev_k3_stop, void* stream);

int64_t hmv_sliding_workspace_bytes(int64_t chunk, int m, int p, int F);
int hmv_sliding_ffdtf_f64(const double* x, int64_t rec_stride, int64_t ld,
                          const int64_t* item_rec, const int64_t* item_start, int64_t n_items,
                          int m, int n, int p, const double* freqs, int F, double fs,
                          double* ffdtf, double* ar_out, double* V_out,
                          int32_t* info_yw, int32_t* info_tf,
                          void* workspace, int64_t workspace_bytes, int64_t chunk,
                          double pivot_tau, int64_t flags,
                          int64_t grid_hop, int64_t grid_first, int64_t grid_nwin, int64_t grid_T,
                          void* ev_k3_start, void* ev_k3_stop, void* stream, void* aux_stream);

int64_t hmv_sliding_bands_workspace_bytes(int64_t chunk, int m, int p, int F);
int hmv_sliding_ffdtf_bands_f64(const double* x, int64_t rec_stride, int64_t ld,
                                const int64_t* item_rec, const int64_t* item_start, int64_t n_items,
                                int m, int n, int p, const double* freqs, int F, double fs,
                                double* band_out, const int32_t* bin_lo, const int32_t* bin_hi, int n_bands,
                                double* ar_out, double* V_out,
                                int32_t* info_yw, int32_t* info_tf,
                                void* workspace, int64_t workspace_bytes, int64_t chunk,
                                double pivot_tau, int64_t flags,
                                int64_t grid_hop, int64_t grid_first, int64_t grid_nwin, int64_t grid_T,
                                void* ev_k3_start, void* ev_k3_stop, void* stream, void* aux_stream);

int64_t hmv_sliding_spectra_workspace_bytes(int64_t chunk, int m, int p, int F);
int hmv_sliding_ffdtf_spectra_f64(const double* x, int64_t rec_stride, int64_t ld,
                                  const int64_t* item_rec, const int64_t* item_start, int64_t n_items,
                                  int m, int n, int p, const double* freqs, int F, double fs,
                                  double* ffdtf, double* S_out, double* ar_out, double* V_out,
                                  int32_t* info_yw, int32_t* info_tf,
                                  void* workspace, int64_t workspace_bytes, int64_t chunk,
                                  double pivot_tau, int64_t flags,
                                  int64_t grid_hop, int64_t grid_first, int64_t grid_nwin, int64_t grid_T,
                                  void* stream, void* aux_stream);

int64_t hmv_sliding_ddtf_workspace_bytes(int64_t chunk, int m, int p, int F, int n_bands);
int hmv_sliding_ddtf_f64(const double* x, int64_t rec_stride, int64_t ld,
                         const int64_t* item_rec, const int64_t* item_start, int64_t n_items,
                         int m, int n, int p, const double* freqs, int F, double fs,
                         double* out, const int32_t* bin_lo, const int32_t* bin_hi, int n_bands,
                         double* ar_out, double* V_out, int32_t* info_yw, int32_t* info_tf,
                         void* workspace, int64_t workspace_bytes, int64_t chunk,
                         double pivot_tau, int64_t flags,
                         int64_t grid_hop, int64_t grid_first, int64_t grid_nwin, int64_t grid_T,
                         void* stream, void* aux_stream);
int64_t hmv_sliding_gpdc_workspace_bytes(int64_t chunk, int m, int p, int F, int n_bands);
int hmv_sliding_gpdc_f64(const double* x, int64_t rec_stride, int64_t ld,
                         const int64_t* item_rec, const int64_t* item_start, int64_t n_items,
                         int m, int n, int p, const double* freqs, int F, double fs,
                         double* out, const int32_t* bin_lo, const int32_t* bin_hi, int n_bands,
                         double* ar_out, double* V_out, int32_t* info_yw,
                         void* workspace, int64_t workspace_bytes, int64_t chunk, int64_t flags,
                         int64_t grid_hop, int64_t grid_first, int64_t grid_nwin, int64_t grid_T,
                         void* stream, void* aux_stream);

#define HMV_MEASURE_FFDTF 0
#define HMV_MEASURE_DDTF 1
#define HMV_MEASURE_GPDC 2
int hmv_yw_solve_auto_f64(const double* R, int64_t n_items, int m, int pmax, int n, int crit, double* ws, double* ar,
                          double* V, int32_t* order_out, double* crit_out, double* vq_logdet, int32_t* info,
                          int64_t flags, void* stream);
int64_t hmv_sliding_auto_workspace_bytes(int measure, int64_t chunk, int m, int pmax, int F, int n_bands);
int hmv_sliding_auto_f64(int measure, const double* x, int64_t rec_stride, int64_t ld,
                         const int64_t* item_rec, const int64_t* item_start, int64_t n_items,
                         int m, int n, int pmax, int crit, const double* freqs, int F, double fs,
                         double* out, const int32_t* bin_lo, const int32_t* bin_hi, int n_bands, double* S_out,
                         double* ar_out, double* V_out, int32_t* order_out, double* crit_out,
                         int32_t* info_yw, int32_t* info_tf, void* workspace, int64_t workspace_bytes, int64_t chunk,
                         double pivot_tau, int64_t flags,
                         int64_t grid_hop, int64_t grid_first, int64_t grid_nwin, int64_t grid_T,
                         void* stream, void* aux_stream);

#define HMV_MAX_HOPS_ENSEMBLE 32
int64_t hmv_lagcov_ensemble_workspace_doubles(int64_t n_items, int m, int n, int p, int64_t grid_hop, int64_t grid_nwin);
int hmv_lagcov_ensemble_f64(const double* x, int64_t rec_stride, int64_t ld, int64_t T,
                            const int64_t* trial_rec, const int64_t* trial_start, const int64_t* group_ptr,
                            int64_t n_groups, const int64_t* item_group, const int64_t* item_offset, int64_t n_items,
                            int m, int n, int p, double* R, double* workspace, int64_t workspace_doubles,
                            int64_t grid_hop, int64_t grid_nwin, int64_t flags, void* stream);
int64_t hmv_sliding_ensemble_workspace_bytes(int measure, int64_t chunk, int m, int n, int p, int F, int n_bands,
                                             int64_t grid_hop, int64_t grid_nwin);
int hmv_sliding_ensemble_f64(int measure, const double* x, int64_t rec_stride, int64_t ld, int64_t T,
                             const int64_t* trial_rec, const int64_t* trial_start, const int64_t* group_ptr,
                             int64_t n_groups, const int64_t* item_group, const int64_t* item_offset, int64_t n_items,
                             int m, int n, int p, const double* freqs, int F, double fs,
                             double* out, const int32_t* bin_lo, const int32_t* bin_hi, int n_bands, double* S_out,
                             double* ar_out, double* V_out, int32_t* info_yw, int32_t* info_tf,
                             void* workspace, int64_t workspace_bytes, int64_t chunk, double pivot_tau, int64_t flags,
                             int64_t grid_hop, int64_t grid_nwin, void* stream, void* aux_stream);

int64_t hmv_fad_workspace_bytes(int64_t n_series, int pmax);
int hmv_fad_f64(const double* x, int64_t rec_stride, int64_t ld, const int64_t* item_rec, const int64_t* item_start,
                int64_t n_items, int m, int n, int pmax, int order, int crit, double fs, double imag_tol,
                int pair_conjugates, int32_t* order_out, double* crit_out, double* ar, double* noise_variance,
                double* poles, double* C, double* alpha, double* freq, double* beta, double* bandwidth, double* phi,
                double* B, uint8_t* osc_mask, int32_t* paired, int32_t* n_paired, int32_t* info, void* stream);
int hmv_fad_decompose_f64(const double* ar, int64_t n_series, int p, double fs, double imag_tol, int pair_conjugates,
                          double* poles, double* C, double* alpha, double* freq, double* beta, double* bandwidth,
                          double* phi, double* B, uint8_t* osc_mask, int32_t* paired, int32_t* n_paired, int32_t* info,
                          void* stream);

int hmv_surrogate_shift_f64(const double* x, int64_t rec_stride, int64_t ld, int64_t T, const int64_t* item_rec,
                            const int64_t* item_start, int64_t n_win, const int64_t* shift, int64_t n_rec, int n_surr, int m,
                            int n, int split, double* out, void* stream);
int hmv_surrogate_phase_c128(const double* spec, int64_t n_win, const double* phi, int n_surr, int m, int n, double* out,
                             void* stream);
int hmv_null_accumulate_f64(const double* observed, const double* surr, const uint8_t* surr_bad, const uint8_t* tested,
                            int64_t n_win, int n_surr, int m, int n_bands, double* M, int32_t* n_valid, int32_t* count,
                            int32_t* count_fwe, int32_t* n_cell, double* mean, double* m2, double* p, double* p_fwe,
                            double* null_mean, double* null_std, void* stream);

#ifdef __cplusplus
}
#endif
#endif
```

Measured before the change: 57250 windows/s.

## Fold lag-cov finish, AR packing, K3 prep and twiddles into YW solve kernel

When the new STEP_GLUE knob is at its default, the step pipeline stops running separate glue launches. The hop-block sums are finished into per-window covariances inside the Levinson-Whittle kernel, using edge samples staged in LDS. That kernel also writes the packed AR layout for the transfer-function kernel directly, resets the normalisation counters and computes the twiddles. This drops the regular lagcov finish, ar_pack, memset and twiddle launches, and skips writing unused AR outputs. The cost is more work and LDS traffic inside the YW kernel, and a tail that now depends on block 0 producing the twiddles before K3 runs. It also adds a small LDS bank-skew tweak in the lagcov finish kernel.

```diff
diff --git a/hyperscanning_signal_analysis_amd/_lib.py b/hyperscanning_signal_analysis_amd/_lib.py
--- a/hyperscanning_signal_analysis_amd/_lib.py
+++ b/hyperscanning_signal_analysis_amd/_lib.py
@@ -113,6 +113,7 @@
 TUNE_K3_FORM = 3
 TUNE_YW_FORM = 4
 TUNE_K3_LDS_PAD = 5
+TUNE_STEP_GLUE = 6
 
 
 _lib = None
diff --git a/hyperscanning_signal_analysis_amd/csrc/capi.hip b/hyperscanning_signal_analysis_amd/csrc/capi.hip
--- a/hyperscanning_signal_analysis_amd/csrc/capi.hip
+++ b/hyperscanning_signal_analysis_amd/csrc/capi.hip
@@ -18,9 +18,9 @@
 inline hipStream_t S(void* s) { return reinterpret_cast<hipStream_t>(s); }
 inline size_t align256(size_t b) { return (b + 255) & ~size_t(255); }
 
-constexpr int N_TUNE = 6;
+constexpr int N_TUNE = 7;
 struct TuneRange { long long lo, hi; };
-constexpr TuneRange kTuneRange[N_TUNE] = {{0, 0}, {0, 1 << 20}, {0, 3}, {0, 2}, {0, 3}, {0, 140000}};
+constexpr TuneRange kTuneRange[N_TUNE] = {{0, 0}, {0, 1 << 20}, {0, 3}, {0, 2}, {0, 3}, {0, 140000}, {0, 1}};
 long long env_knob(const char* name, int key) {
   const char* e = getenv(name);
   if (!e || !*e) return 0;
@@ -35,7 +35,7 @@
 }
 std::atomic<long long> g_tune[N_TUNE] = {{0}, {env_knob("HYPERMVAR_NORM_LAG", 1)}, {env_knob("HYPERMVAR_LAG_GROUP", 2)},
                                          {env_knob("HYPERMVAR_K3_FORM", 3)}, {env_knob("HYPERMVAR_YW_FORM", 4)},
-                                         {env_knob("HYPERMVAR_K3_LDS_PAD", 5)}};
+                                         {env_knob("HYPERMVAR_K3_LDS_PAD", 5)}, {env_knob("HYPERMVAR_STEP_GLUE", 6)}};
 }
 
 namespace hmv {
@@ -398,10 +398,13 @@
 }
 
 namespace {
+bool tf_norm_in_kernel(bool bands, int64_t flags, int F, const double* ffdtf) {
+  return bands || (!(flags & HMV_FLAG_UNFUSED_NORM) && (F % 16 == 0) && (reinterpret_cast<uintptr_t>(ffdtf) % 16 == 0));
+}
 int tf_ffdtf_impl(const char* who, const double* ar, int64_t n_items, int m, int p, const double* tw, int F, double* ffdtf,
                   double* band_out, const int32_t* bin_lo, const int32_t* bin_hi, int n_bands, double* den, double* H,
                   int32_t* info, double pivot_tau, void* workspace, int64_t workspace_bytes, int64_t flags,
-                  void* ev_k3_start, void* ev_k3_stop, void* stream) {
+                  void* ev_k3_start, void* ev_k3_stop, void* stream, bool prepacked = false) {
   auto failw = [&](int code, const char* msg) {
     char buf[200];
     snprintf(buf, sizeof(buf), "%s: %s", who, msg);
@@ -429,7 +432,7 @@
   a.P = reinterpret_cast<double*>(base + w.off_P); a.rowsum = reinterpret_cast<double*>(base + w.off_rowsum);
   a.H = H;
   a.info = info; a.n_items = n_items; a.F = F; a.p = p; a.m = m; a.tau = pivot_tau;
-  const bool fused = bands || (!(flags & HMV_FLAG_UNFUSED_NORM) && (F % 16 == 0) && (reinterpret_cast<uintptr_t>(ffdtf) % 16 == 0));
+  const bool fused = tf_norm_in_kernel(bands, flags, F, ffdtf);
   const int64_t lag = norm_lag_items(mp, F);
   const int64_t n_fused = fused ? n_items : 0;
   if (n_fused > 0) {
@@ -446,7 +449,8 @@
   a.stamps = g_tf_stamps;
 #endif
   hipStream_t st = S(stream);
-  int rc = hmv::launch_tf_inv(a, mp, st, reinterpret_cast<hipEvent_t>(ev_k3_start), reinterpret_cast<hipEvent_t>(ev_k3_stop));
+  int rc = hmv::launch_tf_inv(a, mp, st, reinterpret_cast<hipEvent_t>(ev_k3_start), reinterpret_cast<hipEvent_t>(ev_k3_stop),
+                              prepacked);
   if (rc) return rc;
   if (n_fused < n_items) {
     const int64_t n_tail = n_items - n_fused;
@@ -645,13 +649,37 @@
   double* tw = reinterpret_cast<double*>(base + w.off_tw);
   const bool k3_bands = bands && a.measure == MEAS_FFDTF;
   const int64_t tfws_bytes = (int64_t)tf_ff_layout(a.chunk, mp, a.p, a.F, k3_bands).total;
-  rc = hmv_twiddles_f64(a.freqs, a.F, a.fs, a.p, tw, st0);
+  const bool ldl = (a.flags & (HMV_FLAG_YW_TILED | HMV_FLAG_YW_ONE_LAUNCH)) || hmv::tuning(HMV_TUNE_YW_FORM) == 1;
+  const bool glue = hmv::tuning(HMV_TUNE_STEP_GLUE) == 0 && (automatic || (!ldl && hmv::tuning(HMV_TUNE_YW_FORM) != 3));
+  if (!glue) rc = hmv_twiddles_f64(a.freqs, a.F, a.fs, a.p, tw, st0);
   const size_t ws_item = (size_t)hmv_yw_workspace_doubles(a.m, a.p);
   for (int64_t ci = 0; ci < n_chunks && rc == 0; ++ci) {
     const int64_t i0 = ci * a.chunk;
     const int64_t c = (a.n_items - i0 < a.chunk) ? (a.n_items - i0) : a.chunk;
     double* ar_c = a.ar_out ? a.ar_out + (size_t)i0 * t * a.p : ar;
     double* V_c = a.V_out ? a.V_out + (size_t)i0 * t : V;
+    hmv::YwArgs ya{};
+    ya.R = R; ya.n_items = c; ya.m = a.m; ya.p = a.p; ya.ws = ws; ya.ar = ar_c; ya.V = V_c; ya.info = a.info_yw + i0;
+    ya.tiled = -1;
+    double* full_c = (a.measure == MEAS_FFDTF) ? nullptr
+                     : bands ? reinterpret_cast<double*>(base + w.off_full) : a.ffdtf + (size_t)i0 * a.m * a.m * a.F;
+    double* ff_c = k3_bands ? nullptr : (full_c ? full_c : a.ffdtf + (size_t)i0 * a.m * a.m * a.F);
+    if (glue) {
+      if (a.measure != MEAS_GPDC) {
+        const TfFfWs tl = tf_ff_layout(c, mp, a.p, a.F, k3_bands);
+        ya.arx = reinterpret_cast<double*>(static_cast<char*>(tfws) + tl.off_arx);
+        ya.skip_ar = !a.ar_out && a.measure == MEAS_FFDTF && !a.S_out;
+        if (tf_norm_in_kernel(k3_bands, a.flags, a.F, ff_c)) {
+          ya.wcount = reinterpret_cast<int*>(static_cast<char*>(tfws) + tl.off_cnt);
+          ya.ready = ya.wcount + c;
+          ya.missed = ya.ready + c;
+        }
+      }
+      if (ci == 0) {
+        ya.tw = tw; ya.freqs = a.freqs; ya.fs = a.fs; ya.F = a.F;
+      }
+    }
+    const int64_t rec0 = regular ? i0 / a.grid_nwin : 0, w00 = regular ? i0 - rec0 * a.grid_nwin : 0;
     if (a.ens) {
       hmv::LagcovEnsArgs ea{};
       ea.x = a.x; ea.rec_stride = a.rec_stride; ea.ld = a.ld; ea.T = a.ens->T;
@@ -665,6 +693,13 @@
         ea.it0 = i0; ea.nwin = a.grid_nwin; ea.hop = a.grid_hop; ea.k = (int)(a.n / a.grid_hop); ea.Q = Qb;
       }
       rc = hmv::launch_lagcov_ensemble(ea, mp, ens_shared, st0);
+    } else if (regular && glue && w00 + c <= a.grid_nwin && hmv::yw_lwr_takes_blocks(mp, a.p)) {
+      const int k = (int)(a.n / a.grid_hop);
+      hmv::LagcovArgs la{};
+      la.x = a.x + rec0 * a.rec_stride; la.ld = a.ld; la.n_items = c + k - 1; la.m = a.m; la.n = (int)a.grid_hop; la.p = a.p;
+      la.R = Qb; la.blocks = 1; la.blk_first = a.grid_first + w00 * a.grid_hop; la.blk_T = a.grid_T;
+      rc = hmv::launch_lagcov(la, mp, st0);
+      ya.Q = Qb; ya.x = la.x; ya.x_ld = a.ld; ya.x_first = la.blk_first; ya.x_hop = a.grid_hop; ya.x_T = a.grid_T; ya.x_k = k;
     } else if (regular) {
       for (int64_t it = i0; it < i0 + c && rc == 0;) {
         const int64_t rec = it / a.grid_nwin, w0 = it - rec * a.grid_nwin;
@@ -678,16 +713,12 @@
     }
     if (rc) break;
     if (automatic) {
-      hmv::YwArgs ya{};
-      ya.R = R; ya.n_items = c; ya.m = a.m; ya.p = a.p; ya.ws = ws; ya.ar = ar_c; ya.V = V_c; ya.info = a.info_yw + i0;
-      ya.tiled = -1;
       hmv::YwAutoArgs sel{};
       sel.n = a.n; sel.crit_c = crit_factor(a.crit, a.n); sel.order_out = a.order_out + i0;
       sel.crit_out = a.crit_out ? a.crit_out + (size_t)i0 * a.p : nullptr;
       rc = hmv::launch_yw_auto(ya, sel, mp, st0);
       if (rc) break;
     }
-    const bool ldl = (a.flags & (HMV_FLAG_YW_TILED | HMV_FLAG_YW_ONE_LAUNCH)) || hmv::tuning(HMV_TUNE_YW_FORM) == 1;
     const bool tiled = (a.flags & HMV_FLAG_YW_TILED) || (ldl && !(a.flags & HMV_FLAG_YW_ONE_LAUNCH) && mp == 64 && c >= 128);
     const int64_t yw_flags = (a.flags & ~(int64_t)(HMV_FLAG_YW_TILED | HMV_FLAG_YW_ONE_LAUNCH)) |
                              (ldl ? (tiled ? HMV_FLAG_YW_TILED : HMV_FLAG_YW_ONE_LAUNCH) : 0);
@@ -706,20 +737,21 @@
       }
       if (rc) break;
     }
-    if (!automatic) rc = hmv_yw_solve_f64(R, c0, a.m, a.p, ws, ar_c, V_c, nullptr, a.info_yw + i0, yw_flags, st0);
+    if (!automatic) {
+      ya.n_items = c0;
+      ya.tiled = (yw_flags & HMV_FLAG_YW_TILED) ? 1 : ((yw_flags & HMV_FLAG_YW_ONE_LAUNCH) ? 0 : -1);
+      rc = hmv::launch_yw(ya, mp, st0);
+    }
     if (rc) break;
     const bool last = (ci == n_chunks - 1);
     double* Hc = a.S_out ? reinterpret_cast<double*>(base + w.off_H) : nullptr;
-    double* full_c = (a.measure == MEAS_FFDTF) ? nullptr
-                     : bands ? reinterpret_cast<double*>(base + w.off_full) : a.ffdtf + (size_t)i0 * a.m * a.m * a.F;
     if (a.measure == MEAS_GPDC) {
       rc = hmv::launch_gpdc_sliding(ar_c, V_c, tw, full_c, c, a.F, a.m, mp, a.p, st0);
     } else {
-      rc = tf_ffdtf_impl(a.who, ar_c, c, a.m, a.p, tw, a.F,
-                         k3_bands ? nullptr : (full_c ? full_c : a.ffdtf + (size_t)i0 * a.m * a.m * a.F),
+      rc = tf_ffdtf_impl(a.who, ar_c, c, a.m, a.p, tw, a.F, ff_c,
                          k3_bands ? a.band_out + (size_t)i0 * a.m * a.m * a.n_bands : nullptr, a.bin_lo, a.bin_hi,
                          a.n_bands, den, Hc, a.info_tf + (size_t)i0 * a.F, a.pivot_tau, tfws, tfws_bytes, a.flags,
-                         last ? a.ev_k3_start : nullptr, last ? a.ev_k3_stop : nullptr, st0);
+                         last ? a.ev_k3_start : nullptr, last ? a.ev_k3_stop : nullptr, st0, glue);
     }
     if (!rc && a.measure == MEAS_DDTF) {
       hmv::DdtfArgs da{};
diff --git a/hyperscanning_signal_analysis_amd/csrc/hmv_common.h b/hyperscanning_signal_analysis_amd/csrc/hmv_common.h
--- a/hyperscanning_signal_analysis_amd/csrc/hmv_common.h
+++ b/hyperscanning_signal_analysis_amd/csrc/hmv_common.h
@@ -119,4 +119,24 @@
   return v;
 }
 
+__device__ __forceinline__ void twiddle_at(const double* freqs, double fs, int p, int idx, double* tw) {
+  const int f = idx / p, k = idx - f * p;
+  const double c = (double)(-(k + 1) * 2) * 3.141592653589793;
+  const double th = c * freqs[f] / fs;
+  double s, co;
+  sincos(th, &s, &co);
+  tw[2 * idx] = co;
+  tw[2 * idx + 1] = s;
 }
+
+template <int NT>
+__device__ __forceinline__ void arx_slot(int r, int P2, int& h, int& row, int& col) {
+  const int lane = r & 63; r >>= 6;
+  h = r % P2; r /= P2;
+  const int Jl = r & 3; r >>= 2;
+  const int Ig = r % NT, w = r / NT;
+  row = 16 * Ig + 4 * ((lane >> 2) & 3) + (lane >> 4);
+  col = 4 * (Jl * NT + w) + (lane & 3);
+}
+
+}
diff --git a/hyperscanning_signal_analysis_amd/csrc/hmv_kernels.h b/hyperscanning_signal_analysis_amd/csrc/hmv_kernels.h
--- a/hyperscanning_signal_analysis_amd/csrc/hmv_kernels.h
+++ b/hyperscanning_signal_analysis_amd/csrc/hmv_kernels.h
@@ -60,6 +60,19 @@
   int tiled;
   int only_guarded;
   const int* order;
+  const double* Q;
+  const double* x;
+  long long x_ld, x_first, x_hop, x_T;
+  int x_k;
+  double* arx;
+  int skip_ar;
+  int* wcount;
+  int* ready;
+  int* missed;
+  double* tw;
+  const double* freqs;
+  double fs;
+  int F;
 };
 struct YwAutoArgs {
   int n;
@@ -71,6 +84,7 @@
 int launch_yw(const YwArgs& a, int m_pad, hipStream_t st);
 int launch_yw_lwr(const YwArgs& a, int m_pad, hipStream_t st);
 int launch_yw_lwr2(const YwArgs& a, int m_pad, hipStream_t st);
+bool yw_lwr_takes_blocks(int m_pad, int p);
 int launch_yw_auto(const YwArgs& a, const YwAutoArgs& s, int m_pad, hipStream_t st);
 int launch_yw_guarded(const YwArgs& a, int m_pad, hipStream_t st);
 
@@ -102,7 +116,8 @@
   unsigned long long* stamps;
 };
 int launch_twiddles(const double* freqs, int F, double fs, int p, double* tw, hipStream_t st);
-int launch_tf_inv(const TfArgs& a, int m_pad, hipStream_t st, hipEvent_t ev_start = nullptr, hipEvent_t ev_stop = nullptr);
+int launch_tf_inv(const TfArgs& a, int m_pad, hipStream_t st, hipEvent_t ev_start = nullptr, hipEvent_t ev_stop = nullptr,
+                  bool prepacked = false);
 int launch_cinv(const TfArgs& a, int m_pad, hipStream_t st);
 long long tf_workspace_doubles(long long n_items, int m_pad, int p);
 int tf_band_max_F(int m_pad);
diff --git a/hyperscanning_signal_analysis_amd/csrc/lagcov.hip b/hyperscanning_signal_analysis_amd/csrc/lagcov.hip
--- a/hyperscanning_signal_analysis_amd/csrc/lagcov.hip
+++ b/hyperscanning_signal_analysis_amd/csrc/lagcov.hip
@@ -109,7 +109,7 @@
     const int ch = idx / lag, u = idx - ch * lag;
     const long long ta = s + n - lag + u, tb = s + n + u;
     xa[ch * 32 + u] = (ch < m && ta < a.T) ? a.x[(size_t)ch * a.ld + ta] : 0.0;
-    xb[ch * 32 + u] = (ch < m && tb < a.T) ? a.x[(size_t)ch * a.ld + tb] : 0.0;
+    xb[ch * 32 + ((u + ch) & 31)] = (ch < m && tb < a.T) ? a.x[(size_t)ch * a.ld + tb] : 0.0;
   }
   __syncthreads();
   const double inv_n = 1.0 / (double)n;
@@ -120,7 +120,7 @@
     double acc = 0.0;
     for (int j = 0; j < a.k; ++j) acc += Q[(size_t)j * (a.p + 1) * TILE + e];
     double c = 0.0;
-    for (int u = 0; u < lag; ++u) c = __builtin_fma(xa[row * 32 + u], xb[col * 32 + u], c);
+    for (int u = 0; u < lag; ++u) c = __builtin_fma(xa[row * 32 + u], xb[col * 32 + ((u + col) & 31)], c);
     double v = (acc - c) * inv_n;
     if (lag == 0 && row == col && row >= m) v = 1.0;
     R[e] = v;
diff --git a/hyperscanning_signal_analysis_amd/csrc/tf_inv.hip b/hyperscanning_signal_analysis_amd/csrc/tf_inv.hip
--- a/hyperscanning_signal_analysis_amd/csrc/tf_inv.hip
+++ b/hyperscanning_signal_analysis_amd/csrc/tf_inv.hip
@@ -858,13 +858,8 @@
   const long long idx = (long long)blockIdx.x * 256 + threadIdx.x;
   if (idx >= n_items * per_item) return;
   const long long item = idx / per_item;
-  long long r = idx - item * per_item;
-  const int lane = (int)(r & 63); r >>= 6;
-  const int h = (int)(r % P2); r /= P2;
-  const int Jl = (int)(r & 3); r >>= 2;
-  const int Ig = (int)(r % NT);
-  const int w = (int)(r / NT);
-  const int row = 16 * Ig + 4 * ((lane >> 2) & 3) + (lane >> 4), col = 4 * (Jl * NT + w) + (lane & 3);
+  int h, row, col;
+  arx_slot<NT>((int)(idx - item * per_item), P2, h, row, col);
   const double* e = ar + ((size_t)item * MP * MP + (size_t)row * MP + col) * p;
   double2 v;
   v.x = e[2 * h];
@@ -875,13 +870,7 @@
 __global__ void twiddle_kernel(const double* freqs, int F, double fs, int p, double* tw) {
   const int idx = blockIdx.x * blockDim.x + threadIdx.x;
   if (idx >= F * p) return;
-  const int f = idx / p, k = idx - f * p;
-  const double c = (double)(-(k + 1) * 2) * 3.141592653589793;
-  const double th = c * freqs[f] / fs;
-  double s, co;
-  sincos(th, &s, &co);
-  tw[2 * idx] = co;
-  tw[2 * idx + 1] = s;
+  twiddle_at(freqs, fs, p, idx, tw);
 }
 
 int launch_twiddles(const double* freqs, int F, double fs, int p, double* tw, hipStream_t st) {
@@ -904,14 +893,15 @@
   return n_items * (long long)m_pad * m_pad * 2 * ((p + 1) / 2);
 }
 
-int launch_tf_inv(const TfArgs& a_in, int m_pad, hipStream_t st, hipEvent_t ev_start, hipEvent_t ev_stop) {
+int launch_tf_inv(const TfArgs& a_in, int m_pad, hipStream_t st, hipEvent_t ev_start, hipEvent_t ev_stop, bool prepacked) {
   TfArgs a = a_in;
   if (a.n_items == 0 || a.F == 0) return 0;
   const bool fused = ((a.ff != nullptr || a.bands != nullptr) && a.fuse_items > 0);
   if (fused) {
     if (!a.P || !a.den || !a.wcount || !a.ready || !a.missed || a.lag < 1) return -3;
     if (a.bands && (!a.band_lo || !a.band_hi || a.nb < 1 || a.F % 32 != 0 || a.F > tf_band_max_F(m_pad) || a.A)) return -3;
-    if (const hipError_t e = hipMemsetAsync(a.wcount, 0, sizeof(int) * (2 * (size_t)a.n_items + 1), st)) return (int)e;
+    if (!prepacked)
+      if (const hipError_t e = hipMemsetAsync(a.wcount, 0, sizeof(int) * (2 * (size_t)a.n_items + 1), st)) return (int)e;
   } else {
     a.ff = nullptr;
     a.bands = nullptr;
@@ -921,12 +911,12 @@
   const long long slots = a.n_items * (long long)m_pad * m_pad * ((a.p + 1) / 2);
   const dim3 pgrid((unsigned)((slots + 255) / 256));
   double* arx = const_cast<double*>(a.arx);
-  switch (m_pad) {
+  if (m_pad != 16 && m_pad != 32 && m_pad != 48 && m_pad != 64) return -1;
+  if (!prepacked) switch (m_pad) {
     case 16: hipLaunchKernelGGL(ar_pack_kernel<1>, pgrid, dim3(256), 0, st, a.ar, arx, a.n_items, a.p); break;
     case 32: hipLaunchKernelGGL(ar_pack_kernel<2>, pgrid, dim3(256), 0, st, a.ar, arx, a.n_items, a.p); break;
     case 48: hipLaunchKernelGGL(ar_pack_kernel<3>, pgrid, dim3(256), 0, st, a.ar, arx, a.n_items, a.p); break;
     case 64: hipLaunchKernelGGL(ar_pack_kernel<4>, pgrid, dim3(256), 0, st, a.ar, arx, a.n_items, a.p); break;
-    default: return -1;
   }
   if (ev_start)
     if (const hipError_t e = hipEventRecord(ev_start, st)) return (int)e;
diff --git a/hyperscanning_signal_analysis_amd/csrc/yw_auto.hip b/hyperscanning_signal_analysis_amd/csrc/yw_auto.hip
--- a/hyperscanning_signal_analysis_amd/csrc/yw_auto.hip
+++ b/hyperscanning_signal_analysis_amd/csrc/yw_auto.hip
@@ -12,6 +12,10 @@
   if (a.n_items == 0) return 0;
   a.order = nullptr;
   a.only_guarded = 0;
+  a.skip_ar = 0;
+  if (a.Q && (!a.x || a.x_k < 1 || !yw_lwr_takes_blocks(m_pad, a.p))) return -3;
+  if (a.wcount && (!a.ready || !a.missed)) return -3;
+  if (a.tw && (!a.freqs || a.F < 1)) return -3;
   const dim3 grid((unsigned)a.n_items), block(256);
   switch (m_pad) {
     case 16: hipLaunchKernelGGL((yw_auto_kernel<1>), grid, block, 0, st, a, sel); break;
diff --git a/hyperscanning_signal_analysis_amd/csrc/yw_common.h b/hyperscanning_signal_analysis_amd/csrc/yw_common.h
--- a/hyperscanning_signal_analysis_amd/csrc/yw_common.h
+++ b/hyperscanning_signal_analysis_amd/csrc/yw_common.h
@@ -20,6 +20,30 @@
 }
 __host__ __device__ inline int* yw_guard_ptr(double* ws, long long item, int p, int tile) {
   return reinterpret_cast<int*>(ws + (size_t)(item + 1) * yw_ws_tiles_d(p) * tile) - 1;
+}
+
+template <int NT>
+__device__ __forceinline__ void yw_emit(const double* T, size_t se, size_t sk, int q, int pa, double* ar, double* arx) {
+  constexpr int MP = 16 * NT, TILE = MP * MP;
+  if (ar) {
+    const int total = TILE * pa;
+    for (int idx = threadIdx.x; idx < total; idx += 256) {
+      const int e = idx / pa, k = idx - e * pa;
+      ar[idx] = (k < q) ? T[(size_t)e * se + (size_t)k * sk] : 0.0;
+    }
+  }
+  if (arx) {
+    const int P2 = (pa + 1) >> 1, slots = TILE * P2;
+    for (int idx = threadIdx.x; idx < slots; idx += 256) {
+      int h, row, col;
+      arx_slot<NT>(idx, P2, h, row, col);
+      const double* e = T + ((size_t)row * MP + col) * se;
+      f64x2 v;
+      v.x = (2 * h < q) ? e[(size_t)(2 * h) * sk] : 0.0;
+      v.y = (2 * h + 1 < q) ? e[(size_t)(2 * h + 1) * sk] : 0.0;
+      reinterpret_cast<f64x2*>(arx)[idx] = v;
+    }
+  }
 }
 
 template <int NT>
diff --git a/hyperscanning_signal_analysis_amd/csrc/yw_lwr.hip b/hyperscanning_signal_analysis_amd/csrc/yw_lwr.hip
--- a/hyperscanning_signal_analysis_amd/csrc/yw_lwr.hip
+++ b/hyperscanning_signal_analysis_amd/csrc/yw_lwr.hip
@@ -7,9 +7,18 @@
   yw_lwr_body<NT, VQ, false>(a, YwAutoArgs{});
 }
 
+bool yw_lwr_takes_blocks(int m_pad, int p) {
+  if (m_pad != 16 && m_pad != 32 && m_pad != 48 && m_pad != 64) return false;
+  return (long long)m_pad * (2 * p + 1) <= yw_lwr_buf_doubles(m_pad / 16);
+}
+
 int launch_yw_lwr(const YwArgs& a, int m_pad, hipStream_t st) {
   if (a.n_items == 0) return 0;
-  if (tuning(4 ) == 3) return launch_yw_lwr2(a, m_pad, st);
+  const bool glue = a.Q || a.arx || a.skip_ar || a.wcount || a.tw;
+  if (tuning(4 ) == 3) return glue ? -3 : launch_yw_lwr2(a, m_pad, st);
+  if (a.Q && (!a.x || a.x_k < 1 || !yw_lwr_takes_blocks(m_pad, a.p))) return -3;
+  if (a.wcount && (!a.ready || !a.missed)) return -3;
+  if (a.tw && (!a.freqs || a.F < 1)) return -3;
   const dim3 grid((unsigned)a.n_items), block(256);
   const bool vq = (a.Vq_logdet != nullptr);
   switch (m_pad) {
diff --git a/hyperscanning_signal_analysis_amd/csrc/yw_lwr_core.h b/hyperscanning_signal_analysis_amd/csrc/yw_lwr_core.h
--- a/hyperscanning_signal_analysis_amd/csrc/yw_lwr_core.h
+++ b/hyperscanning_signal_analysis_amd/csrc/yw_lwr_core.h
@@ -6,6 +6,11 @@
 #ifndef HMV_LWR_GUARD
 #define HMV_LWR_GUARD 1e-7
 #endif
+
+__host__ __device__ constexpr int yw_lwr_buf_doubles(int NT) {
+  const int MP = 16 * NT, SH = MP / 2 + 6, S = (MP <= 38) ? 38 : 70;
+  return 2 * MP * SH > MP * S ? 2 * MP * SH : MP * S;
+}
 
 template <int NT, bool VQ, bool AUTO>
 __device__ __forceinline__ void yw_lwr_body(const YwArgs& a, const YwAutoArgs& sel) {
@@ -14,6 +19,7 @@
   constexpr int NV = (MP * KH / 2 + 255) / 256;
   constexpr int SI = YwCfg<NT>::S;
   constexpr int GEMM_D = 2 * MP * SH, INV_D = MP * SI, BUF_D = GEMM_D > INV_D ? GEMM_D : INV_D;
+  static_assert(BUF_D == yw_lwr_buf_doubles(NT), "the launcher's size rule for the edge samples");
   __shared__ __attribute__((aligned(16))) double buf[BUF_D];
   __shared__ double Pb[2 * MP * 4];
   __shared__ double Nb[4 * MP * 4];
@@ -45,6 +51,45 @@
       s_qstar = 0;
     }
   }
+  if (a.Q) {
+    const int ES = 2 * p + 1;
+    const int n = (int)(a.x_hop * a.x_k);
+    const long long s0 = a.x_first + item * a.x_hop + n - p;
+    for (int idx = threadIdx.x; idx < MP * 2 * p; idx += 256) {
+      const int ch = idx / (2 * p), v = idx - ch * (2 * p);
+      const long long t = s0 + v;
+      buf[ch * ES + v] = (ch < a.m && t < a.x_T) ? a.x[(size_t)ch * a.x_ld + t] : 0.0;
+    }
+    __syncthreads();
+    const double inv_n = 1.0 / (double)n;
+    const size_t qs = (size_t)(p + 1) * TILE;
+    for (int lag = 0; lag <= p; ++lag) {
+      const double* Q = a.Q + ((size_t)item * (p + 1) + lag) * TILE;
+      double* Rw = const_cast<double*>(R) + (size_t)lag * TILE;
+      for (int e = threadIdx.x; e < TILE; e += 256) {
+        const int row = e / MP, col = e - row * MP;
+        double sum = 0.0;
+        for (int j = 0; j < a.x_k; ++j) sum += Q[(size_t)j * qs + e];
+        const double* xa = buf + row * ES + p - lag;
+        const double* xb = buf + col * ES + p;
+        double c = 0.0;
+        for (int u = 0; u < lag; ++u) c = __builtin_fma(xa[u], xb[u], c);
+        double v = (sum - c) * inv_n;
+        if (lag == 0 && row == col && row >= a.m) v = 1.0;
+        Rw[e] = v;
+      }
+    }
+    __syncthreads();
+  }
+  auto k3_prep = [&]() __attribute__((always_inline)) {
+    if (a.wcount && threadIdx.x == 0) {
+      a.wcount[item] = 0;
+      a.ready[item] = 0;
+      if (item == 0) a.missed[0] = 0;
+    }
+    if (a.tw && item == 0)
+      for (int idx = threadIdx.x; idx < a.F * p; idx += 256) twiddle_at(a.freqs, a.fs, p, idx, a.tw);
+  };
 
   auto lane = [&]() __attribute__((always_inline)) {
     int lo;
@@ -340,6 +385,8 @@
       double* Vo = a.V + (size_t)item * TILE;
       for (int idx = threadIdx.x; idx < TILE; idx += 256) Vo[idx] = R[idx];
     }
+    if (a.arx) yw_emit<NT>(ar, p, 1, qs, p, nullptr, a.arx + (size_t)item * TILE * 2 * ((p + 1) >> 1));
+    k3_prep();
     return;
   }
   load_tile(g, Vf, false);
@@ -348,13 +395,9 @@
     a.info[item] = s_info;
     *yw_guard_ptr(a.ws, item, p, TILE) = (s_info == 0) ? s_guard : 0;
   }
-  const double* Af = Agen[p & 1];
-  double* ar = a.ar + (size_t)item * TILE * p;
-  const int total = TILE * p;
-  for (int idx = threadIdx.x; idx < total; idx += 256) {
-    const int e = idx / p, k = idx - e * p;
-    ar[idx] = Af[(size_t)k * TILE + e];
-  }
+  yw_emit<NT>(Agen[p & 1], 1, TILE, p, p, a.skip_ar ? nullptr : a.ar + (size_t)item * TILE * p,
+              a.arx ? a.arx + (size_t)item * TILE * 2 * ((p + 1) >> 1) : nullptr);
+  k3_prep();
 }
 
 }
diff --git a/hyperscanning_signal_analysis_amd/csrc/yw_solve.hip b/hyperscanning_signal_analysis_amd/csrc/yw_solve.hip
--- a/hyperscanning_signal_analysis_amd/csrc/yw_solve.hip
+++ b/hyperscanning_signal_analysis_amd/csrc/yw_solve.hip
@@ -294,12 +294,8 @@
     __syncthreads();
   }
   const int pa = a.p;
-  double* ar = a.ar + (size_t)item * TILE * pa;
-  const int total = TILE * pa;
-  for (int idx = threadIdx.x; idx < total; idx += 256) {
-    const int e = idx / pa, k = idx - e * pa;
-    ar[idx] = (k < p) ? q.Zt[(size_t)k * TILE + e] : 0.0;
-  }
+  yw_emit<NT>(q.Zt, 1, TILE, p, pa, a.skip_ar ? nullptr : a.ar + (size_t)item * TILE * pa,
+              a.arx ? a.arx + (size_t)item * TILE * 2 * ((pa + 1) >> 1) : nullptr);
 }
 
 template <int NT>
@@ -339,6 +335,7 @@
   a.order = nullptr;
   if (a.n_items == 0) return 0;
   const long long form = tuning(4 );
+  if (!(a.tiled < 0 && form != 1) && (a.Q || a.arx || a.skip_ar || a.wcount || a.tw)) return -3;
   if (a.tiled < 0 && form != 1) {
     int rc = launch_yw_lwr(a, m_pad, st);
     if (rc) return rc;
diff --git a/include/hypermvar.h b/include/hypermvar.h
--- a/include/hypermvar.h
+++ b/include/hypermvar.h
@@ -19,6 +19,7 @@
 #define HMV_TUNE_K3_FORM 3
 #define HMV_TUNE_YW_FORM 4
 #define HMV_TUNE_K3_LDS_PAD 5
+#define HMV_TUNE_STEP_GLUE 6
 int hmv_set_tuning(int key, int64_t value);
 int64_t hmv_get_tuning(int key);
 int64_t hmv_yw_workspace_doubles(int m, int p);
```

Measured after the change: 57070 windows/s. Within noise of the previous version (-0.3%).
